# hzykent/LiDAL

Measured on AMD Instinct MI355X. Metric: voxels/sec SPVCNN fwd+bwd @120k pts, higher is better.
Workload: dtype bf16; 1 GPU; spvcnn train step (train.py:127-140: fwd + CE + bwd + Adam), 5 scans x ~120k pts per GPU, 0.05 m voxels, kernel maps rebuilt every step (each step builds the next step's coordinate tables on a second stream; variants.inline_geometry: built inside the forward pass); parallelism=dp1

## Files before the change

include/lidal_amd.h:

```cpp
#ifndef LIDAL_AMD_H
#define LIDAL_AMD_H

#include <stdint.h>

#ifdef __cplusplus
extern "C" {
#endif

#define LIDAL_F32 0
#define LIDAL_BF16 1
#define LIDAL_F32_SPLIT 2

const char* lidal_last_error(void);
int lidal_version(void);

int lidal_hash(const int32_t* coords, int64_t n, int64_t* out, void* stream);
int lidal_floor_coords(const float* coords, int64_t n, int stride, int32_t* out, void* stream);
int lidal_revoxelize_coords(const float* coords, int64_t n, float init_res, float after_res, float* out_float,
                            int32_t* out_floor, void* stream);
int lidal_kernel_hash(const int32_t* coords, int64_t n, const int32_t* offsets, int k,
                      int64_t* out, void* stream);

int64_t lidal_hash_table_bytes(int64_t n_keys);
int lidal_hash_table_build(const int64_t* keys, int64_t n, void* table, int64_t table_bytes,
                           void* stream);
int lidal_hash_table_build_coords(const int32_t* coords, int64_t n, int stride, void* table, int64_t table_bytes,
                                  void* stream);
int lidal_hash_table_query(const void* table, int64_t table_bytes, const int64_t* q, int64_t nq,
                           int64_t* out, void* stream);

int64_t lidal_unique_workspace_bytes(int64_t n);
int lidal_unique_sorted_i64(const int64_t* keys, int64_t n, int64_t* out, int64_t* n_out_dev,
                            void* ws, int64_t ws_bytes, void* stream);
int64_t lidal_downsample_workspace_bytes(int64_t n);
int lidal_downsample(const int32_t* coords, int64_t n, int sx, int sy, int sz, int32_t* out,
                     int64_t* n_out_dev, void* ws, int64_t ws_bytes, void* stream);

int64_t lidal_downsample_pyramid_workspace_bytes(int64_t n, int levels);
int lidal_downsample_pyramid(const int32_t* coords, int64_t n, int sx, int sy, int sz, int levels, int32_t* out,
                             int64_t* starts_dev, void* ws, int64_t ws_bytes, void* stream);

int64_t lidal_voxelize_points_workspace_bytes(int64_t p);
int lidal_voxelize_points(const float* points, const float* intensity, int64_t p,
                          const double* m_dev, const double* rnd_dev, double scale, int full_scale,
                          float* feats_p, int32_t* coords_v, int64_t* unique_idx, int64_t* inverse,
                          int64_t* n_out_dev, int32_t* n_invalid_dev, void* ws, int64_t ws_bytes,
                          void* stream);

int64_t lidal_train_labels_workspace_bytes(int64_t p);
int lidal_train_labels(const void* raw, int raw_bytes, int64_t p, const int64_t* label_map, int map_len,
                       const int64_t* sv_ptr, const int64_t* sv_idx, int64_t nnz, int s, const int64_t* sv_flag,
                       const int64_t* pseudo, const int64_t* unique_idx, int64_t n, int64_t* labels_p,
                       int64_t* labels_v, int32_t* n_invalid_dev, void* ws, int64_t ws_bytes, void* stream);

int64_t lidal_kmap_workspace_bytes(int64_t n_out, int k);
int lidal_kmap_build(const void* table, int64_t table_bytes, const int32_t* out_coords,
                     int64_t n_out, const int32_t* offsets, int k, int symmetric, int32_t* nbr_out,
                     int32_t* nbmaps, int32_t* nbsizes, int64_t* koff, int mode, void* ws,
                     int64_t ws_bytes, void* stream);
int lidal_kmap_from_rules(const int32_t* nbmaps, const int32_t* nbsizes, int k, int64_t n_rules,
                          int64_t n_in, int64_t n_out, int32_t* nbr_out, int32_t* n_bad_dev, void* stream);
int64_t lidal_kmap_build_batch_workspace_bytes(const int64_t* n_out, const int32_t* k, int n_jobs);
int lidal_kmap_build_batch(const void* const* tables, const int64_t* table_bytes,
                           const int32_t* const* out_coords, const int64_t* n_out,
                           const int32_t* const* offsets, const int32_t* k, const int32_t* symmetric,
                           int32_t* const* nbr_out, int32_t* const* nbmaps, int32_t* const* nbsizes,
                           int64_t* const* koff, int n_jobs, void* ws, int64_t ws_bytes, void* stream);
int lidal_kmap_invert(const int32_t* nbr_out, int64_t n_out, int k, int32_t* nbr_in, int64_t n_in,
                      void* stream);

int64_t lidal_sort_pairs_workspace_bytes(int64_t n);
int lidal_sort_pairs(const uint32_t* keys_in, const int32_t* vals_in, uint32_t* keys_out, int32_t* vals_out,
                     int64_t n, int bits, void* ws, int64_t ws_bytes, void* stream);
int lidal_sort_pairs_u64(const uint64_t* keys_in, const int32_t* vals_in, uint64_t* keys_out, int32_t* vals_out,
                         int64_t n, int bits, void* ws, int64_t ws_bytes, void* stream);
int64_t lidal_kmap_order_workspace_bytes(int64_t n_rows);
int lidal_kmap_order_batch(const int32_t* const* nbr, const int64_t* n_rows, int n_jobs, int k,
                           int32_t* const* perm, int32_t* const* nbr_perm, uint32_t* const* tile_masks,
                           void* ws, int64_t ws_bytes, void* stream);
int lidal_kmap_order(const int32_t* nbr, int64_t n_rows, int k, int32_t* perm, int32_t* nbr_perm,
                     uint32_t* tile_masks, void* ws, int64_t ws_bytes, void* stream);

int lidal_count(const int32_t* idx, int64_t n, int32_t* out, int64_t m, void* stream);
int lidal_voxelize_fwd(const float* feat, const int32_t* idx, const int32_t* counts, float* out,
                       int64_t n, int64_t m, int c, void* stream);
int lidal_voxelize_fwd_1to1(const void* feat, const int32_t* idx, void* out, int64_t n, int c, int dtype,
                            void* stream);
int lidal_voxelize_bwd(const void* gout, const int32_t* idx, const int32_t* counts,
                       const void* residual, void* gin, int64_t n, int64_t m, int c, int dtype,
                       void* stream);
int lidal_devoxelize_fwd(const void* feat, const int32_t* idx, const float* w, void* out,
                         int64_t n, int64_t m, int c, int dtype, void* stream);
int lidal_devoxelize_bwd(const float* gout, const int32_t* idx, const float* w, float* gin,
                         int64_t n, int64_t m, int c, void* stream);
int64_t lidal_invlist_workspace_bytes(int64_t n_entries);
int lidal_invlist_build(const int32_t* idx, const float* w, int64_t n_entries, int64_t m,
                        int32_t* order, int64_t* seg_ptr, void* ws, int64_t ws_bytes, void* stream);
int64_t lidal_segment_workspace_bytes(int64_t n_entries, int64_t m, int c);
int lidal_voxelize_fwd_sorted(const void* feat, const int32_t* order, const int64_t* seg_ptr,
                              const int32_t* counts, void* out, int64_t m, int c, int dtype,
                              int64_t n_entries, void* ws, int64_t ws_bytes, void* stream);
int lidal_devoxelize_bwd_sorted(const void* gout, const int32_t* order, const int64_t* seg_ptr,
                                const float* w, void* gin, int64_t m, int c, int dtype,
                                int64_t n_entries, void* ws, int64_t ws_bytes, void* stream);
int64_t lidal_devoxelize_bwd_cells_workspace_bytes(int64_t m, int c);
int lidal_devoxelize_bwd_cells(const void* gout, const int32_t* vorder, const int64_t* vseg, const float* w8,
                               const int32_t* corder, const int64_t* cseg, void* gin, int64_t m, int c, int dtype,
                               void* ws, int64_t ws_bytes, void* stream);
int lidal_ti_weights(const float* coords, int cstride, const int64_t* idx, int64_t n, float scale,
                     float* w, int32_t* idx32, void* stream);

int lidal_conv_stats_tile_rows(void);
int64_t lidal_conv_weight_image_bytes(int k, int ci, int co, int dtype, int64_t n_out);
int lidal_conv_weight_image_tiling(int ci, int co, int dtype, int64_t n_out);
int lidal_conv_weight_image(const void* w, int w_dtype, int role, void* img, int dtype, int k,
                            int n_red, int n_col, int64_t n_out, void* stream);
int lidal_conv_weight_image_pair(const void* w, int w_dtype, void* img_fwd, int64_t n_out_fwd,
                                 void* img_bwd, int64_t n_out_bwd, int dtype, int k, int ci, int co,
                                 void* stream);
int lidal_conv_weight_image_job_bytes(void);
int64_t lidal_conv_weight_image_job(void* job, const void* w, int role, void* img_fwd,
                                    int64_t n_out_fwd, void* img_bwd, int64_t n_out_bwd, int dtype,
                                    int k, int ci, int co, int64_t first);
int lidal_conv_weight_image_batch(const void* jobs, int n_jobs, int64_t total_segments, int w_dtype,
                                  int dtype, void* stream);
int lidal_conv_apply_image(const void* in, const void* wimg, const int32_t* nbr, const int32_t* perm,
                           const uint32_t* tile_masks, void* out, int64_t n_in, int64_t n_out,
                           int ci, int co, int k, int kflip, int dtype, const float* ep_scale,
                           const float* ep_shift, int ep_relu, const void* ep_residual,
                           float* tile_stats, void* stream);
int64_t lidal_conv_apply_workspace_bytes(int64_t n_out, int co);
int lidal_conv_apply_image_ws(const void* in, const void* wimg, const int32_t* nbr, const int32_t* perm,
                              const uint32_t* tile_masks, void* out, int64_t n_in, int64_t n_out,
                              int ci, int co, int k, int kflip, int dtype, const float* ep_scale,
                              const float* ep_shift, int ep_relu, const void* ep_residual,
                              float* tile_stats, void* ws, int64_t ws_bytes, void* stream);
int lidal_conv_dgrad_bn_sums(const void* gout, const void* wimg, const int32_t* nbr, const int32_t* perm,
                             const uint32_t* tile_masks, void* gin, int64_t n_gout, int64_t n_gin, int c_gout,
                             int c_gin, int k, int kflip, int dtype, const void* bn_x, const float* bn_mean,
                             const float* bn_invstd, const float* bn_gamma, const float* bn_beta, int bn_relu,
                             float* bn_sums, void* stream);
int lidal_conv_dgrad_bn_sums_ws(const void* gout, const void* wimg, const int32_t* nbr, const int32_t* perm,
                                const uint32_t* tile_masks, void* gin, int64_t n_gout, int64_t n_gin, int c_gout,
                                int c_gin, int k, int kflip, int dtype, const void* bn_x, const float* bn_mean,
                                const float* bn_invstd, const float* bn_gamma, const float* bn_beta, int bn_relu,
                                float* bn_sums, void* ws, int64_t ws_bytes, void* stream);
int64_t lidal_conv_wgrad_slabs(int64_t n_a, int64_t n_b, int k, int ca, int cb, int dtype);
int lidal_conv_wgrad(const void* a, const void* b, int64_t n_a, int64_t n_b, const int32_t* pairs,
                     const int64_t* koff, int a_col, float* gw, float* partial, int64_t n_slabs,
                     int k, int ca, int cb, int dtype, void* stream);

int lidal_wgrad_streams_workgroups(void);
int64_t lidal_wgrad_streams_rules(int64_t n_rows, int k, int n_wg);
int64_t lidal_wgrad_streams_desc_words(int k, int n_wg);
int64_t lidal_wgrad_streams_workspace_bytes(int64_t n_rows, int k);
int lidal_wgrad_streams_build(const int32_t* pairs, const int64_t* koff, int k, int64_t n_rows, const int32_t* key_tab,
                              int key_k, int64_t key_range, int n_wg, int32_t* spairs, int64_t spairs_rules,
                              int32_t* sdesc, void* ws, int64_t ws_bytes, void* stream);
int lidal_conv_wgrad_streams_serves(int64_t n_a, int64_t n_b, int k, int ca, int cb);
int lidal_conv_wgrad_streams(const void* a, const void* b, int64_t n_a, int64_t n_b, const int32_t* spairs,
                             const int32_t* sdesc, int n_wg, int a_col, float* gw, float* partial, int64_t n_slabs,
                             int k, int ca, int cb, int dtype, void* stream);

int64_t lidal_bn_workspace_bytes(int64_t n, int c);
int lidal_bn_train_fwd(const void* x, int dtype, int64_t n, int c, const float* gamma,
                       const float* beta, float eps, float momentum, float* running_mean,
                       float* running_var, int64_t* num_batches_tracked, int relu,
                       const void* residual, void* y, float* save_mean, float* save_invstd, void* ws,
                       int64_t ws_bytes, void* stream);
int lidal_bn_train_fwd_tiles(const void* x, int dtype, int64_t n, int c, const float* gamma,
                             const float* beta, float eps, float momentum, float* running_mean,
                             float* running_var, int64_t* num_batches_tracked, int relu,
                             const void* residual, void* y, float* save_mean, float* save_invstd,
                             const float* tile_stats, int64_t n_tiles, void* stream);
int lidal_bn_eval_fwd(const void* x, int dtype, int64_t n, int c, const float* gamma,
                      const float* beta, const float* running_mean, const float* running_var,
                      float eps, int relu, void* y, void* stream);
int lidal_bn_bwd(const void* x, const void* dy, int64_t dy_stride, int dtype, int64_t n, int c, const float* gamma,
                 const float* beta, int relu, const float* save_mean, const float* save_invstd,
                 void* dx, float* grad_gamma, float* grad_beta, void* ws, int64_t ws_bytes,
                 void* stream);
int lidal_bn_bwd_tiles(const void* x, const void* dy, int64_t dy_stride, int dtype, int64_t n, int c,
                       const float* gamma, const float* beta, int relu, const float* save_mean,
                       const float* save_invstd, void* dx, float* grad_gamma, float* grad_beta,
                       const float* tile_sums, int64_t n_tiles, void* stream);
int lidal_add_relu_bwd_bn_sums(const void* out, const void* g, void* gm, int dtype, int64_t n, int c,
                               const void* x_a, const float* mean_a, const float* invstd_a, void* part_a,
                               const void* x_b, const float* mean_b, const float* invstd_b, void* part_b,
                               int64_t part_bytes, void* stream);
int64_t lidal_bn_tail_parts(int64_t n, int c, int dtype);
int lidal_add_relu_bwd_bn_tile_sums(const void* out, const void* g, void* gm, int dtype, int64_t n, int c,
                                    const void* x_a, const float* mean_a, const float* invstd_a, float* sums_a,
                                    const void* x_b, const float* mean_b, const float* invstd_b, float* sums_b,
                                    int64_t n_parts, void* stream);
int lidal_bn_bwd_from_sums(const void* x, const void* dy, int64_t dy_stride, int dtype, int64_t n, int c,
                           const float* gamma, const float* beta, int relu, const float* save_mean,
                           const float* save_invstd, void* dx, float* grad_gamma, float* grad_beta,
                           const void* part, int64_t part_bytes, void* stream);
int lidal_bn_set_fused(int on);
int lidal_bn_set_slab_sums(int on);
int lidal_bn_check_device(void);
int lidal_bn_fold(const float* gamma, const float* beta, const float* running_mean,
                  const float* running_var, float eps, int c, float* scale, float* shift,
                  void* stream);
int lidal_colsum(const void* x, int dtype, int64_t n, int c, float* out, void* ws,
                 int64_t ws_bytes, void* stream);

int lidal_add_relu_fwd(const void* a, const void* b, void* y, int64_t numel, int dtype,
                       void* stream);
int lidal_add_relu_bwd(const void* y, const void* g, void* gin, int64_t numel, int dtype,
                       void* stream);
int64_t lidal_ce_workspace_bytes(int64_t n);
int lidal_ce_fwd(const void* logits, int dtype, const int64_t* labels, int64_t n, int c,
                 int64_t ignore_index, float* out2, void* ws, int64_t ws_bytes, void* stream);
int lidal_ce_bwd(const void* logits, int dtype, const int64_t* labels, int64_t n, int c,
                 int64_t ignore_index, const float* fwd_out2, const float* grad_scale,
                 void* dlogits, void* stream);

int lidal_view_mean_softmax(const float* logits, const int64_t* inverse, int reps, int64_t p,
                            int c, float* prob, int64_t* pred, void* stream);

int lidal_confusion_accumulate(const float* logits, const int64_t* inverse, const int64_t* labels,
                               int64_t p, int c, int32_t* conf, void* stream);

int lidal_register_points(const float* points, int64_t p, const double* pose_dev, double* world,
                          void* stream);
int64_t lidal_nn_grid_bytes(int64_t p);
int64_t lidal_nn_grid_workspace_bytes(int64_t p);
int lidal_nn_grid_build(const double* pts, int64_t p, double cell, void* grid, int64_t grid_bytes,
                        void* ws, int64_t ws_bytes, void* stream);
int64_t lidal_interframe_workspace_bytes(int64_t p, int n_nei);
int lidal_interframe_score(const double* q_pts, const float* q_prob, int64_t p, int c,
                           const void* const* nei_grids_host, const double* const* nei_pts_host,
                           const float* const* nei_prob_host, const int64_t* nei_p_host,
                           int n_nei, double dis_thresh, double* interd, float* intere,
                           int32_t* map_count, void* ws, int64_t ws_bytes, void* stream);
int lidal_interframe_score_ordered(const double* q_pts, const float* q_prob, int64_t p, int c,
                                   const void* const* nei_grids_host, const double* const* nei_pts_host,
                                   const float* const* nei_prob_host, const int64_t* nei_p_host,
                                   int n_nei, double dis_thresh, double* interd, float* intere,
                                   int32_t* map_count, void* ws, int64_t ws_bytes, const void* q_grid,
                                   void* stream);
int lidal_supervoxel_reduce(const double* interd, const float* intere, const double* pts,
                            const int64_t* sv_ptr, const int64_t* sv_idx, int s, float* sv_interd,
                            float* sv_intere, float* sv_center, void* stream);

int64_t lidal_knn_workspace_bytes(int64_t p);
int lidal_knn(const float* xyz, int64_t p, int k, double cell, int32_t* knn, void* ws, int64_t ws_bytes, void* stream);
int lidal_surface_variation(const float* xyz, int64_t p, int k, double cell, float threshold, float* sigma, void* ws,
                            int64_t ws_bytes, void* stream);
int64_t lidal_region_scores_workspace_bytes(int64_t p);
int lidal_region_scores(const float* prob, int64_t p, int c, const float* feat, int d, const float* curvature,
                        const int64_t* sv_ptr, const int64_t* sv_idx, int s, float alpha, float gamma, float* sv_scores,
                        float* sv_feats, int64_t* sv_pnums, void* ws, int64_t ws_bytes, void* stream);
int64_t lidal_kmeans_workspace_bytes(int64_t n, int d, int k, int trials);
int lidal_kmeans(const float* x, int64_t n, int d, int k, int64_t first, const double* u, int trials, int max_iter,
                 double tol, int32_t* seeds, int32_t* labels, double* centers, double* inertia_host,
                 int32_t* n_iter_host, void* ws, int64_t ws_bytes, void* stream);

int64_t lidal_frame_uncertainty_workspace_bytes(int64_t p);
int lidal_frame_uncertainty(const float* prob, int64_t p, int c, float* out, void* ws, int64_t ws_bytes, void* stream);
int64_t lidal_segment_entropy_workspace_bytes(int s);
int lidal_segment_entropy(const int64_t* pred, int64_t p, const int64_t* sv_ptr, const int64_t* sv_idx, int s,
                          int class_num, double* out, void* ws, int64_t ws_bytes, void* stream);
int64_t lidal_frame_feature_workspace_bytes(int64_t p);
int lidal_frame_feature(const float* feat, int64_t p, int d, float* out, void* ws, int64_t ws_bytes, void* stream);
int64_t lidal_coreset_workspace_bytes(int64_t n, int num_add);
int lidal_coreset(const float* feats, int64_t n, int d, const int64_t* labeled, int64_t n_labeled, int num_add,
                  int64_t* picks, float* min_dist, int32_t* status_dev, void* ws, int64_t ws_bytes, void* stream);

int lidal_copy2d(const void* src, int64_t src_pitch, void* dst, int64_t dst_pitch, int64_t rows, int64_t row_bytes,
                 int64_t zero_bytes, void* stream);
int lidal_add2d(const void* a, int64_t a_stride, const void* b, int64_t b_stride, void* out, int64_t out_stride,
                int64_t rows, int c, int dtype, void* stream);
int lidal_transpose_f32(const float* src, int64_t src_stride, float* dst, int rows, int cols, void* stream);
int lidal_cast_rows_bf16(const float* src, int c_src, void* dst, int c_dst, int64_t n, void* stream);

enum {
  LIDAL_OP_CONV_WEIGHT_IMAGE_BATCH = 1, LIDAL_OP_CONV_APPLY_IMAGE = 2, LIDAL_OP_CONV_DGRAD_BN_SUMS = 3,
  LIDAL_OP_CONV_WGRAD = 4, LIDAL_OP_BN_TRAIN_FWD = 5, LIDAL_OP_BN_TRAIN_FWD_TILES = 6, LIDAL_OP_BN_BWD = 7,
  LIDAL_OP_BN_BWD_TILES = 8, LIDAL_OP_BN_EVAL_FWD = 9, LIDAL_OP_BN_FOLD = 10, LIDAL_OP_COLSUM = 11,
  LIDAL_OP_ADD_RELU_FWD = 12, LIDAL_OP_ADD_RELU_BWD = 13, LIDAL_OP_VOXELIZE_FWD_1TO1 = 14,
  LIDAL_OP_VOXELIZE_FWD_SORTED = 15, LIDAL_OP_VOXELIZE_BWD = 16, LIDAL_OP_DEVOXELIZE_FWD = 17,
  LIDAL_OP_DEVOXELIZE_BWD_SORTED = 18, LIDAL_OP_CE_FWD = 19, LIDAL_OP_CE_BWD = 20, LIDAL_OP_COPY2D = 21,
  LIDAL_OP_ADD2D = 22, LIDAL_OP_TRANSPOSE_F32 = 23, LIDAL_OP_CAST_ROWS_BF16 = 24, LIDAL_OP_VIEW_MEAN_SOFTMAX = 25,
  LIDAL_OP_FORK_SIDE = 26, LIDAL_OP_JOIN_SIDE = 27, LIDAL_OP_CONV_APPLY_IMAGE_WS = 28,
  LIDAL_OP_CONV_DGRAD_BN_SUMS_WS = 29, LIDAL_OP_ADD_RELU_BWD_BN_SUMS = 30, LIDAL_OP_BN_BWD_FROM_SUMS = 31,
  LIDAL_OP_ADD_RELU_BWD_BN_TILE_SUMS = 32, LIDAL_OP_DEVOXELIZE_BWD_CELLS = 33,
  LIDAL_OP_CONV_WGRAD_STREAMS = 34
};
#define LIDAL_OP_FLAG_SIDE 1
int lidal_plan_op_args(int kind);
int lidal_debug_read(const void* dev, void* host, int64_t nbytes);
int lidal_plan_run(const int64_t* words, int64_t n_words, int64_t n_ops, void* stream, void* side_stream);
int lidal_plan_run_streams(const int64_t* words, int64_t n_words, int64_t n_ops, void* const* streams, int n_streams);

#ifdef __cplusplus
}
#endif
#endif
```

lidal_amd/backend.py:

```python
import ctypes
import os

import torch

_HERE = os.path.dirname(os.path.abspath(__file__))
LIB_PATH = os.environ.get('LIDAL_AMD_LIB') or os.path.join(_HERE, 'liblidal_amd.so')

F32, BF16 = 0, 1
_lib = None
HITS = {}


def hit(name):
    HITS[name] = HITS.get(name, 0) + 1

_vp, _i32, _i64, _f32, _f64 = (ctypes.c_void_p, ctypes.c_int, ctypes.c_int64, ctypes.c_float,
                               ctypes.c_double)

SIGNATURES = {
    'lidal_last_error': (ctypes.c_char_p, []),
    'lidal_version': (_i32, []),
    'lidal_floor_coords': (_i32, [_vp, _i64, _i32, _vp, _vp]),
    'lidal_revoxelize_coords': (_i32, [_vp, _i64, _f32, _f32, _vp, _vp, _vp]),
    'lidal_hash': (_i32, [_vp, _i64, _vp, _vp]),
    'lidal_kernel_hash': (_i32, [_vp, _i64, _vp, _i32, _vp, _vp]),
    'lidal_hash_table_bytes': (_i64, [_i64]),
    'lidal_hash_table_build_coords': (_i32, [_vp, _i64, _i32, _vp, _i64, _vp]),
    'lidal_hash_table_build': (_i32, [_vp, _i64, _vp, _i64, _vp]),
    'lidal_hash_table_query': (_i32, [_vp, _i64, _vp, _i64, _vp, _vp]),
    'lidal_unique_workspace_bytes': (_i64, [_i64]),
    'lidal_unique_sorted_i64': (_i32, [_vp, _i64, _vp, _vp, _vp, _i64, _vp]),
    'lidal_downsample_workspace_bytes': (_i64, [_i64]),
    'lidal_downsample': (_i32, [_vp, _i64, _i32, _i32, _i32, _vp, _vp, _vp, _i64, _vp]),
    'lidal_downsample_pyramid_workspace_bytes': (_i64, [_i64, _i32]),
    'lidal_downsample_pyramid': (_i32, [_vp, _i64, _i32, _i32, _i32, _i32, _vp, _vp, _vp, _i64, _vp]),
    'lidal_voxelize_points_workspace_bytes': (_i64, [_i64]),
    'lidal_voxelize_points': (_i32, [_vp, _vp, _i64, _vp, _vp, _f64, _i32, _vp, _vp, _vp, _vp, _vp, _vp,
                                     _vp, _i64, _vp]),
    'lidal_train_labels_workspace_bytes': (_i64, [_i64]),
    'lidal_train_labels': (_i32, [_vp, _i32, _i64, _vp, _i32, _vp, _vp, _i64, _i32, _vp, _vp, _vp, _i64, _vp, _vp, _vp,
                                  _vp, _i64, _vp]),
    'lidal_kmap_workspace_bytes': (_i64, [_i64, _i32]),
    'lidal_kmap_build': (_i32, [_vp, _i64, _vp, _i64, _vp, _i32, _i32, _vp, _vp, _vp, _vp, _i32, _vp,
                                _i64, _vp]),
    'lidal_kmap_build_batch_workspace_bytes': (_i64, [_vp, _vp, _i32]),
    'lidal_kmap_build_batch': (_i32, [_vp, _vp, _vp, _vp, _vp, _vp, _vp, _vp, _vp, _vp, _vp, _i32, _vp, _i64, _vp]),
    'lidal_kmap_invert': (_i32, [_vp, _i64, _i32, _vp, _i64, _vp]),
    'lidal_kmap_from_rules': (_i32, [_vp, _vp, _i32, _i64, _i64, _i64, _vp, _vp, _vp]),
    'lidal_count': (_i32, [_vp, _i64, _vp, _i64, _vp]),
    'lidal_voxelize_fwd': (_i32, [_vp, _vp, _vp, _vp, _i64, _i64, _i32, _vp]),
    'lidal_voxelize_fwd_1to1': (_i32, [_vp, _vp, _vp, _i64, _i32, _i32, _vp]),
    'lidal_voxelize_bwd': (_i32, [_vp, _vp, _vp, _vp, _vp, _i64, _i64, _i32, _i32, _vp]),
    'lidal_devoxelize_fwd': (_i32, [_vp, _vp, _vp, _vp, _i64, _i64, _i32, _i32, _vp]),
    'lidal_devoxelize_bwd': (_i32, [_vp, _vp, _vp, _vp, _i64, _i64, _i32, _vp]),
    'lidal_invlist_workspace_bytes': (_i64, [_i64]),
    'lidal_invlist_build': (_i32, [_vp, _vp, _i64, _i64, _vp, _vp, _vp, _i64, _vp]),
    'lidal_segment_workspace_bytes': (_i64, [_i64, _i64, _i32]),
    'lidal_voxelize_fwd_sorted': (_i32, [_vp, _vp, _vp, _vp, _vp, _i64, _i32, _i32, _i64, _vp, _i64, _vp]),
    'lidal_devoxelize_bwd_sorted': (_i32, [_vp, _vp, _vp, _vp, _vp, _i64, _i32, _i32, _i64, _vp, _i64, _vp]),
    'lidal_devoxelize_bwd_cells': (_i32, [_vp, _vp, _vp, _vp, _vp, _vp, _vp, _i64, _i32, _i32, _vp, _i64, _vp]),
    'lidal_devoxelize_bwd_cells_workspace_bytes': (_i64, [_i64, _i32]),
    'lidal_ti_weights': (_i32, [_vp, _i32, _vp, _i64, _f32, _vp, _vp, _vp]),
    'lidal_sort_pairs_workspace_bytes': (_i64, [_i64]),
    'lidal_sort_pairs': (_i32, [_vp, _vp, _vp, _vp, _i64, _i32, _vp, _i64, _vp]),
    'lidal_sort_pairs_u64': (_i32, [_vp, _vp, _vp, _vp, _i64, _i32, _vp, _i64, _vp]),
    'lidal_kmap_order_workspace_bytes': (_i64, [_i64]),
    'lidal_kmap_order': (_i32, [_vp, _i64, _i32, _vp, _vp, _vp, _vp, _i64, _vp]),
    'lidal_kmap_order_batch': (_i32, [_vp, _vp, _i32, _i32, _vp, _vp, _vp, _vp, _i64, _vp]),
    'lidal_conv_stats_tile_rows': (_i32, []),
    'lidal_conv_weight_image_bytes': (_i64, [_i32, _i32, _i32, _i32, _i64]),
    'lidal_conv_weight_image_tiling': (_i32, [_i32, _i32, _i32, _i64]),
    'lidal_conv_weight_image': (_i32, [_vp, _i32, _i32, _vp, _i32, _i32, _i32, _i32, _i64, _vp]),
    'lidal_conv_weight_image_pair': (_i32, [_vp, _i32, _vp, _i64, _vp, _i64, _i32, _i32, _i32, _i32, _vp]),
    'lidal_conv_weight_image_job_bytes': (_i32, []),
    'lidal_conv_weight_image_job': (_i64, [_vp, _vp, _i32, _vp, _i64, _vp, _i64, _i32, _i32, _i32, _i32, _i64]),
    'lidal_conv_weight_image_batch': (_i32, [_vp, _i32, _i64, _i32, _i32, _vp]),
    'lidal_conv_apply_image': (_i32, [_vp, _vp, _vp, _vp, _vp, _vp, _i64, _i64, _i32, _i32, _i32, _i32, _i32, _vp,
                                      _vp, _i32, _vp, _vp, _vp]),
    'lidal_conv_dgrad_bn_sums': (_i32, [_vp, _vp, _vp, _vp, _vp, _vp, _i64, _i64, _i32, _i32, _i32, _i32, _i32, _vp,
                                        _vp, _vp, _vp, _vp, _i32, _vp, _vp]),
    'lidal_conv_apply_workspace_bytes': (_i64, [_i64, _i32]),
    'lidal_conv_apply_image_ws': (_i32, [_vp, _vp, _vp, _vp, _vp, _vp, _i64, _i64, _i32, _i32, _i32, _i32, _i32, _vp,
                                         _vp, _i32, _vp, _vp, _vp, _i64, _vp]),
    'lidal_conv_dgrad_bn_sums_ws': (_i32, [_vp, _vp, _vp, _vp, _vp, _vp, _i64, _i64, _i32, _i32, _i32, _i32, _i32, _vp,
                                           _vp, _vp, _vp, _vp, _i32, _vp, _vp, _i64, _vp]),
    'lidal_conv_wgrad_slabs': (_i64, [_i64, _i64, _i32, _i32, _i32, _i32]),
    'lidal_conv_wgrad': (_i32, [_vp, _vp, _i64, _i64, _vp, _vp, _i32, _vp, _vp, _i64, _i32, _i32, _i32, _i32, _vp]),
    'lidal_conv_wgrad_streams': (_i32, [_vp, _vp, _i64, _i64, _vp, _vp, _i32, _i32, _vp, _vp, _i64, _i32, _i32, _i32, _i32, _vp]),
    'lidal_conv_wgrad_streams_serves': (_i32, [_i64, _i64, _i32, _i32, _i32]),
    'lidal_wgrad_streams_workgroups': (_i32, []),
    'lidal_wgrad_streams_rules': (_i64, [_i64, _i32, _i32]),
    'lidal_wgrad_streams_desc_words': (_i64, [_i32, _i32]),
    'lidal_wgrad_streams_workspace_bytes': (_i64, [_i64, _i32]),
    'lidal_wgrad_streams_build': (_i32, [_vp, _vp, _i32, _i64, _vp, _i32, _i64, _i32, _vp, _i64, _vp, _vp, _i64, _vp]),
    'lidal_bn_workspace_bytes': (_i64, [_i64, _i32]),
    'lidal_bn_train_fwd': (_i32, [_vp, _i32, _i64, _i32, _vp, _vp, _f32, _f32, _vp, _vp, _vp, _i32, _vp, _vp, _vp,
                                  _vp, _vp, _i64, _vp]),
    'lidal_bn_train_fwd_tiles': (_i32, [_vp, _i32, _i64, _i32, _vp, _vp, _f32, _f32, _vp, _vp, _vp, _i32, _vp, _vp,
                                        _vp, _vp, _vp, _i64, _vp]),
    'lidal_bn_eval_fwd': (_i32, [_vp, _i32, _i64, _i32, _vp, _vp, _vp, _vp, _f32, _i32, _vp, _vp]),
    'lidal_bn_bwd': (_i32, [_vp, _vp, _i64, _i32, _i64, _i32, _vp, _vp, _i32, _vp, _vp, _vp, _vp, _vp, _vp,
                            _i64, _vp]),
    'lidal_bn_bwd_tiles': (_i32, [_vp, _vp, _i64, _i32, _i64, _i32, _vp, _vp, _i32, _vp, _vp, _vp, _vp, _vp, _vp,
                                  _i64, _vp]),
    'lidal_add_relu_bwd_bn_sums': (_i32, [_vp, _vp, _vp, _i32, _i64, _i32, _vp, _vp, _vp, _vp, _vp, _vp, _vp, _vp, _i64, _vp]),
    'lidal_add_relu_bwd_bn_tile_sums': (_i32, [_vp, _vp, _vp, _i32, _i64, _i32, _vp, _vp, _vp, _vp, _vp, _vp, _vp, _vp, _i64, _vp]),
    'lidal_bn_tail_parts': (_i64, [_i64, _i32, _i32]),
    'lidal_bn_bwd_from_sums': (_i32, [_vp, _vp, _i64, _i32, _i64, _i32, _vp, _vp, _i32, _vp, _vp, _vp, _vp, _vp, _vp,
                                      _i64, _vp]),
    'lidal_bn_set_fused': (_i32, [_i32]),
    'lidal_bn_set_slab_sums': (_i32, [_i32]),
    'lidal_bn_check_device': (_i32, []),
    'lidal_bn_fold': (_i32, [_vp, _vp, _vp, _vp, _f32, _i32, _vp, _vp, _vp]),
    'lidal_colsum': (_i32, [_vp, _i32, _i64, _i32, _vp, _vp, _i64, _vp]),
    'lidal_add_relu_fwd': (_i32, [_vp, _vp, _vp, _i64, _i32, _vp]),
    'lidal_add_relu_bwd': (_i32, [_vp, _vp, _vp, _i64, _i32, _vp]),
    'lidal_ce_workspace_bytes': (_i64, [_i64]),
    'lidal_ce_fwd': (_i32, [_vp, _i32, _vp, _i64, _i32, _i64, _vp, _vp, _i64, _vp]),
    'lidal_ce_bwd': (_i32, [_vp, _i32, _vp, _i64, _i32, _i64, _vp, _vp, _vp, _vp]),
    'lidal_view_mean_softmax': (_i32, [_vp, _vp, _i32, _i64, _i32, _vp, _vp, _vp]),
    'lidal_confusion_accumulate': (_i32, [_vp, _vp, _vp, _i64, _i32, _vp, _vp]),
    'lidal_register_points': (_i32, [_vp, _i64, _vp, _vp, _vp]),
    'lidal_nn_grid_bytes': (_i64, [_i64]),
    'lidal_nn_grid_workspace_bytes': (_i64, [_i64]),
    'lidal_nn_grid_build': (_i32, [_vp, _i64, _f64, _vp, _i64, _vp, _i64, _vp]),
    'lidal_interframe_workspace_bytes': (_i64, [_i64, _i32]),
    'lidal_interframe_score': (_i32, [_vp, _vp, _i64, _i32, _vp, _vp, _vp, _vp, _i32, _f64, _vp,
                                      _vp, _vp, _vp, _i64, _vp]),
    'lidal_interframe_score_ordered': (_i32, [_vp, _vp, _i64, _i32, _vp, _vp, _vp, _vp, _i32, _f64, _vp,
                                              _vp, _vp, _vp, _i64, _vp, _vp]),
    'lidal_supervoxel_reduce': (_i32, [_vp, _vp, _vp, _vp, _vp, _i32, _vp, _vp, _vp, _vp]),
    'lidal_knn_workspace_bytes': (_i64, [_i64]),
    'lidal_knn': (_i32, [_vp, _i64, _i32, _f64, _vp, _vp, _i64, _vp]),
    'lidal_surface_variation': (_i32, [_vp, _i64, _i32, _f64, _f32, _vp, _vp, _i64, _vp]),
    'lidal_region_scores_workspace_bytes': (_i64, [_i64]),
    'lidal_region_scores': (_i32, [_vp, _i64, _i32, _vp, _i32, _vp, _vp, _vp, _i32, _f32, _f32, _vp, _vp, _vp, _vp,
                                   _i64, _vp]),
    'lidal_kmeans_workspace_bytes': (_i64, [_i64, _i32, _i32, _i32]),
    'lidal_kmeans': (_i32, [_vp, _i64, _i32, _i32, _i64, _vp, _i32, _i32, _f64, _vp, _vp, _vp, _vp, _vp, _vp, _i64,
                            _vp]),
    'lidal_frame_uncertainty_workspace_bytes': (_i64, [_i64]),
    'lidal_frame_uncertainty': (_i32, [_vp, _i64, _i32, _vp, _vp, _i64, _vp]),
    'lidal_segment_entropy_workspace_bytes': (_i64, [_i32]),
    'lidal_segment_entropy': (_i32, [_vp, _i64, _vp, _vp, _i32, _i32, _vp, _vp, _i64, _vp]),
    'lidal_frame_feature_workspace_bytes': (_i64, [_i64]),
    'lidal_frame_feature': (_i32, [_vp, _i64, _i32, _vp, _vp, _i64, _vp]),
    'lidal_coreset_workspace_bytes': (_i64, [_i64, _i32]),
    'lidal_coreset': (_i32, [_vp, _i64, _i32, _vp, _i64, _i32, _vp, _vp, _vp, _vp, _i64, _vp]),
    'lidal_copy2d': (_i32, [_vp, _i64, _vp, _i64, _i64, _i64, _i64, _vp]),
    'lidal_add2d': (_i32, [_vp, _i64, _vp, _i64, _vp, _i64, _i64, _i32, _i32, _vp]),
    'lidal_transpose_f32': (_i32, [_vp, _i64, _vp, _i32, _i32, _vp]),
    'lidal_cast_rows_bf16': (_i32, [_vp, _i32, _vp, _i32, _i64, _vp]),
    'lidal_plan_op_args': (_i32, [_i32]),
    'lidal_debug_read': (_i32, [_vp, _vp, _i64]),
    'lidal_plan_run': (_i32, [_vp, _i64, _i64, _vp, _vp]),
    'lidal_plan_run_streams': (_i32, [_vp, _i64, _i64, _vp, _i32]),
}


class _TimedLib:

    def __init__(self, handle, sink):
        self._handle, self._sink = handle, sink

    def __getattr__(self, name):
        fn = getattr(self._handle, name)
        if fn.restype is not _i32 or name.endswith(('_bytes', '_tiling', '_rows', '_workgroups', '_serves')) or name == 'lidal_version':
            return fn
        sink = self._sink

        def timed(*args):
            e0 = torch.cuda.Event(enable_timing=True)
            e1 = torch.cuda.Event(enable_timing=True)
            e0.record()
            rc = fn(*args)
            e1.record()
            sink(name, args, e0, e1)
            return rc
        return timed


_timer = None


def set_call_timer(sink):
    global _timer
    _timer = None if sink is None else _TimedLib(lib_handle(), sink)


def lib_handle():
    global _lib
    if _lib is None:
        if not os.path.exists(LIB_PATH):
            raise RuntimeError(
                'lidal_amd: %s is missing -- build it with `python -m lidal_amd.build` '
                '(hipcc --offload-arch=gfx950).  There is no CPU fallback.' % LIB_PATH)
        handle = ctypes.CDLL(LIB_PATH)
        for name, (res, args) in SIGNATURES.items():
            fn = getattr(handle, name)
            fn.restype = res
            fn.argtypes = args
        _lib = handle
    return _lib


def lib():
    return _timer if _timer is not None else lib_handle()


def check(rc, what):
    HITS[what] = HITS.get(what, 0) + 1
    if rc != 0:
        raise RuntimeError('lidal_amd.%s failed (%d): %s' %
                           (what, rc, lib().lidal_last_error().decode()))


def bind_cpus_near(device_index=0):
    try:
        props = torch.cuda.get_device_properties(device_index)
        bdf = '%04x:%02x:%02x.0' % (props.pci_domain_id, props.pci_bus_id, props.pci_device_id)
        text = open('/sys/bus/pci/devices/%s/local_cpulist' % bdf).read().strip()
        cpus = set()
        for part in text.split(','):
            if '-' in part:
                a, b = part.split('-')
                cpus.update(range(int(a), int(b) + 1))
            elif part:
                cpus.add(int(part))
        cpus &= os.sched_getaffinity(0)
        if not cpus:
            return None
        os.sched_setaffinity(0, cpus)
        for tid in os.listdir('/proc/self/task'):
            try:
                os.sched_setaffinity(int(tid), cpus)
            except (OSError, ValueError):
                pass
        return cpus
# ... 295 lines not shown
```

lidal_amd/csrc/conv_img.hip:

```cpp
#include <type_traits>

#include "common.h"

using namespace lidal;

namespace {

typedef __attribute__((ext_vector_type(4))) float f32x4;
typedef __attribute__((ext_vector_type(8))) __bf16 bf16x8;
typedef int raw4 __attribute__((ext_vector_type(4)));

template <typename T> struct DT;
template <> struct DT<float> {
  static constexpr int VEC = 4;
  static constexpr int CH = 16;
  typedef f32x4 frag;
  __device__ static float to_f32(float v) { return v; }
  __device__ static float from_f32(float v) { return v; }
};
template <> struct DT<__bf16> {
  static constexpr int VEC = 8;
  static constexpr int CH = 32;
  typedef bf16x8 frag;
  __device__ static float to_f32(__bf16 v) { return (float)v; }
  __device__ static __bf16 from_f32(float v) { return (__bf16)v; }
};

__device__ __forceinline__ void mma(f32x4& acc, const f32x4& a, const f32x4& b) {
#pragma unroll
  for (int e = 0; e < 4; ++e) acc = __builtin_amdgcn_mfma_f32_16x16x4f32(a[e], b[e], acc, 0, 0, 0);
}
__device__ __forceinline__ void mma(f32x4& acc, const bf16x8& a, const bf16x8& b) {
  acc = __builtin_amdgcn_mfma_f32_16x16x32_bf16(a, b, acc, 0, 0, 0);
}

constexpr int MAXK = 32;

constexpr int NB4_LIMIT = 384;
struct Tiling { int nb; int row_bytes; };

__host__ __device__ inline Tiling pick_tiling(int ci, int co, int64_t n_out, int esz) {
  Tiling t;
  const int row_bytes = ci * esz;
  t.row_bytes = (row_bytes % 192 == 0 && row_bytes % 128 != 0) ? 192
                : (row_bytes % 128 != 0 && row_bytes % 64 == 0) ? 64 : 128;
  if (co <= 32) t.nb = 2;
  else if (co <= 64 || (co % 64 == 0 && ((n_out + 127) / 128) * ((co + 127) / 128) <= NB4_LIMIT)) t.nb = 4;
  else if (co % 128 != 0 && (co % 96 == 0 || co < 128)) t.nb = 6;
  else t.nb = 8;
  return t;
}
__host__ __device__ inline int64_t image_bytes(int k, int ci, int co, Tiling t, int esz) {
  const int bn = 16 * t.nb, kc = t.row_bytes / esz;
  const int nblk = (co + bn - 1) / bn, npass = (ci + kc - 1) / kc;
  return (int64_t)k * nblk * npass * bn * t.row_bytes;
}

template <typename TI, typename TO>
__device__ __forceinline__ void image_segment(const TI* __restrict__ w, TO* __restrict__ img, int n_red,
                                              int n_col, int role, int nb, int kc, int64_t s) {
  constexpr int VEC = DT<TO>::VEC, CH = DT<TO>::CH;
  const int bn = 16 * nb, ncc = kc / CH;
  const int nblk = (n_col + bn - 1) / bn, npass = (n_red + kc - 1) / kc;
  unsigned r = (unsigned)s;
  const int row16 = (int)(r & 15u); r >>= 4;
  const int b = (int)(r % (unsigned)nb); r /= (unsigned)nb;
  const int gsel = (int)(r & 3u); r >>= 2;
  const int cc = (int)(r % (unsigned)ncc); r /= (unsigned)ncc;
  const int pass = (int)(r % (unsigned)npass); r /= (unsigned)npass;
  const int blk = (int)(r % (unsigned)nblk); r /= (unsigned)nblk;
  const int k = (int)r;
  const int col = blk * bn + b * 16 + row16;
  const int red0 = pass * kc + cc * CH + gsel * VEC;
  if (role != 0) {
    if (gsel != 0) return;
    const bool inside = col < n_col;
    const int64_t src = (int64_t)k * n_red * n_col + (int64_t)col * n_red + red0;
    float f[CH];
    if (inside && red0 + CH <= n_red && sizeof(TI) == 4 && (n_red & 3) == 0 && (reinterpret_cast<uintptr_t>(w) & 15) == 0) {
#pragma unroll
      for (int e = 0; e < CH; e += 4) {
        const float4 q = *reinterpret_cast<const float4*>(reinterpret_cast<const float*>(w) + src + e);
        f[e] = q.x; f[e + 1] = q.y; f[e + 2] = q.z; f[e + 3] = q.w;
      }
    } else {
#pragma unroll
      for (int e = 0; e < CH; ++e) f[e] = (inside && red0 + e < n_red) ? DT<TI>::to_f32(w[src + e]) : 0.f;
    }
    typedef typename DT<TO>::frag frag;
#pragma unroll
    for (int g = 0; g < 4; ++g) {
      TO v[VEC];
#pragma unroll
      for (int e = 0; e < VEC; ++e) v[e] = DT<TO>::from_f32(f[g * VEC + e]);
      *reinterpret_cast<frag*>(img + (s + (int64_t)g * nb * 16) * VEC) = *reinterpret_cast<frag*>(v);
    }
    return;
  }
  TO v[VEC];
#pragma unroll
  for (int e = 0; e < VEC; ++e) {
    const int red = red0 + e;
    float f = 0.f;
    if (col < n_col && red < n_red) {
      const int64_t base = (int64_t)k * n_red * n_col;
      f = DT<TI>::to_f32(role == 0 ? w[base + (int64_t)red * n_col + col] : w[base + (int64_t)col * n_red + red]);
    }
    v[e] = DT<TO>::from_f32(f);
  }
  typedef typename DT<TO>::frag frag;
  *reinterpret_cast<frag*>(img + s * VEC) = *reinterpret_cast<frag*>(v);
}

template <typename TI, typename TO>
__global__ void __launch_bounds__(256)
weight_image_kernel(const TI* __restrict__ w, TO* __restrict__ img_a, int n_red, int n_col, int role,
                    int nb_a, int kc_a, int64_t segs_a, TO* __restrict__ img_b, int nb_b, int kc_b,
                    int64_t segs_b) {
  const int64_t s = (int64_t)blockIdx.x * blockDim.x + threadIdx.x;
  if (s < segs_a) image_segment<TI, TO>(w, img_a, n_red, n_col, role, nb_a, kc_a, s);
  else if (s < segs_a + segs_b) image_segment<TI, TO>(w, img_b, n_col, n_red, role ^ 1, nb_b, kc_b, s - segs_a);
}

struct ImageJob {
  const void* w; void* img_a; void* img_b;
  long long first, segs_a, segs_b;
  int n_red, n_col, role, nb_a, kc_a, nb_b, kc_b, pad;
};
template <typename TI, typename TO>
__global__ void __launch_bounds__(256)
weight_image_batch_kernel(const ImageJob* __restrict__ jobs, int n_jobs, int64_t total) {
  const int64_t s = (int64_t)blockIdx.x * blockDim.x + threadIdx.x;
  if (s >= total) return;
  int lo = 0, hi = n_jobs - 1;
  while (lo < hi) {
    const int mid = (lo + hi + 1) >> 1;
    if (jobs[mid].first <= s) lo = mid; else hi = mid - 1;
  }
  const ImageJob j = jobs[lo];
  const int64_t l = s - j.first;
  if (l < j.segs_a) image_segment<TI, TO>((const TI*)j.w, (TO*)j.img_a, j.n_red, j.n_col, j.role, j.nb_a, j.kc_a, l);
  else if (l < j.segs_a + j.segs_b)
    image_segment<TI, TO>((const TI*)j.w, (TO*)j.img_b, j.n_col, j.n_red, j.role ^ 1, j.nb_b, j.kc_b, l - j.segs_a);
}

constexpr int TILE_ROWS = 128;
__device__ __forceinline__ int tile_of_block() { return (int)gridDim.x - 1 - (int)blockIdx.x; }
constexpr int LEAN_WAVES = 8;
constexpr int LEAN_MINWAVES = 4;
constexpr int64_t DEEP_MAX_ROWS = 150000;
struct BnBwd {
  const void* x; const float* mean; const float* invstd; const float* gamma; const float* beta;
  float* sums;
  int relu;
};

struct Split { float* partial; int nsplit; int co_pad; long long rows_pad; };

template <typename T, int NB, int G, int NWAVES>
__device__ __forceinline__ void store_tile(f32x4 (&acc)[G][NB], unsigned char* wl, int wave, int lane,
                                           int64_t r0, int n0, int64_t n_out, int co,
                                           const int* __restrict__ perm, T* __restrict__ out,
                                           const float* __restrict__ ep_scale,
                                           const float* __restrict__ ep_shift, int ep_relu,
                                           const T* __restrict__ ep_res, bool perm_in_reg = false,
                                           int perm_v = 0, float* __restrict__ tile_stats = nullptr,
                                           int stats_tile = -1, const BnBwd* bnb = nullptr) {
  constexpr int VEC = DT<T>::VEC;
  constexpr int BN = 16 * NB;
  constexpr int RW = G * 16;
  constexpr int ESTRIDE = BN + VEC;
  typedef typename DT<T>::frag frag;
  const int row16 = lane & 15, gsel = lane >> 4;
  T* et = reinterpret_cast<T*>(wl) + wave * RW * ESTRIDE;
  if (ep_scale != nullptr) {
#pragma unroll
    for (int nb = 0; nb < NB; ++nb) {
      const int col = n0 + nb * 16 + row16;
      const float es = col < co ? ep_scale[col] : 1.f, eh = col < co ? ep_shift[col] : 0.f;
#pragma unroll
      for (int g = 0; g < G; ++g)
#pragma unroll
        for (int r = 0; r < 4; ++r) {
          float v = acc[g][nb][r] * es + eh;
          acc[g][nb][r] = ((ep_relu & 1) && v < 0.f) ? 0.f : v;
        }
    }
  }
#pragma unroll
  for (int g = 0; g < G; ++g)
#pragma unroll
    for (int nb = 0; nb < NB; ++nb)
#pragma unroll
      for (int r = 0; r < 4; ++r)
        et[(g * 16 + gsel * 4 + r) * ESTRIDE + nb * 16 + row16] = DT<T>::from_f32(acc[g][nb][r]);
  __builtin_amdgcn_s_waitcnt(0xC07F);
  constexpr int RSEGS = BN / VEC;
  for (int i = lane; i < RW * RSEGS; i += 64) {
    const int r = i / RSEGS, cseg = (i - r * RSEGS) * VEC;
    const int prow = perm_in_reg ? __shfl(perm_v, r & (RW - 1), 64) : 0;
    if (r0 + r >= n_out) continue;
    const int64_t row = perm ? (perm_in_reg ? (int64_t)prow : (int64_t)perm[r0 + r]) : r0 + r;
    T* dst = out + row * co + n0 + cseg;
    const T* srcp = et + r * ESTRIDE + cseg;
    if (n0 + cseg + VEC <= co) {
      frag v = *reinterpret_cast<const frag*>(srcp);
      if (ep_res != nullptr) {
        const frag rr = *reinterpret_cast<const frag*>(ep_res + row * co + n0 + cseg);
#pragma unroll
        for (int e = 0; e < VEC; ++e) {
          float f = DT<T>::to_f32(v[e]) + DT<T>::to_f32(rr[e]);
          if ((ep_relu & 2) && f < 0.f) f = 0.f;
          v[e] = DT<T>::from_f32(f);
        }
      }
      *reinterpret_cast<frag*>(dst) = v;
    } else {
#pragma unroll
      for (int e = 0; e < VEC; ++e)
        if (n0 + cseg + e < co) {
          float v = DT<T>::to_f32(srcp[e]);
          if (ep_res != nullptr) {
            v += DT<T>::to_f32(ep_res[row * co + n0 + cseg + e]);
            if ((ep_relu & 2) && v < 0.f) v = 0.f;
          }
          dst[e] = DT<T>::from_f32(v);
        }
    }
  }
  if (tile_stats != nullptr) {
    constexpr int EPI_BYTES = NWAVES * RW * ESTRIDE * (int)sizeof(T);
    float* st = reinterpret_cast<float*>(wl + EPI_BYTES);
    const int64_t left = n_out - r0;
    const int nvalid = left <= 0 ? 0 : (left < RW ? (int)left : RW);
    const float inv_n = nvalid > 0 ? 1.f / (float)nvalid : 0.f;
#pragma unroll
    for (int nb = 0; nb < NB; ++nb) {
      float v[G][4];
      float sum = 0.f;
#pragma unroll
      for (int g = 0; g < G; ++g)
#pragma unroll
        for (int r = 0; r < 4; ++r) {
          v[g][r] = DT<T>::to_f32(DT<T>::from_f32(acc[g][nb][r]));
          if (g * 16 + gsel * 4 + r < nvalid) sum += v[g][r];
        }
      sum += __shfl_xor(sum, 16, 64);
      sum += __shfl_xor(sum, 32, 64);
      const float mean = sum * inv_n;
      float m2 = 0.f;
#pragma unroll
      for (int g = 0; g < G; ++g)
#pragma unroll
        for (int r = 0; r < 4; ++r)
          if (g * 16 + gsel * 4 + r < nvalid) { const float d = v[g][r] - mean; m2 += d * d; }
      m2 += __shfl_xor(m2, 16, 64);
      m2 += __shfl_xor(m2, 32, 64);
      if (gsel == 0) {
        st[(wave * BN + nb * 16 + row16) * 2] = mean;
        st[(wave * BN + nb * 16 + row16) * 2 + 1] = m2;
      }
    }
    __syncthreads();
    const int c = wave * 64 + lane;
    if (c < BN && n0 + c < co) {
      const int64_t rb = r0 - (int64_t)wave * RW;
      float na = 0.f, ma = 0.f, qa = 0.f;
      for (int w = 0; w < NWAVES; ++w) {
        const int64_t lw = n_out - (rb + (int64_t)w * RW);
        const float nw = lw <= 0 ? 0.f : (lw < RW ? (float)lw : (float)RW);
        if (nw > 0.f) {
          const float mw = st[(w * BN + c) * 2], qw = st[(w * BN + c) * 2 + 1];
          const float n = na + nw, d = mw - ma;
          ma += d * (nw / n);
          qa += qw + d * d * (na * nw / n);
          na = n;
        }
      }
      float* dst = tile_stats + ((int64_t)(n0 + c) * gridDim.x + (stats_tile >= 0 ? stats_tile : (int)blockIdx.x)) * 3;
      dst[0] = na; dst[1] = ma; dst[2] = qa;
    }
  }
  if (bnb != nullptr && bnb->sums != nullptr) {
    constexpr int EPI_BYTES = NWAVES * RW * ESTRIDE * (int)sizeof(T);
    float* st = reinterpret_cast<float*>(wl + EPI_BYTES);
    const T* bx = reinterpret_cast<const T*>(bnb->x);
    const int64_t left = n_out - r0;
    const int nvalid = left <= 0 ? 0 : (left < RW ? (int)left : RW);
    __builtin_amdgcn_s_waitcnt(0xC07F);
    for (int i = lane; i < RW * RSEGS; i += 64) {
      const int r = i / RSEGS, cseg = (i - r * RSEGS) * VEC;
      const int prow = perm_in_reg ? __shfl(perm_v, r & (RW - 1), 64) : 0;
      frag v;
#pragma unroll
      for (int e = 0; e < VEC; ++e) v[e] = DT<T>::from_f32(0.f);
      if (r < nvalid && n0 + cseg + VEC <= co) {
        const int64_t row = perm ? (perm_in_reg ? (int64_t)prow : (int64_t)perm[r0 + r]) : r0 + r;
        v = *reinterpret_cast<const frag*>(bx + row * co + n0 + cseg);
      }
      *reinterpret_cast<frag*>(et + r * ESTRIDE + cseg) = v;
    }
    __builtin_amdgcn_s_waitcnt(0xC07F);
#pragma unroll
    for (int nb = 0; nb < NB; ++nb) {
      const int col = n0 + nb * 16 + row16;
      const bool cok = col < co;
      const float mu = cok ? bnb->mean[col] : 0.f, is = cok ? bnb->invstd[col] : 0.f;
      const float ga = (cok && bnb->gamma) ? bnb->gamma[col] : 1.f, be = (cok && bnb->beta) ? bnb->beta[col] : 0.f;
      float a = 0.f, b = 0.f;
#pragma unroll
      for (int g = 0; g < G; ++g)
#pragma unroll
        for (int r = 0; r < 4; ++r) {
          const int rr = g * 16 + gsel * 4 + r;
          if (rr < nvalid) {
            const float xh = (DT<T>::to_f32(et[rr * ESTRIDE + nb * 16 + row16]) - mu) * is;
            float dy = DT<T>::to_f32(DT<T>::from_f32(acc[g][nb][r]));
            if (bnb->relu && !(xh * ga + be > 0.f)) dy = 0.f;
            a += dy; b += dy * xh;
          }
        }
      a += __shfl_xor(a, 16, 64); a += __shfl_xor(a, 32, 64);
      b += __shfl_xor(b, 16, 64); b += __shfl_xor(b, 32, 64);
      if (gsel == 0) {
        st[(wave * BN + nb * 16 + row16) * 2] = a;
        st[(wave * BN + nb * 16 + row16) * 2 + 1] = b;
      }
    }
    __syncthreads();
    const int c = wave * 64 + lane;
    if (c < BN && n0 + c < co) {
      float a = 0.f, b = 0.f;
      for (int w = 0; w < NWAVES; ++w) { a += st[(w * BN + c) * 2]; b += st[(w * BN + c) * 2 + 1]; }
      float* dst = bnb->sums + ((int64_t)(n0 + c) * gridDim.x + (stats_tile >= 0 ? stats_tile : (int)blockIdx.x)) * 2;
      dst[0] = a; dst[1] = b;
    }
  }
}

constexpr int IMG_MINWAVES = 2;

template <typename T, int NB, int ROW_BYTES, int G, int NWAVES, int MINW, bool DENSE, int D>
__global__ void __launch_bounds__(64 * NWAVES, MINW)
conv_apply_img_kernel(const T* __restrict__ in, const T* __restrict__ wimg,
                      const int* __restrict__ nbr, const int* __restrict__ perm,
                      const unsigned* __restrict__ tmasks, T* __restrict__ out, int64_t n_out,
                      int ci, int co, int K, int kflip, const float* __restrict__ ep_scale,
                      const float* __restrict__ ep_shift, int ep_relu, const T* __restrict__ ep_res,
                      unsigned in_bytes, unsigned img_bytes, unsigned nbr_bytes,
                      float* __restrict__ tile_stats, BnBwd bnb) {
  constexpr int NTHREADS = 64 * NWAVES;
  constexpr int BM = NWAVES * G * 16;
  constexpr int BN = 16 * NB;
  constexpr int VEC = DT<T>::VEC;
  constexpr int CH = DT<T>::CH;
  constexpr int KC = ROW_BYTES / (int)sizeof(T);
  constexpr int MAXCC = KC / CH;
  constexpr int SLAB = BN * ROW_BYTES;
  constexpr int PIECES = SLAB / 1024;
  constexpr int PPW = (PIECES + NWAVES - 1) / NWAVES;
  constexpr int RW = G * 16;
  constexpr int ESTRIDE = BN + VEC;
  constexpr int EPI = NWAVES * RW * ESTRIDE * (int)sizeof(T);
  constexpr int R = D + 1;
  constexpr int WREGION = (R * SLAB > EPI) ? R * SLAB : EPI;
  constexpr int GA = G * MAXCC;
  static_assert(D >= 1 && D <= 3, "pipeline depth 1..3");
  static_assert(SLAB % 1024 == 0, "slab must be whole LDS-DMA pieces");
  typedef typename DT<T>::frag frag;

  extern __shared__ __attribute__((aligned(16))) unsigned char smem[];
  unsigned char* wl = smem;
  unsigned char* dump = smem + WREGION;

  const int tid = threadIdx.x;
  const int lane = tid & 63;
  const int wave = __builtin_amdgcn_readfirstlane(tid >> 6);
  const int row16 = lane & 15;
  const int gsel = lane >> 4;
  const int bx = tile_of_block();
  const int64_t r0 = (int64_t)bx * BM + wave * RW;
  const int n0 = blockIdx.y * BN;
  const int npass = (ci + KC - 1) / KC;

  unsigned tmask;
  if constexpr (DENSE) {
    tmask = 1u;
  } else {
    unsigned m = 0u;
    const int64_t t0 = ((int64_t)bx * BM) >> 7;
#pragma unroll
    for (int h = 0; h < (BM >= 128 ? BM / 128 : 1); ++h)
      if ((t0 + h) * 128 < n_out) m |= tmasks[t0 + h];
    if (kflip) m = __brev(m) >> (32 - K);
    tmask = m;
  }
  tmask = __builtin_amdgcn_readfirstlane(tmask);
  const int n_act = __popc(tmask);
  const int nphase = n_act * npass;

  struct Walk { unsigned rem; int k; int pass; };
  auto walk_begin = [&]() {
    Walk w;
    w.k = tmask ? __builtin_ctz(tmask) : 0;
    w.rem = tmask & (tmask - 1u);
    w.pass = 0;
    return w;
  };
  auto walk_next = [&](Walk& w) {
    if (++w.pass == npass) {
      w.pass = 0;
      w.k = w.rem ? __builtin_ctz(w.rem) : 0;
      w.rem &= w.rem - 1u;
    }
  };

  constexpr unsigned OOB_OFF = 0x80000000u;
  const __amdgpu_buffer_rsrc_t rs_in =
      __builtin_amdgcn_make_buffer_rsrc(const_cast<T*>(in), 0, (int)in_bytes, 0x00020000);
  const __amdgpu_buffer_rsrc_t rs_w =
      __builtin_amdgcn_make_buffer_rsrc(const_cast<T*>(wimg), 0, (int)img_bytes, 0x00020000);
  const __amdgpu_buffer_rsrc_t rs_nbr =
      __builtin_amdgcn_make_buffer_rsrc(const_cast<int*>(nbr), 0, (int)nbr_bytes, 0x00020000);
  const int nblk = gridDim.y;

  auto stage_dma = [&](int k, int pass, int slot, bool live) {
    const unsigned slab_off = (unsigned)((((int64_t)k * nblk + blockIdx.y) * npass + pass) * SLAB);
#pragma unroll
    for (int t = 0; t < PPW; ++t) {
      const int piece = wave + t * NWAVES;
      const bool ok = live && piece < PIECES;
      unsigned char* dst = ok ? wl + slot * SLAB + piece * 1024 : dump;
      const unsigned soff = ok ? slab_off + (unsigned)piece * 1024u : OOB_OFF;
      __builtin_amdgcn_raw_ptr_buffer_load_lds(rs_w, (__attribute__((address_space(3))) void*)dst, 16,
                                               (unsigned)lane * 16u, soff, 0, 0);
    }
  };
  const unsigned row_off = (unsigned)((r0 + row16) * 4);
  bool row_ok[G];
#pragma unroll
  for (int g = 0; g < G; ++g) row_ok[g] = r0 + g * 16 + row16 < n_out;
  auto load_idx = [&](int (&dst)[G], int k) {
    if constexpr (DENSE) {
#pragma unroll
      for (int g = 0; g < G; ++g) dst[g] = (int)(r0 + g * 16 + row16);
    } else {
      const int kk = kflip ? (K - 1 - k) : k;
      const unsigned koff = (unsigned)kk * (unsigned)n_out * 4u;
#pragma unroll
      for (int g = 0; g < G; ++g)
        dst[g] = __builtin_amdgcn_raw_buffer_load_b32(rs_nbr, row_off + (unsigned)(g * 64), koff, 0);
    }
  };
  auto kill_bit = [&](bool live) {
    unsigned kb = live ? 0u : OOB_OFF;
    asm volatile("" : "+s"(kb));
    return kb;
  };
  auto load_a = [&](raw4 (&a)[G][MAXCC], unsigned long long (&present)[G], const int (&idx)[G],
                    int c0, bool live) {
    const int kc = min(KC, ci - c0);
    const unsigned row_bytes = (unsigned)(ci * (int)sizeof(T));
    const unsigned lane_off = (unsigned)((c0 + gsel * VEC) * (int)sizeof(T));
    const unsigned kill = kill_bit(live);
    const unsigned long long live_mask = kill ? 0ull : ~0ull;
#pragma unroll
    for (int g = 0; g < G; ++g) {
      int src = row_ok[g] ? idx[g] : -1;
      present[g] = __ballot(src != -1) & live_mask;
      const unsigned base = ((src >= 0) ? (unsigned)src * row_bytes + lane_off : OOB_OFF) | kill;
#pragma unroll
      for (int cc = 0; cc < MAXCC; ++cc) {
        const unsigned off = (cc * CH + gsel * VEC < kc) ? base + (unsigned)(cc * CH * (int)sizeof(T)) : OOB_OFF;
        a[g][cc] = __builtin_bit_cast(raw4, __builtin_amdgcn_raw_buffer_load_b128(rs_in, off, 0, 0));
      }
    }
  };

  f32x4 acc[G][NB];
#pragma unroll
  for (int g = 0; g < G; ++g)
#pragma unroll
    for (int nb = 0; nb < NB; ++nb) acc[g][nb] = f32x4{0.f, 0.f, 0.f, 0.f};

// ... 836 lines not shown
  constexpr int SLAB = BN * ROW_BYTES;
  constexpr int EPI = NWAVES * G * 16 * (BN + DT<T>::VEC) * (int)sizeof(T);
  constexpr int D = IMG_DEPTH;
  constexpr int WREGION = ((D + 1) * SLAB > EPI) ? (D + 1) * SLAB : EPI;
  static_assert(BM == TILE_ROWS, "tile masks and BatchNorm statistics triples are per 128-row tile");
  if constexpr (G == 1 && NWAVES == 8) {
    if (ci % (ROW_BYTES / (int)sizeof(T)) == 0 && ep.in_bytes / ((unsigned)ci * sizeof(T)) < (1u << 24)) {
      constexpr int LW = LEAN_WAVES;
      constexpr int LBM = LW * 16;
      static_assert(LBM == TILE_ROWS, "tile masks and BatchNorm statistics triples are per 128-row tile");
      constexpr int LEPI = LW * 16 * (BN + DT<T>::VEC) * (int)sizeof(T);
      constexpr int LSTATS = LW * BN * 2 * (int)sizeof(float);
      constexpr int LEAN_LDS = ((2 * SLAB > LEPI + LSTATS) ? 2 * SLAB : LEPI + LSTATS) + 4096;
      if constexpr (sizeof(T) == 2 && NB == 8 && ROW_BYTES == 128 && LW == 8) {
#ifdef LIDAL_PHASE_STAMPS
       if (false) {
#else
       if (nbr != nullptr && n_out <= DEEP_MAX_ROWS && n_out >= 30000 && ci >= 256) {
#endif
        constexpr int DEPI = LEPI + LSTATS;
        constexpr int DEEP_LDS = ((3 * SLAB > DEPI) ? 3 * SLAB : DEPI) + 4096;
        auto dk = conv_lean_deep_kernel<T, NB, ROW_BYTES, LW, false>;
        static size_t deep_attr[MAX_DEVICES] = {};
        const int ddev = current_device();
        if (deep_attr[ddev] < (size_t)DEEP_LDS) {
          LIDAL_HIP(hipFuncSetAttribute(reinterpret_cast<const void*>(dk),
                                        hipFuncAttributeMaxDynamicSharedMemorySize, DEEP_LDS));
          deep_attr[ddev] = DEEP_LDS;
        }
        dim3 dgrid((unsigned)cdiv(n_out, LBM), (unsigned)cdiv(co, BN));
        dk<<<dgrid, 64 * LW, DEEP_LDS, s>>>((const T*)in, (const T*)wimg, nbr, perm, tmasks, (T*)out, n_out,
                                            ci, co, K, kflip, ep.scale, ep.shift, ep.relu, (const T*)ep.res,
                                            ep.in_bytes, ep.img_bytes, ep.nbr_bytes, ep.tile_stats, ep.bnb);
        LIDAL_CHECK_LAUNCH("lidal_conv_apply_image(deep)");
        return 0;
       }
      }
      auto lk = nbr ? conv_lean_kernel<T, NB, ROW_BYTES, LW, false>
                    : conv_lean_kernel<T, NB, ROW_BYTES, LW, true>;
      static size_t lean_attr[2][MAX_DEVICES] = {};
      const int ldev = current_device();
      if (lean_attr[nbr ? 0 : 1][ldev] < (size_t)LEAN_LDS) {
        LIDAL_HIP(hipFuncSetAttribute(reinterpret_cast<const void*>(lk),
                                      hipFuncAttributeMaxDynamicSharedMemorySize, LEAN_LDS));
        lean_attr[nbr ? 0 : 1][ldev] = LEAN_LDS;
      }
      dim3 lgrid((unsigned)cdiv(n_out, LBM), (unsigned)cdiv(co, BN));
      Split sp{nullptr, 1, 0, 0};
      if (nbr != nullptr && ep.ws != nullptr && sizeof(T) == 2) {
        const int ns = pick_split((int64_t)lgrid.x * lgrid.y, K, ci / (ROW_BYTES / (int)sizeof(T)));
        const long long rows_pad = (long long)lgrid.x * LBM;
        const int co_pad = (int)lgrid.y * BN;
        if (ns > 1 && ep.ws_bytes >= (long long)ns * rows_pad * co_pad * 4)
          sp = Split{(float*)ep.ws, ns, co_pad, rows_pad};
      }
      lgrid.z = (unsigned)sp.nsplit;
      lk<<<lgrid, 64 * LW, LEAN_LDS, s>>>((const T*)in, (const T*)wimg, nbr, perm, tmasks, (T*)out, n_out,
                                          ci, co, K, kflip, ep.scale, ep.shift, ep.relu, (const T*)ep.res,
                                          ep.in_bytes, ep.img_bytes, ep.nbr_bytes, ep.tile_stats, ep.bnb, sp);
      LIDAL_CHECK_LAUNCH("lidal_conv_apply_image(lean)");
      if (sp.nsplit > 1) {
        constexpr int COMB_LDS = LEPI + LSTATS;
        auto ck = conv_combine_kernel<T, NB, LW>;
        static size_t comb_attr[MAX_DEVICES] = {};
        if (comb_attr[ldev] < (size_t)COMB_LDS) {
          LIDAL_HIP(hipFuncSetAttribute(reinterpret_cast<const void*>(ck),
                                        hipFuncAttributeMaxDynamicSharedMemorySize, COMB_LDS));
          comb_attr[ldev] = COMB_LDS;
        }
        lgrid.z = 1;
        ck<<<lgrid, 64 * LW, COMB_LDS, s>>>(sp, perm, (T*)out, n_out, co, ep.scale, ep.shift, ep.relu,
                                            (const T*)ep.res, ep.tile_stats, ep.bnb);
        LIDAL_CHECK_LAUNCH("lidal_conv_apply_image(combine)");
      }
      return 0;
    }
  }
  const size_t lds = WREGION + 1024 + NWAVES * BN * 2 * sizeof(float);
  auto kern = nbr ? conv_apply_img_kernel<T, NB, ROW_BYTES, G, NWAVES, IMG_MINWAVES, false, D>
                  : conv_apply_img_kernel<T, NB, ROW_BYTES, G, NWAVES, IMG_MINWAVES, true, D>;
  static size_t attr_set[2][MAX_DEVICES] = {};
  const int dev = current_device();
  if (attr_set[nbr ? 0 : 1][dev] < lds) {
    LIDAL_HIP(hipFuncSetAttribute(reinterpret_cast<const void*>(kern),
                                  hipFuncAttributeMaxDynamicSharedMemorySize, (int)lds));
    attr_set[nbr ? 0 : 1][dev] = lds;
  }
  dim3 grid((unsigned)cdiv(n_out, BM), (unsigned)cdiv(co, BN));
  kern<<<grid, NTHREADS, lds, s>>>((const T*)in, (const T*)wimg, nbr, perm, tmasks, (T*)out, n_out, ci,
                                   co, K, kflip, ep.scale, ep.shift, ep.relu, (const T*)ep.res,
                                   ep.in_bytes, ep.img_bytes, ep.nbr_bytes, ep.tile_stats, ep.bnb);
  LIDAL_CHECK_LAUNCH("lidal_conv_apply_image");
  return 0;
}

template <typename T>
int dispatch_img(Tiling t, const void* in, const void* wimg, const int* nbr, const int* perm,
                 const unsigned* tmasks, void* out, int64_t n_out, int ci, int co, int K, int kflip,
                 Epi ep, hipStream_t s) {
#define IMG_CASE(NBV, RB) \
  if (t.nb == NBV && t.row_bytes == RB) \
    return launch_img<T, NBV, RB>(in, wimg, nbr, perm, tmasks, out, n_out, ci, co, K, kflip, ep, s);
  IMG_CASE(2, 64) IMG_CASE(4, 64) IMG_CASE(6, 64) IMG_CASE(8, 64)
  IMG_CASE(2, 128) IMG_CASE(4, 128) IMG_CASE(6, 128) IMG_CASE(8, 128)
  IMG_CASE(2, 192) IMG_CASE(4, 192) IMG_CASE(6, 192) IMG_CASE(8, 192)
  IMG_CASE(2, 256) IMG_CASE(4, 256) IMG_CASE(6, 256) IMG_CASE(8, 256)
#undef IMG_CASE
  set_error("conv_apply_image: no kernel for tiling nb=%d row_bytes=%d", t.nb, t.row_bytes);
  return 2;
}


__host__ inline int split_nb(int co) { return co <= 32 ? 2 : (co <= 64 ? 4 : ((co % 128 != 0 && (co % 96 == 0 || co < 128)) ? 6 : 8)); }
__host__ inline int64_t split_image_bytes(int k, int n_red, int n_col) {
  const int bn = 16 * split_nb(n_col);
  return (int64_t)k * ((n_col + bn - 1) / bn) * (n_red / SPLIT_KCH) * bn * SPLIT_ROW;
}
template <int NB>
int launch_split(const void* in, const void* wimg, const int* nbr, const int* perm, const unsigned* tmasks, void* out,
                 int64_t n_out, int ci, int co, int K, int kflip, Epi ep, hipStream_t s) {
  constexpr int LW = 8, BN = 16 * NB, SLAB = BN * SPLIT_ROW;
  constexpr int LEPI_ALL = LW * 16 * (BN + 4) * 4 + LW * BN * 2 * (int)sizeof(float);
  constexpr int LDS = ((2 * SLAB > LEPI_ALL) ? 2 * SLAB : LEPI_ALL) + 4096;
  auto kern = nbr ? conv_split_kernel<NB, LW, false> : conv_split_kernel<NB, LW, true>;
  static size_t attr[2][MAX_DEVICES] = {};
  const int dev = current_device();
  if (attr[nbr ? 0 : 1][dev] < (size_t)LDS) {
    LIDAL_HIP(hipFuncSetAttribute(reinterpret_cast<const void*>(kern), hipFuncAttributeMaxDynamicSharedMemorySize, LDS));
    attr[nbr ? 0 : 1][dev] = LDS;
  }
  dim3 grid((unsigned)cdiv(n_out, LW * 16), (unsigned)cdiv(co, BN));
  Split sp{nullptr, 1, 0, 0};
  if (nbr != nullptr && ep.ws != nullptr) {
    const int64_t wgs = (int64_t)grid.x * grid.y;
    const int ns = (wgs > SPLIT_F32_MAX_WGS || K * (ci / SPLIT_KCH) < 54) ? 1 : (wgs <= 256 ? 4 : 3);
    const long long rows_pad = (long long)grid.x * LW * 16;
    const int co_pad = (int)grid.y * BN;
    if (ns > 1 && ep.ws_bytes >= (long long)ns * rows_pad * co_pad * 4) sp = Split{(float*)ep.ws, ns, co_pad, rows_pad};
  }
  grid.z = (unsigned)sp.nsplit;
  kern<<<grid, 64 * LW, LDS, s>>>((const float*)in, (const __bf16*)wimg, nbr, perm, tmasks, (float*)out, n_out, ci, co, K,
                                  kflip, ep.scale, ep.shift, ep.relu, (const float*)ep.res, ep.in_bytes, ep.img_bytes,
                                  ep.nbr_bytes, sp);
  LIDAL_CHECK_LAUNCH("lidal_conv_apply_image(split)");
  if (sp.nsplit > 1) {
    constexpr int COMB_LDS = LEPI_ALL;
    auto ck = conv_combine_kernel<float, NB, LW>;
    static size_t comb_attr[MAX_DEVICES] = {};
    if (comb_attr[dev] < (size_t)COMB_LDS) {
      LIDAL_HIP(hipFuncSetAttribute(reinterpret_cast<const void*>(ck), hipFuncAttributeMaxDynamicSharedMemorySize, COMB_LDS));
      comb_attr[dev] = COMB_LDS;
    }
    grid.z = 1;
    BnBwd none{nullptr, nullptr, nullptr, nullptr, nullptr, nullptr, 0};
    ck<<<grid, 64 * LW, COMB_LDS, s>>>(sp, perm, (float*)out, n_out, co, ep.scale, ep.shift, ep.relu, (const float*)ep.res,
                                       nullptr, none);
    LIDAL_CHECK_LAUNCH("lidal_conv_apply_image(split, combine)");
  }
  return 0;
}

}

extern "C" int lidal_conv_stats_tile_rows(void) { return TILE_ROWS; }

extern "C" int lidal_conv_weight_image_tiling(int ci, int co, int dtype, int64_t n_out) {
  if (dtype == LIDAL_F32_SPLIT) return split_nb(co) * 1000 + SPLIT_ROW + 1;
  const Tiling t = pick_tiling(ci, co, n_out, dtype == LIDAL_BF16 ? 2 : 4);
  return t.nb * 1000 + t.row_bytes;
}

extern "C" int64_t lidal_conv_weight_image_bytes(int k, int ci, int co, int dtype, int64_t n_out) {
  if (dtype == LIDAL_F32_SPLIT) return (ci > 0 && ci % SPLIT_KCH == 0) ? split_image_bytes(k, ci, co) : -1;
  const int esz = dtype == LIDAL_BF16 ? 2 : 4;
  return image_bytes(k, ci, co, pick_tiling(ci, co, n_out, esz), esz);
}

static int weight_images(const void* w, int w_dtype, int role, void* img_a, int64_t n_out_a, void* img_b,
                         int64_t n_out_b, int dtype, int k, int n_red, int n_col, hipStream_t s) {
  if (k == 0 || n_red == 0 || n_col == 0) return 0;
  LIDAL_REQUIRE(role == 0 || role == 1, "weight_image: role must be 0 (forward) or 1 (data gradient)");
  if (dtype == LIDAL_F32_SPLIT) {
    LIDAL_REQUIRE(img_b == nullptr && n_red % SPLIT_KCH == 0, "weight_image(split): one image per call, reduction a "
                  "multiple of %d channels (got %d)", SPLIT_KCH, n_red);
    const int64_t segs = split_image_bytes(k, n_red, n_col) / 16;
    LIDAL_REQUIRE(segs < (1ll << 31), "weight_image: an image of more than 2^31 segments");
    const unsigned grid = (unsigned)cdiv(segs, 256);
    if (w_dtype == LIDAL_F32)
      weight_image_split_kernel<float><<<grid, 256, 0, s>>>((const float*)w, (__bf16*)img_a, n_red, n_col, role,
                                                            split_nb(n_col), segs);
    else
      weight_image_split_kernel<__bf16><<<grid, 256, 0, s>>>((const __bf16*)w, (__bf16*)img_a, n_red, n_col, role,
                                                             split_nb(n_col), segs);
    LIDAL_CHECK_LAUNCH("lidal_conv_weight_image(split)");
    return 0;
  }
  const int esz = dtype == LIDAL_BF16 ? 2 : 4;
  const Tiling ta = pick_tiling(n_red, n_col, n_out_a, esz);
  const int64_t segs_a = image_bytes(k, n_red, n_col, ta, esz) / 16;
  Tiling tb = ta;
  int64_t segs_b = 0;
  if (img_b != nullptr) {
    tb = pick_tiling(n_col, n_red, n_out_b, esz);
    segs_b = image_bytes(k, n_col, n_red, tb, esz) / 16;
  }
  LIDAL_REQUIRE(segs_a < (1ll << 31) && segs_b < (1ll << 31), "weight_image: an image of more than 2^31 segments");
  const unsigned grid = (unsigned)cdiv(segs_a + segs_b, 256);
#define IMG_LAUNCH(TI, TO) \
  weight_image_kernel<TI, TO><<<grid, 256, 0, s>>>((const TI*)w, (TO*)img_a, n_red, n_col, role, ta.nb, \
                                                   ta.row_bytes / esz, segs_a, (TO*)img_b, tb.nb,       \
                                                   tb.row_bytes / esz, segs_b)
  if (w_dtype == LIDAL_F32 && dtype == LIDAL_F32) IMG_LAUNCH(float, float);
  else if (w_dtype == LIDAL_F32 && dtype == LIDAL_BF16) IMG_LAUNCH(float, __bf16);
  else if (w_dtype == LIDAL_BF16 && dtype == LIDAL_BF16) IMG_LAUNCH(__bf16, __bf16);
  else if (w_dtype == LIDAL_BF16 && dtype == LIDAL_F32) IMG_LAUNCH(__bf16, float);
  else {
    set_error("weight_image: bad dtypes %d %d", w_dtype, dtype);
    return 2;
  }
#undef IMG_LAUNCH
  LIDAL_CHECK_LAUNCH("lidal_conv_weight_image");
  return 0;
}

extern "C" int lidal_conv_weight_image(const void* w, int w_dtype, int role, void* img, int dtype,
                                       int k, int n_red, int n_col, int64_t n_out, void* stream) {
  return weight_images(w, w_dtype, role, img, n_out, nullptr, 0, dtype, k, n_red, n_col, (hipStream_t)stream);
}

extern "C" int lidal_conv_weight_image_pair(const void* w, int w_dtype, void* img_fwd, int64_t n_out_fwd,
                                            void* img_bwd, int64_t n_out_bwd, int dtype, int k, int ci,
                                            int co, void* stream) {
  return weight_images(w, w_dtype, 0, img_fwd, n_out_fwd, img_bwd, n_out_bwd, dtype, k, ci, co,
                       (hipStream_t)stream);
}

extern "C" int lidal_conv_weight_image_job_bytes(void) { return (int)sizeof(ImageJob); }

extern "C" int64_t lidal_conv_weight_image_job(void* job, const void* w, int role, void* img_fwd,
                                               int64_t n_out_fwd, void* img_bwd, int64_t n_out_bwd,
                                               int dtype, int k, int ci, int co, int64_t first) {
  if (job == nullptr || (dtype != LIDAL_F32 && dtype != LIDAL_BF16 && dtype != LIDAL_F32_SPLIT) || (role != 0 && role != 1)) {
    set_error("weight_image_job: bad arguments");
    return -1;
  }
  if (dtype == LIDAL_F32_SPLIT) {
    if (ci % SPLIT_KCH != 0 || (img_bwd != nullptr && co % SPLIT_KCH != 0)) {
      set_error("weight_image_job(split): the reduction must be a multiple of %d channels (got ci=%d%s co=%d)", SPLIT_KCH, ci,
                img_bwd != nullptr ? ", data-gradient image:" : ",", co);
      return -1;
    }
    ImageJob j;
    j.w = w; j.img_a = img_fwd; j.img_b = img_bwd; j.first = first;
    j.segs_a = split_image_bytes(k, ci, co) / 16;
    j.segs_b = img_bwd != nullptr ? split_image_bytes(k, co, ci) / 16 : 0;
    j.n_red = ci; j.n_col = co; j.role = role; j.nb_a = split_nb(co); j.kc_a = 0; j.nb_b = split_nb(ci); j.kc_b = 0; j.pad = 0;
    if (j.segs_a >= (1ll << 31) || j.segs_b >= (1ll << 31)) {
      set_error("weight_image_job: an image of %lld segments", (long long)(j.segs_a > j.segs_b ? j.segs_a : j.segs_b));
      return -1;
    }
    *reinterpret_cast<ImageJob*>(job) = j;
    return j.segs_a + j.segs_b;
  }
  const int esz = dtype == LIDAL_BF16 ? 2 : 4;
  const Tiling ta = pick_tiling(ci, co, n_out_fwd, esz);
  ImageJob j;
  j.w = w; j.img_a = img_fwd; j.img_b = img_bwd; j.first = first;
  j.segs_a = image_bytes(k, ci, co, ta, esz) / 16;
  j.n_red = ci; j.n_col = co; j.role = role; j.nb_a = ta.nb; j.kc_a = ta.row_bytes / esz;
  j.segs_b = 0; j.nb_b = ta.nb; j.kc_b = j.kc_a; j.pad = 0;
  if (img_bwd != nullptr) {
    const Tiling tb = pick_tiling(co, ci, n_out_bwd, esz);
    j.segs_b = image_bytes(k, co, ci, tb, esz) / 16;
    j.nb_b = tb.nb; j.kc_b = tb.row_bytes / esz;
  }
  if (j.segs_a >= (1ll << 31) || j.segs_b >= (1ll << 31)) {
    set_error("weight_image_job: an image of %lld segments", (long long)(j.segs_a > j.segs_b ? j.segs_a : j.segs_b));
    return -1;
  }
  *reinterpret_cast<ImageJob*>(job) = j;
  return j.segs_a + j.segs_b;
}

extern "C" int lidal_conv_weight_image_batch(const void* jobs, int n_jobs, int64_t total_segments,
                                             int w_dtype, int dtype, void* stream) {
  if (n_jobs == 0 || total_segments == 0) return 0;
  hipStream_t s = (hipStream_t)stream;
  const unsigned grid = (unsigned)cdiv(total_segments, 256);
#define IMG_BATCH(TI, TO) \
  weight_image_batch_kernel<TI, TO><<<grid, 256, 0, s>>>((const ImageJob*)jobs, n_jobs, total_segments)
  if (dtype == LIDAL_F32_SPLIT && w_dtype == LIDAL_F32)
    weight_image_batch_split_kernel<float><<<grid, 256, 0, s>>>((const ImageJob*)jobs, n_jobs, total_segments);
  else if (dtype == LIDAL_F32_SPLIT && w_dtype == LIDAL_BF16)
    weight_image_batch_split_kernel<__bf16><<<grid, 256, 0, s>>>((const ImageJob*)jobs, n_jobs, total_segments);
  else if (w_dtype == LIDAL_F32 && dtype == LIDAL_F32) IMG_BATCH(float, float);
  else if (w_dtype == LIDAL_F32 && dtype == LIDAL_BF16) IMG_BATCH(float, __bf16);
  else if (w_dtype == LIDAL_BF16 && dtype == LIDAL_BF16) IMG_BATCH(__bf16, __bf16);
  else if (w_dtype == LIDAL_BF16 && dtype == LIDAL_F32) IMG_BATCH(__bf16, float);
  else {
    set_error("weight_image_batch: bad dtypes %d %d", w_dtype, dtype);
    return 2;
  }
#undef IMG_BATCH
  LIDAL_CHECK_LAUNCH("lidal_conv_weight_image_batch");
  return 0;
}

static int conv_apply_image(const void* in, const void* wimg, const int32_t* nbr, const int32_t* perm,
                            const uint32_t* tile_masks, void* out, int64_t n_in, int64_t n_out, int ci, int co,
                            int k, int kflip, int dtype, const float* ep_scale, const float* ep_shift,
                            int ep_relu, const void* ep_residual, float* tile_stats, BnBwd bnb, void* ws,
                            int64_t ws_bytes, hipStream_t s) {
  if (n_out == 0 || co == 0) return 0;
  LIDAL_REQUIRE((ep_scale == nullptr) == (ep_shift == nullptr), "conv_apply_image: scale and shift go together");
  LIDAL_REQUIRE(dtype == LIDAL_F32 || dtype == LIDAL_BF16 || dtype == LIDAL_F32_SPLIT, "conv_apply_image: bad dtype %d", dtype);
  if (dtype == LIDAL_F32_SPLIT) {
    LIDAL_REQUIRE(ci > 0 && ci % SPLIT_KCH == 0 && co % 4 == 0 && k > 0 && k <= MAXK,
                  "conv_apply_image(split): ci must be a multiple of %d, co of 4, k <= %d (got ci=%d co=%d k=%d)",
                  SPLIT_KCH, MAXK, ci, co, k);
    LIDAL_REQUIRE(nbr == nullptr ? (k == 1 && n_in == n_out) : (tile_masks != nullptr),
                  "conv_apply_image: needs lidal_kmap_order's tile masks (or NULL table = identity, k = 1)");
    LIDAL_REQUIRE(tile_stats == nullptr && bnb.sums == nullptr, "conv_apply_image(split): no BatchNorm statistics (inference form)");
    const int64_t ib = split_image_bytes(k, ci, co);
    LIDAL_REQUIRE(n_in >= 0 && n_in * ci * 4 < 0x7FFFFFF0ll && ib < 0x7FFFFFF0ll && n_in < (1 << 24),
                  "conv_apply_image: the input matrix and the weight image must each stay below 2 GiB (2^24 rows)");
    LIDAL_REQUIRE((int64_t)k * n_out * 4 < 0x7FFFFFF0ll, "conv_apply_image: neighbour table above 2 GiB");
    Epi ep{ep_scale, ep_shift, ep_relu, ep_residual, (unsigned)(n_in * ci * 4), (unsigned)ib,
           (unsigned)((int64_t)k * n_out * 4), nullptr, bnb, ws, (long long)ws_bytes};
    switch (split_nb(co)) {
      case 2: return launch_split<2>(in, wimg, nbr, perm, tile_masks, out, n_out, ci, co, k, kflip, ep, s);
      case 4: return launch_split<4>(in, wimg, nbr, perm, tile_masks, out, n_out, ci, co, k, kflip, ep, s);
      case 6: return launch_split<6>(in, wimg, nbr, perm, tile_masks, out, n_out, ci, co, k, kflip, ep, s);
      default: return launch_split<8>(in, wimg, nbr, perm, tile_masks, out, n_out, ci, co, k, kflip, ep, s);
    }
  }
  const int esz = dtype == LIDAL_BF16 ? 2 : 4;
  const int vec = 16 / esz;
  LIDAL_REQUIRE(ci > 0 && ci % vec == 0 && co % 4 == 0 && k > 0 && k <= MAXK,
                "conv_apply_image: ci must be a multiple of %d, co of 4, k <= %d (got ci=%d co=%d k=%d)",
                vec, MAXK, ci, co, k);
  LIDAL_REQUIRE(nbr == nullptr ? (k == 1 && n_in == n_out) : (tile_masks != nullptr),
                "conv_apply_image: needs lidal_kmap_order's tile masks (or NULL table = identity, k = 1)");
  LIDAL_REQUIRE(bnb.sums == nullptr || (co % vec == 0 && ep_residual == nullptr && ep_scale == nullptr &&
                                        tile_stats == nullptr && bnb.x && bnb.mean && bnb.invstd),
                "conv_apply_image: BatchNorm backward sums need whole 16-byte column vectors, no other epilogue");
  const Tiling t = pick_tiling(ci, co, n_out, esz);
  const int64_t ib = image_bytes(k, ci, co, t, esz);
  LIDAL_REQUIRE(n_in >= 0 && n_in * ci * esz < 0x7FFFFFF0ll && ib < 0x7FFFFFF0ll,
                "conv_apply_image: the input matrix and the weight image must each stay below 2 GiB");
  LIDAL_REQUIRE((int64_t)k * n_out * 4 < 0x7FFFFFF0ll, "conv_apply_image: neighbour table above 2 GiB");
  Epi ep{ep_scale, ep_shift, ep_relu, ep_residual, (unsigned)(n_in * ci * esz), (unsigned)ib,
         (unsigned)((int64_t)k * n_out * 4), tile_stats, bnb, ws, (long long)ws_bytes};
  if (dtype == LIDAL_F32)
    return dispatch_img<float>(t, in, wimg, nbr, perm, tile_masks, out, n_out, ci, co, k, kflip, ep, s);
  return dispatch_img<__bf16>(t, in, wimg, nbr, perm, tile_masks, out, n_out, ci, co, k, kflip, ep, s);
}

#ifdef LIDAL_PHASE_STAMPS
extern "C" int lidal_debug_phase_stamps(void* buf) {
  LIDAL_HIP(hipMemcpyToSymbol(HIP_SYMBOL(g_stamp_buf), &buf, sizeof(buf)));
  return 0;
}
#endif

extern "C" int lidal_conv_apply_image(const void* in, const void* wimg, const int32_t* nbr,
                                      const int32_t* perm, const uint32_t* tile_masks, void* out,
                                      int64_t n_in, int64_t n_out, int ci, int co, int k, int kflip,
                                      int dtype, const float* ep_scale, const float* ep_shift,
                                      int ep_relu, const void* ep_residual, float* tile_stats,
                                      void* stream) {
  BnBwd none{nullptr, nullptr, nullptr, nullptr, nullptr, nullptr, 0};
  return conv_apply_image(in, wimg, nbr, perm, tile_masks, out, n_in, n_out, ci, co, k, kflip, dtype, ep_scale,
                          ep_shift, ep_relu, ep_residual, tile_stats, none, nullptr, 0, (hipStream_t)stream);
}

extern "C" int64_t lidal_conv_apply_workspace_bytes(int64_t n_out, int co) {
  const int64_t tiles = cdiv(n_out > 0 ? n_out : 1, TILE_ROWS);
  if (tiles * cdiv(co, 128) > SPLIT_F32_MAX_WGS) return 0;
  return 4 * tiles * TILE_ROWS * align_up(co, 128) * 4;
}

extern "C" int lidal_conv_apply_image_ws(const void* in, const void* wimg, const int32_t* nbr,
                                         const int32_t* perm, const uint32_t* tile_masks, void* out,
                                         int64_t n_in, int64_t n_out, int ci, int co, int k, int kflip,
                                         int dtype, const float* ep_scale, const float* ep_shift,
                                         int ep_relu, const void* ep_residual, float* tile_stats, void* ws,
                                         int64_t ws_bytes, void* stream) {
  BnBwd none{nullptr, nullptr, nullptr, nullptr, nullptr, nullptr, 0};
  return conv_apply_image(in, wimg, nbr, perm, tile_masks, out, n_in, n_out, ci, co, k, kflip, dtype, ep_scale,
                          ep_shift, ep_relu, ep_residual, tile_stats, none, ws, ws_bytes, (hipStream_t)stream);
}

extern "C" int lidal_conv_dgrad_bn_sums(const void* gout, const void* wimg, const int32_t* nbr,
                                        const int32_t* perm, const uint32_t* tile_masks, void* gin,
                                        int64_t n_gout, int64_t n_gin, int c_gout, int c_gin, int k, int kflip,
                                        int dtype, const void* bn_x, const float* bn_mean,
                                        const float* bn_invstd, const float* bn_gamma, const float* bn_beta,
                                        int bn_relu, float* bn_sums, void* stream) {
  BnBwd b{bn_x, bn_mean, bn_invstd, bn_gamma, bn_beta, bn_sums, bn_relu};
  return conv_apply_image(gout, wimg, nbr, perm, tile_masks, gin, n_gout, n_gin, c_gout, c_gin, k, kflip, dtype,
                          nullptr, nullptr, 0, nullptr, nullptr, b, nullptr, 0, (hipStream_t)stream);
}

extern "C" int lidal_conv_dgrad_bn_sums_ws(const void* gout, const void* wimg, const int32_t* nbr,
                                           const int32_t* perm, const uint32_t* tile_masks, void* gin,
                                           int64_t n_gout, int64_t n_gin, int c_gout, int c_gin, int k, int kflip,
                                           int dtype, const void* bn_x, const float* bn_mean,
                                           const float* bn_invstd, const float* bn_gamma, const float* bn_beta,
                                           int bn_relu, float* bn_sums, void* ws, int64_t ws_bytes, void* stream) {
  BnBwd b{bn_x, bn_mean, bn_invstd, bn_gamma, bn_beta, bn_sums, bn_relu};
  return conv_apply_image(gout, wimg, nbr, perm, tile_masks, gin, n_gout, n_gin, c_gout, c_gin, k, kflip, dtype,
                          nullptr, nullptr, 0, nullptr, nullptr, b, ws, ws_bytes, (hipStream_t)stream);
}
```

lidal_amd/csrc/plan.hip:

```cpp
#include <string.h>
#include <mutex>

#include "common.h"

using namespace lidal;

namespace {

typedef __attribute__((ext_vector_type(8))) __bf16 bf16x8_t;

template <typename U>
__global__ void __launch_bounds__(256) copy2d_kernel(const U* __restrict__ src, int64_t src_pitch,
                                                     U* __restrict__ dst, int64_t dst_pitch, int64_t rows,
                                                     int row_units, int zero_units) {
  const int per = row_units + zero_units;
  const int64_t total = rows * per;
  const int64_t stride = (int64_t)gridDim.x * 256;
  for (int64_t i = (int64_t)blockIdx.x * 256 + threadIdx.x; i < total; i += stride) {
    const int64_t r = i / per;
    const int u = (int)(i - r * per);
    U v;
    if (u < row_units) v = src[r * src_pitch + u];
    else memset(&v, 0, sizeof(U));
    dst[r * dst_pitch + u] = v;
// ... 132 lines not shown
  if (n == 0) return 0;
  cast_rows_kernel<<<grid_for(n * c_dst), 256, 0, (hipStream_t)stream>>>(src, c_src, (__bf16*)dst, c_dst, n);
  LIDAL_CHECK_LAUNCH("lidal_cast_rows_bf16");
  return 0;
}

extern "C" int lidal_debug_read(const void* dev, void* host, int64_t nbytes) {
  LIDAL_REQUIRE(dev != nullptr && host != nullptr && nbytes >= 0, "debug_read: bad arguments");
  LIDAL_HIP(hipDeviceSynchronize());
  LIDAL_HIP(hipMemcpy(host, dev, (size_t)nbytes, hipMemcpyDeviceToHost));
  return 0;
}

namespace {

struct OpInfo { int n_args; const char* name; };

const OpInfo kOps[] = {
     {-1, "(none)"},
     {5, "conv_weight_image_batch"},
     {18, "conv_apply_image"},
     {20, "conv_dgrad_bn_sums"},
     {14, "conv_wgrad"},
     {18, "bn_train_fwd"},
     {18, "bn_train_fwd_tiles"},
     {16, "bn_bwd"},
     {16, "bn_bwd_tiles"},
     {11, "bn_eval_fwd"},
     {8, "bn_fold"},
     {7, "colsum"},
     {5, "add_relu_fwd"},
     {5, "add_relu_bwd"},
     {6, "voxelize_fwd_1to1"},
     {11, "voxelize_fwd_sorted"},
     {9, "voxelize_bwd"},
     {8, "devoxelize_fwd"},
     {11, "devoxelize_bwd_sorted"},
     {9, "ce_fwd"},
     {9, "ce_bwd"},
     {7, "copy2d"},
     {9, "add2d"},
     {5, "transpose_f32"},
     {5, "cast_rows_bf16"},
     {7, "view_mean_softmax"},
     {0, "fork_side"},
     {0, "join_side"},
     {20, "conv_apply_image_ws"},
     {22, "conv_dgrad_bn_sums_ws"},
     {15, "add_relu_bwd_bn_sums"},
     {16, "bn_bwd_from_sums"},
     {15, "add_relu_bwd_bn_tile_sums"},
     {12, "devoxelize_bwd_cells"},
     {15, "conv_wgrad_streams"},
};
constexpr int kNumOps = (int)(sizeof(kOps) / sizeof(kOps[0]));

inline double as_double(int64_t w) {
  double d;
  memcpy(&d, &w, sizeof(d));
  return d;
}

constexpr int MAX_SIDE = 8;
hipEvent_t g_fork_ev[MAX_DEVICES][MAX_SIDE], g_join_ev[MAX_DEVICES][MAX_SIDE];
bool g_ev_ready[MAX_DEVICES][MAX_SIDE];
std::mutex g_ev_mutex[MAX_DEVICES];

int stream_edge(int idx, bool join, hipStream_t from, hipStream_t to) {
  const int d = current_device();
  std::lock_guard<std::mutex> lock(g_ev_mutex[d]);
  if (!g_ev_ready[d][idx]) {
    LIDAL_HIP(hipEventCreateWithFlags(&g_fork_ev[d][idx], hipEventDisableTiming));
    LIDAL_HIP(hipEventCreateWithFlags(&g_join_ev[d][idx], hipEventDisableTiming));
    g_ev_ready[d][idx] = true;
  }
  hipEvent_t ev = join ? g_join_ev[d][idx] : g_fork_ev[d][idx];
  LIDAL_HIP(hipEventRecord(ev, from));
  LIDAL_HIP(hipStreamWaitEvent(to, ev, 0));
  return 0;
}

}

extern "C" int lidal_plan_op_args(int kind) { return kind > 0 && kind < kNumOps ? kOps[kind].n_args : -1; }

extern "C" int lidal_plan_run(const int64_t* words, int64_t n_words, int64_t n_ops, void* stream, void* side_stream) {
  void* streams[2] = {stream, side_stream};
  return lidal_plan_run_streams(words, n_words, n_ops, streams, side_stream != nullptr ? 2 : 1);
}

namespace {
int run_ops(const int64_t* words, int64_t n_words, int64_t n_ops, void* const* streams, int n_streams, bool* side_open);
}

extern "C" int lidal_plan_run_streams(const int64_t* words, int64_t n_words, int64_t n_ops, void* const* streams,
                                      int n_streams) {
  LIDAL_REQUIRE(streams != nullptr && n_streams >= 1 && n_streams <= MAX_SIDE, "plan_run: 1..%d streams", MAX_SIDE);
  if (int rc = lidal_bn_check_device()) return rc;
  bool side_open[MAX_SIDE] = {};
  const int rc = run_ops(words, n_words, n_ops, streams, n_streams, side_open);
  if (rc != 0) {
    char msg[400];
    snprintf(msg, sizeof(msg), "%s", lidal_last_error());
    for (int i = 1; i < n_streams; ++i)
      if (side_open[i] && streams[i] != nullptr) stream_edge(i, true, (hipStream_t)streams[i], (hipStream_t)streams[0]);
    set_error("%s", msg);
  }
  return rc;
}

namespace {
int run_ops(const int64_t* words, int64_t n_words, int64_t n_ops, void* const* streams, int n_streams, bool* side_open) {
  void* const stream = streams[0];
#define P(i) ((void*)(uintptr_t)a[i])
#define CP(T, i) ((const T*)(uintptr_t)a[i])
#define MP(T, i) ((T*)(uintptr_t)a[i])
#define I(i) ((int)a[i])
#define L(i) ((int64_t)a[i])
#define F(i) ((float)as_double(a[i]))
  int64_t pos = 0;
  for (int64_t op = 0; op < n_ops; ++op) {
    LIDAL_REQUIRE(pos < n_words, "plan_run: op %lld starts past the end of the stream (%lld words)", (long long)op,
                  (long long)n_words);
    const int kind = (int)(words[pos] & 0xFFFF);
    const int flags = (int)((words[pos] >> 16) & 0xFFFF);
    LIDAL_REQUIRE(kind > 0 && kind < kNumOps, "plan_run: op %lld has unknown kind %d", (long long)op, kind);
    const int na = kOps[kind].n_args;
    LIDAL_REQUIRE(pos + 1 + na <= n_words, "plan_run: op %lld (%s) is truncated", (long long)op, kOps[kind].name);
    const int64_t* a = words + pos + 1;
    pos += 1 + na;
    void* st = stream;
    const int sidx = flags & 0xF;
    if (sidx != 0 && kind != LIDAL_OP_FORK_SIDE && kind != LIDAL_OP_JOIN_SIDE) {
      LIDAL_REQUIRE(sidx < n_streams && streams[sidx] != nullptr && side_open[sidx], "plan_run: op %lld (%s) wants side "
                    "stream %d outside a fork / join bracket", (long long)op, kOps[kind].name, sidx);
      st = streams[sidx];
    }
    int rc = 0;
    switch (kind) {
      case LIDAL_OP_CONV_WEIGHT_IMAGE_BATCH:
        rc = lidal_conv_weight_image_batch(P(0), I(1), L(2), I(3), I(4), st);
        break;
      case LIDAL_OP_CONV_APPLY_IMAGE:
        rc = lidal_conv_apply_image(P(0), P(1), CP(int32_t, 2), CP(int32_t, 3), CP(uint32_t, 4), P(5), L(6), L(7), I(8),
                                    I(9), I(10), I(11), I(12), CP(float, 13), CP(float, 14), I(15), P(16),
                                    MP(float, 17), st);
        break;
      case LIDAL_OP_CONV_DGRAD_BN_SUMS:
        rc = lidal_conv_dgrad_bn_sums(P(0), P(1), CP(int32_t, 2), CP(int32_t, 3), CP(uint32_t, 4), P(5), L(6), L(7),
                                      I(8), I(9), I(10), I(11), I(12), P(13), CP(float, 14), CP(float, 15),
                                      CP(float, 16), CP(float, 17), I(18), MP(float, 19), st);
        break;
      case LIDAL_OP_CONV_APPLY_IMAGE_WS:
        rc = lidal_conv_apply_image_ws(P(0), P(1), CP(int32_t, 2), CP(int32_t, 3), CP(uint32_t, 4), P(5), L(6), L(7),
                                       I(8), I(9), I(10), I(11), I(12), CP(float, 13), CP(float, 14), I(15), P(16),
                                       MP(float, 17), P(18), L(19), st);
        break;
      case LIDAL_OP_CONV_DGRAD_BN_SUMS_WS:
        rc = lidal_conv_dgrad_bn_sums_ws(P(0), P(1), CP(int32_t, 2), CP(int32_t, 3), CP(uint32_t, 4), P(5), L(6), L(7),
                                         I(8), I(9), I(10), I(11), I(12), P(13), CP(float, 14), CP(float, 15),
                                         CP(float, 16), CP(float, 17), I(18), MP(float, 19), P(20), L(21), st);
        break;
      case LIDAL_OP_CONV_WGRAD:
        rc = lidal_conv_wgrad(P(0), P(1), L(2), L(3), CP(int32_t, 4), CP(int64_t, 5), I(6), MP(float, 7), MP(float, 8),
                              L(9), I(10), I(11), I(12), I(13), st);
        break;
      case LIDAL_OP_CONV_WGRAD_STREAMS:
        rc = lidal_conv_wgrad_streams(P(0), P(1), L(2), L(3), CP(int32_t, 4), CP(int32_t, 5), I(6), I(7), MP(float, 8),
                                      MP(float, 9), L(10), I(11), I(12), I(13), I(14), st);
        break;
      case LIDAL_OP_BN_TRAIN_FWD:
        rc = lidal_bn_train_fwd(P(0), I(1), L(2), I(3), CP(float, 4), CP(float, 5), F(6), F(7), MP(float, 8),
                                MP(float, 9), MP(int64_t, 10), I(11), P(12), P(13), MP(float, 14), MP(float, 15), P(16),
                                L(17), st);
        break;
      case LIDAL_OP_BN_TRAIN_FWD_TILES:
        rc = lidal_bn_train_fwd_tiles(P(0), I(1), L(2), I(3), CP(float, 4), CP(float, 5), F(6), F(7), MP(float, 8),
                                      MP(float, 9), MP(int64_t, 10), I(11), P(12), P(13), MP(float, 14), MP(float, 15),
                                      CP(float, 16), L(17), st);
        break;
      case LIDAL_OP_BN_BWD:
        rc = lidal_bn_bwd(P(0), P(1), L(2), I(3), L(4), I(5), CP(float, 6), CP(float, 7), I(8), CP(float, 9),
                          CP(float, 10), P(11), MP(float, 12), MP(float, 13), P(14), L(15), st);
        break;
      case LIDAL_OP_BN_BWD_FROM_SUMS:
        rc = lidal_bn_bwd_from_sums(P(0), P(1), L(2), I(3), L(4), I(5), CP(float, 6), CP(float, 7), I(8), CP(float, 9),
                                    CP(float, 10), P(11), MP(float, 12), MP(float, 13), P(14), L(15), st);
        break;
      case LIDAL_OP_ADD_RELU_BWD_BN_SUMS:
        rc = lidal_add_relu_bwd_bn_sums(P(0), P(1), P(2), I(3), L(4), I(5), P(6), CP(float, 7), CP(float, 8), P(9), P(10),
                                        CP(float, 11), CP(float, 12), P(13), L(14), st);
        break;
      case LIDAL_OP_ADD_RELU_BWD_BN_TILE_SUMS:
        rc = lidal_add_relu_bwd_bn_tile_sums(P(0), P(1), P(2), I(3), L(4), I(5), P(6), CP(float, 7), CP(float, 8),
                                             MP(float, 9), P(10), CP(float, 11), CP(float, 12), MP(float, 13), L(14), st);
        break;
      case LIDAL_OP_BN_BWD_TILES:
        rc = lidal_bn_bwd_tiles(P(0), P(1), L(2), I(3), L(4), I(5), CP(float, 6), CP(float, 7), I(8), CP(float, 9),
                                CP(float, 10), P(11), MP(float, 12), MP(float, 13), CP(float, 14), L(15), st);
        break;
      case LIDAL_OP_BN_EVAL_FWD:
        rc = lidal_bn_eval_fwd(P(0), I(1), L(2), I(3), CP(float, 4), CP(float, 5), CP(float, 6), CP(float, 7), F(8),
                               I(9), P(10), st);
        break;
      case LIDAL_OP_BN_FOLD:
        rc = lidal_bn_fold(CP(float, 0), CP(float, 1), CP(float, 2), CP(float, 3), F(4), I(5), MP(float, 6),
                           MP(float, 7), st);
        break;
      case LIDAL_OP_COLSUM:
        rc = lidal_colsum(P(0), I(1), L(2), I(3), MP(float, 4), P(5), L(6), st);
        break;
      case LIDAL_OP_ADD_RELU_FWD:
        rc = lidal_add_relu_fwd(P(0), P(1), P(2), L(3), I(4), st);
        break;
      case LIDAL_OP_ADD_RELU_BWD:
        rc = lidal_add_relu_bwd(P(0), P(1), P(2), L(3), I(4), st);
        break;
      case LIDAL_OP_VOXELIZE_FWD_1TO1:
        rc = lidal_voxelize_fwd_1to1(P(0), CP(int32_t, 1), P(2), L(3), I(4), I(5), st);
        break;
      case LIDAL_OP_VOXELIZE_FWD_SORTED:
        rc = lidal_voxelize_fwd_sorted(P(0), CP(int32_t, 1), CP(int64_t, 2), CP(int32_t, 3), P(4), L(5), I(6), I(7),
                                       L(8), P(9), L(10), st);
        break;
      case LIDAL_OP_VOXELIZE_BWD:
        rc = lidal_voxelize_bwd(P(0), CP(int32_t, 1), CP(int32_t, 2), P(3), P(4), L(5), L(6), I(7), I(8), st);
        break;
      case LIDAL_OP_DEVOXELIZE_FWD:
        rc = lidal_devoxelize_fwd(P(0), CP(int32_t, 1), CP(float, 2), P(3), L(4), L(5), I(6), I(7), st);
        break;
      case LIDAL_OP_DEVOXELIZE_BWD_SORTED:
        rc = lidal_devoxelize_bwd_sorted(P(0), CP(int32_t, 1), CP(int64_t, 2), CP(float, 3), P(4), L(5), I(6), I(7),
                                         L(8), P(9), L(10), st);
        break;
      case LIDAL_OP_DEVOXELIZE_BWD_CELLS:
        rc = lidal_devoxelize_bwd_cells(P(0), CP(int32_t, 1), CP(int64_t, 2), CP(float, 3), CP(int32_t, 4), CP(int64_t, 5),
                                        P(6), L(7), I(8), I(9), P(10), L(11), st);
        break;
      case LIDAL_OP_CE_FWD:
        rc = lidal_ce_fwd(P(0), I(1), CP(int64_t, 2), L(3), I(4), L(5), MP(float, 6), P(7), L(8), st);
        break;
      case LIDAL_OP_CE_BWD:
        rc = lidal_ce_bwd(P(0), I(1), CP(int64_t, 2), L(3), I(4), L(5), CP(float, 6), CP(float, 7), P(8), st);
        break;
      case LIDAL_OP_COPY2D:
        rc = lidal_copy2d(P(0), L(1), P(2), L(3), L(4), L(5), L(6), st);
        break;
      case LIDAL_OP_ADD2D:
        rc = lidal_add2d(P(0), L(1), P(2), L(3), P(4), L(5), L(6), I(7), I(8), st);
        break;
      case LIDAL_OP_TRANSPOSE_F32:
        rc = lidal_transpose_f32(CP(float, 0), L(1), MP(float, 2), I(3), I(4), st);
        break;
      case LIDAL_OP_CAST_ROWS_BF16:
        rc = lidal_cast_rows_bf16(CP(float, 0), I(1), P(2), I(3), L(4), st);
        break;
      case LIDAL_OP_VIEW_MEAN_SOFTMAX:
        rc = lidal_view_mean_softmax(CP(float, 0), CP(int64_t, 1), I(2), L(3), I(4), MP(float, 5), MP(int64_t, 6), st);
        break;
      case LIDAL_OP_FORK_SIDE: {
        const int i = sidx ? sidx : 1;
        LIDAL_REQUIRE(i < n_streams && streams[i] != nullptr, "plan_run: op %lld forks to side stream %d, which was not "
                      "given", (long long)op, i);
        if (stream_edge(i, false, (hipStream_t)stream, (hipStream_t)streams[i])) return 1;
        side_open[i] = true;
        break;
      }
      case LIDAL_OP_JOIN_SIDE: {
        const int i = sidx ? sidx : 1;
        LIDAL_REQUIRE(i < n_streams && streams[i] != nullptr, "plan_run: op %lld joins side stream %d, which was not "
                      "given", (long long)op, i);
        if (stream_edge(i, true, (hipStream_t)streams[i], (hipStream_t)stream)) return 1;
        side_open[i] = false;
        break;
      }
      default:
        set_error("plan_run: op %lld: kind %d not handled", (long long)op, kind);
        return 2;
    }
    if (rc != 0) {
      char msg[400];
      snprintf(msg, sizeof(msg), "%s", lidal_last_error());
      set_error("plan_run: op %lld (%s): %s", (long long)op, kOps[kind].name, msg);
      return rc;
    }
  }
  LIDAL_REQUIRE(pos == n_words, "plan_run: %lld ops used %lld of %lld words", (long long)n_ops, (long long)pos,
                (long long)n_words);
  return 0;
#undef P
#undef CP
#undef MP
#undef I
#undef L
#undef F
}
}
```

lidal_amd/network/blocks.py:

```python
import torch
from torch import nn

from .. import SparseTensor
from .. import backend as B
from .. import nn as spnn
from ..nn.functional.conv import conv3d
from ..nn.functional.dense import rows_linear
from ..nn.functional.fused import add_relu
from ..utils import make_ntuple


import os as _os

from ..nn.functional import conv as _C
from ..nn.functional import dense as _D
from ..nn.functional import norm as _N

FUSE_BLOCKS = _os.environ.get('LIDAL_FUSE_BLOCKS', '1') != '0'
BN_SUMS = _os.environ.get('LIDAL_BN_SUMS', '1') != '0'


def _bn_args(bn):
    return (bn.weight, bn.bias, bn.running_mean, bn.running_var, bn.momentum, bn.eps)


def _bn_ok(bn, feats):
    return (bn.training and bn.track_running_stats and bn.momentum is not None and bn.weight is not None
            and bn.bias is not None and bn.weight.dtype == torch.float32 and feats.is_cuda)


class _ConvNormAct(torch.autograd.Function):

    @staticmethod
    def forward(ctx, feats, kernel, gamma, beta, kmap, transposed, bn, relu, stats):
        need_gx = ctx.needs_input_grad[0]
        xc, x1, ctx.img_bwd = _C._forward(feats, kernel, kmap, transposed, None, need_gx, stats)
        y, mean, invstd, x1, w, b = _N.train_forward(x1, gamma, beta, bn.running_mean, bn.running_var, bn.momentum,
                                                     bn.eps, relu, bn.num_batches_tracked,
                                                     getattr(x1, '_lidal_bn_stats', None))
        ctx.kmap, ctx.transposed, ctx.relu = kmap, transposed, relu
        ctx.save_for_backward(xc, kernel, x1, w, b, mean, invstd)
        return y

    @staticmethod
    def backward(ctx, g):
        B.note_backward()
        xc, kernel, x1, w, b, mean, invstd = ctx.saved_tensors
        dx, gg, gb, _ = _N.train_backward(x1, w, b, mean, invstd, ctx.relu, g, True)
        gx, gk = _C.conv_backward(xc, kernel, ctx.kmap, ctx.transposed, ctx.img_bwd, dx, None,
                                  ctx.needs_input_grad[0], ctx.needs_input_grad[1])
        return gx, gk, gg, gb, None, None, None, None, None


class _Residual(torch.autograd.Function):

    @staticmethod
    def forward(ctx, feats, k1, g1, b1, k2, g2, b2, ks, gs, bs, kmap, bn1, bn2, bns, stats):
        need_gx = ctx.needs_input_grad[0]
        xc, x1, ctx.img1 = _C._forward(feats, k1, kmap, False, None, need_gx, stats[0])
        y1, mean1, inv1, x1, w1, c1 = _N.train_forward(x1, g1, b1, bn1.running_mean, bn1.running_var, bn1.momentum,
                                                       bn1.eps, True, bn1.num_batches_tracked,
                                                       getattr(x1, '_lidal_bn_stats', None))
        _, x2, ctx.img2 = _C._forward(y1, k2, kmap, False, None, True, stats[1])
        ctx.shortcut = ks is not None
        if ctx.shortcut:
            xs_in, ctx.wcs, ctx.pads, xs, ctx.imgs = _D._forward(feats, ks, None, False, None, need_gx, stats[2])
            res, means, invs, xs, ws, cs = _N.train_forward(xs, gs, bs, bns.running_mean, bns.running_var,
                                                            bns.momentum, bns.eps, False, bns.num_batches_tracked,
                                                            getattr(xs, '_lidal_bn_stats', None))
        else:
            res = feats
        out, mean2, inv2, x2, w2, c2 = _N.train_forward(x2, g2, b2, bn2.running_mean, bn2.running_var, bn2.momentum,
                                                        bn2.eps, False, bn2.num_batches_tracked,
                                                        getattr(x2, '_lidal_bn_stats', None), res, True)
        ctx.kmap = kmap
        saved = [xc, k1, x1, w1, c1, mean1, inv1, y1, k2, x2, w2, c2, mean2, inv2, out]
        if ctx.shortcut:
            saved += [xs_in, ks, xs, ws, cs, means, invs]
        ctx.save_for_backward(*saved)
        return out

    @staticmethod
    def backward(ctx, g):
        B.note_backward()
        t = ctx.saved_tensors
        xc, k1, x1, w1, c1, mean1, inv1, y1, k2, x2, w2, c2, mean2, inv2, out = t[:15]
        need_gx = ctx.needs_input_grad[0]
        gks = ggs = gbs = None
        if ctx.shortcut:
            xs_in, ks, xs, ws, cs, means, invs = t[15:]
            gm, (dx2, gg2, gb2), (dxs, ggs, gbs) = _N.tail_backward(g, out, x2, w2, c2, mean2, inv2, (xs, ws, cs, means, invs))
            g_skip, gks, _ = _D.rows_backward(xs_in, ks, ctx.wcs, ctx.imgs, ctx.pads, False, dxs, need_gx,
                                              ctx.needs_input_grad[7], False)
        else:
            gm, (dx2, gg2, gb2), _ = _N.tail_backward(g, out, x2, w2, c2, mean2, inv2)
            g_skip = gm
        dy1, gk2 = _C.conv_backward(y1, k2, ctx.kmap, False, ctx.img2, dx2, None, True, ctx.needs_input_grad[4],
                                    (x1, mean1, inv1, w1, c1, True) if BN_SUMS else None)
        dx1, gg1, gb1, _ = _N.train_backward(x1, w1, c1, mean1, inv1, True, dy1, True, None,
                                             getattr(dy1, '_lidal_bnb_sums', None))
        gx, gk1 = _C.conv_backward(xc, k1, ctx.kmap, False, ctx.img1, dx1, g_skip if need_gx else None, need_gx,
                                   ctx.needs_input_grad[1])
        return gx, gk1, gg1, gb1, gk2, gg2, gb2, gks, ggs, gbs, None, None, None, None, None


def _kmap_of(x, conv):
    from ..nn.functional.conv import build_kernel_map
    if conv.transposed:
        ts = tuple(x.stride[k] // conv.stride[k] for k in range(3))
        return x.kmaps[(ts, conv.kernel_size, conv.stride, (1, 1, 1))], x.cmaps[ts], ts
    key = (x.stride, conv.kernel_size, conv.stride, (1, 1, 1))
    out_stride = tuple(x.stride[k] * conv.stride[k] for k in range(3))
    kmap = x.kmaps.get(key)
    if kmap is None:
        kmap, out_coords = build_kernel_map(x.coords, x.stride, conv.kernel_size, conv.stride, x.cmaps)
        x.kmaps[key] = kmap
        if any(s > 1 for s in conv.stride):
            x.cmaps.setdefault(out_stride, out_coords)
    out_coords = x.coords if all(s == 1 for s in conv.stride) else x.cmaps[out_stride]
    return kmap, out_coords, out_stride


def _wrap(feats, coords, stride, like):
    out = SparseTensor(feats, coords, stride)
    out.cmaps, out.kmaps = like.cmaps, like.kmaps
    out.cmaps.setdefault(out.stride, out.coords)
    return out


def _plain_conv(conv):
    d = conv.dilation
    return (conv.bias is None and conv.kernel_size != (1, 1, 1) and (d == 1 or tuple(make_ntuple(d, 3)) == (1, 1, 1)))


def fused_conv_norm_act(x, conv, bn):
    if not (FUSE_BLOCKS and _plain_conv(conv) and _bn_ok(bn, x.F) and B.wants_grad(x.F, conv.kernel, bn.weight)
            and isinstance(bn, spnn.BatchNorm)):
        return None
    kmap, coords, stride = _kmap_of(x, conv)
    y = _ConvNormAct.apply(x.F, conv.kernel, bn.weight, bn.bias, kmap, conv.transposed, bn, bool(bn.fused_relu),
                           bool(conv.bn_follows))
    return _wrap(y, coords, stride, x)


class ConvNormSequential(nn.Sequential):

    def forward(self, x, residual=None, relu_after=False, start=0):
        mods = list(self)
        while mods and isinstance(mods[-1], nn.Identity):
            mods.pop()
        i = start
        while i < len(mods):
            m = mods[i]
            nxt = mods[i + 1] if i + 1 < len(mods) else None
            if (FUSE_BLOCKS and isinstance(m, spnn.Conv3d) and isinstance(nxt, spnn.BatchNorm) and nxt.training
                    and nxt.fused_relu and not torch.is_tensor(x)
                    and not (i + 2 == len(mods) and residual is not None)):
                y = fused_conv_norm_act(x, m, nxt)
                if y is not None:
                    x = y
                    i += 2
                    continue
            if isinstance(m, spnn.Conv3d) and isinstance(nxt, spnn.BatchNorm) and _fusable(m, nxt, x):
                last = i + 2 == len(mods) and residual is not None
                x = _conv_norm(m, nxt, x, residual if last else None, relu_after)
                if last:
                    residual = None
                i += 2
            elif (isinstance(m, spnn.Linear) and isinstance(nxt, spnn.BatchNorm1d)
                  and torch.is_tensor(x) and _fusable_rows(nxt, x, m.weight, m.bias)):
                scale, shift = _fold(nxt, x.device)
                last = i + 2 == len(mods)
                relu = int(nxt.fused_relu) | (2 if (last and relu_after and residual is not None) else 0)
                x = rows_linear(x, m.weight, m.bias,
                                epilogue=(scale, shift, relu, residual if last else None))
                if last:
                    residual = None
                i += 2
            elif (isinstance(m, spnn.BatchNorm1d) and not isinstance(m, spnn.BatchNorm) and torch.is_tensor(x)
                  and i + 1 == len(mods) and residual is not None and not relu_after and m.training
                  and (B.FORK & 4)):
                x = m(x, residual=residual)
                residual = None
                i += 1
            elif (isinstance(m, spnn.BatchNorm) and not torch.is_tensor(x) and i + 1 == len(mods)
                  and residual is not None and relu_after and m.training and (B.FORK & 8)):
                x = m(x, residual=residual, relu_after=True)
                residual = None
                i += 1
            else:
                x = m(x)
                i += 1
        if residual is None:
            return x
        if torch.is_tensor(x):
            return add_relu(x, residual) if relu_after else residual + x
        out = SparseTensor(add_relu(x.F, residual) if relu_after else x.F + residual, x.C, x.s)
        out.cmaps, out.kmaps = x.cmaps, x.kmaps
        return out


def _fusable_rows(bn, feats, *params):
    return (not bn.training and bn.track_running_stats and feats.is_cuda
            and not B.wants_grad(feats, bn.weight, bn.bias, *params)
            and bn.weight is not None and bn.weight.dtype == torch.float32)


def _fusable(conv, bn, x):
    return conv.bias is None and _fusable_rows(bn, x.F, conv.kernel)


def _fold(bn, device):
    key = (B.weights_key(bn.weight), B.weights_key(bn.bias), B.weights_key(bn.running_mean),
           B.weights_key(bn.running_var), str(device))
    cached = getattr(bn, '_lidal_fold', None)
    if cached is not None and cached[0] == key:
        return cached[1], cached[2]
    c = bn.num_features
    fold = torch.empty((2, c), dtype=torch.float32, device=device)
    B.check(B.lib().lidal_bn_fold(B.ptr(bn.weight), B.ptr(bn.bias), B.ptr(bn.running_mean),
                                  B.ptr(bn.running_var), float(bn.eps), c, B.ptr(fold[0]),
                                  B.ptr(fold[1]), B.stream()), 'bn_fold')
    object.__setattr__(bn, '_lidal_fold', (key, fold[0], fold[1]))
    return fold[0], fold[1]


def _conv_norm(conv, bn, x, residual=None, relu_after=False):
    scale, shift = _fold(bn, x.F.device)
    relu = int(bn.fused_relu) | (2 if (relu_after and residual is not None) else 0)
    return conv3d(x, conv.kernel, kernel_size=conv.kernel_size, bias=None, stride=conv.stride,
                  dilation=conv.dilation, transposed=conv.transposed,
                  epilogue=(scale, shift, relu, residual))


def _conv_bn(inc, outc, ks, stride=1, transposed=False):
    conv = spnn.Conv3d(inc, outc, kernel_size=ks, stride=stride, dilation=1, transposed=transposed)
    conv.bn_follows = True
    return [conv, spnn.BatchNorm(outc)]


def conv_bn_relu(inc, outc, ks, stride=1, transposed=False):
    conv, bn = _conv_bn(inc, outc, ks, stride, transposed)
    bn.fused_relu = True
    return [conv, bn, nn.Identity()]


class BasicConvolutionBlock(nn.Module):

    def __init__(self, inc, outc, ks=3, stride=1, dilation=1):
        super().__init__()
        self.net = ConvNormSequential(*conv_bn_relu(inc, outc, ks, stride))

    def forward(self, x):
        return self.net(x)


class BasicDeconvolutionBlock(nn.Module):

    def __init__(self, inc, outc, ks=3, stride=1):
        super().__init__()
        self.net = ConvNormSequential(*conv_bn_relu(inc, outc, ks, stride, transposed=True))

    def forward(self, x):
        return self.net(x)


class ResidualBlock(nn.Module):

    def __init__(self, inc, outc, ks=3, stride=1, dilation=1):
        super().__init__()
        self.net = ConvNormSequential(*conv_bn_relu(inc, outc, ks, stride), *_conv_bn(outc, outc, ks, 1))
        if inc == outc and stride == 1:
            self.downsample = nn.Identity()
        else:
            self.downsample = ConvNormSequential(*_conv_bn(inc, outc, 1, stride))
        self.relu = spnn.ReLU(True)

    def _fused(self, x):
        net = self.net
        c1, n1, c2, n2 = net[0], net[1], net[3], net[4]
        if not (FUSE_BLOCKS and B.wants_grad(x.F, c1.kernel) and _plain_conv(c1) and _plain_conv(c2)
                and not c1.transposed and not c2.transposed and c1.stride == (1, 1, 1) and c2.stride == (1, 1, 1)
                and _bn_ok(n1, x.F) and _bn_ok(n2, x.F) and n1.fused_relu and not n2.fused_relu):
            return None
        ks = gs = bs = ns = None
        if not isinstance(self.downsample, nn.Identity):
            cs, ns = self.downsample[0], self.downsample[1]
            if not (cs.kernel_size == (1, 1, 1) and cs.stride == (1, 1, 1) and cs.bias is None and _bn_ok(ns, x.F)
                    and not ns.fused_relu):
                return None
            ks, gs, bs = cs.kernel, ns.weight, ns.bias
        elif x.F.shape[1] != c2.out_channels:
            return None
        kmap, coords, stride = _kmap_of(x, c1)
        stats = (bool(c1.bn_follows), bool(c2.bn_follows), bool(ks is not None and self.downsample[0].bn_follows))
        out = _Residual.apply(x.F, c1.kernel, n1.weight, n1.bias, c2.kernel, n2.weight, n2.bias, ks, gs, bs, kmap,
                              n1, n2, ns, stats)
        return _wrap(out, coords, stride, x)

    def forward(self, x):
        y = self._fused(x)
        if y is not None:
            return y
        first = self.net[0]
        if ((B.FORK & 1) and B.wants_grad(x.F) and x.F.requires_grad and first.bias is None
                and first.kernel_size != (1, 1, 1) and not first.transposed):
            y, x_skip = self.net[0](x, fork=True)
            b = self.downsample(x_skip)
            return self.net(y, residual=b.F, relu_after=True, start=1)
        b = self.downsample(x)
        return self.net(x, residual=b.F, relu_after=True)
```

lidal_amd/network/plan.py:

```python
import array
import ctypes
import os
import struct

import torch

from .. import backend as B
from ..nn.functional import conv as _C
from ..nn.functional import norm as _N
from ..nn.functional import devoxelize as _DV
from ..nn.functional.invlist import inverse_lists
from ..nn.functional.voxelize import _index32

__all__ = ['planned_forward', 'enabled', 'COUNTERS']

ENABLED = os.environ.get('LIDAL_PLAN', '1') != '0'
BN_SUMS = None

OP_CONV_WEIGHT_IMAGE_BATCH, OP_CONV_APPLY_IMAGE, OP_CONV_DGRAD_BN_SUMS, OP_CONV_WGRAD = 1, 2, 3, 4
OP_BN_TRAIN_FWD, OP_BN_TRAIN_FWD_TILES, OP_BN_BWD, OP_BN_BWD_TILES, OP_BN_EVAL_FWD, OP_BN_FOLD = 5, 6, 7, 8, 9, 10
OP_COLSUM, OP_ADD_RELU_FWD, OP_ADD_RELU_BWD, OP_VOXELIZE_FWD_1TO1, OP_VOXELIZE_FWD_SORTED = 11, 12, 13, 14, 15
OP_VOXELIZE_BWD, OP_DEVOXELIZE_FWD, OP_DEVOXELIZE_BWD_SORTED, OP_CE_FWD, OP_CE_BWD = 16, 17, 18, 19, 20
OP_COPY2D, OP_ADD2D, OP_TRANSPOSE_F32, OP_CAST_ROWS_BF16, OP_VIEW_MEAN_SOFTMAX = 21, 22, 23, 24, 25
OP_FORK_SIDE, OP_JOIN_SIDE, OP_CONV_APPLY_IMAGE_WS, OP_CONV_DGRAD_BN_SUMS_WS = 26, 27, 28, 29
OP_ADD_RELU_BWD_BN_SUMS, OP_BN_BWD_FROM_SUMS, OP_ADD_RELU_BWD_BN_TILE_SUMS, OP_DEVOXELIZE_BWD_CELLS = 30, 31, 32, 33
OP_CONV_WGRAD_STREAMS = 34

COUNTERS = {'ops': 0, 'plans': 0}
TALLY = os.environ.get('LIDAL_PLAN_TALLY', '0') != '0'
TRACE = None
SIDE_ROWS = int(os.environ.get('LIDAL_PLAN_SIDE_ROWS', str(1 << 40)))
SIDE_F32 = os.environ.get('LIDAL_PLAN_SIDE_F32', '0') == '1'
BRANCH_ROWS = int(os.environ.get('LIDAL_PLAN_BRANCH_ROWS', '100000'))
POINT_SIDE = int(os.environ.get('LIDAL_PLAN_POINT_SIDE', '1'))
F32_BN_ALONE = os.environ.get('LIDAL_PLAN_F32_BN_ALONE', '1') != '0'
_NARGS = {}
_HIT_NAMES = {1: 'conv_weight_image', 2: 'conv_apply', 3: 'conv_apply', 4: 'conv_wgrad', 5: 'bn_train_fwd',
              6: 'bn_train_fwd', 7: 'bn_bwd', 8: 'bn_bwd', 9: 'bn_eval_fwd', 10: 'bn_fold', 11: 'colsum',
              12: 'add_relu_fwd', 13: 'add_relu_bwd', 14: 'voxelize_fwd_1to1', 15: 'voxelize_fwd_sorted',
              16: 'voxelize_bwd', 17: 'devoxelize_fwd', 18: 'devoxelize_bwd_sorted', 19: 'ce_fwd', 20: 'ce_bwd',
              21: 'copy2d', 22: 'add2d', 23: 'transpose_f32', 24: 'cast_rows_bf16', 25: 'view_mean_softmax',
              26: 'fork_side', 27: 'join_side', 28: 'conv_apply', 29: 'conv_apply', 30: 'add_relu_bwd', 31: 'bn_bwd',
              32: 'add_relu_bwd', 33: 'devoxelize_bwd_cells', 34: 'conv_wgrad_streams'}


def _tally(words):
    if not _NARGS:
        L = B.lib_handle()
        for k in _HIT_NAMES:
            _NARGS[k] = int(L.lidal_plan_op_args(k))
    i, n = 0, len(words)
    while i < n:
        kind = words[i] & 0xFFFF
        name = _HIT_NAMES[kind]
        if kind in (OP_CONV_APPLY_IMAGE, OP_CONV_APPLY_IMAGE_WS) and words[i + 3] == 0:
            name = 'conv_apply(dense)'
        elif kind == OP_CONV_WGRAD and words[i + 5] == 0:
            name = 'conv_wgrad(dense)'
        elif kind == OP_BN_BWD_TILES:
            B.hit('bn_bwd(tile sums)')
        B.hit(name)
        i += 1 + _NARGS[kind]


def enabled():
    return ENABLED


def _dbits(x):
    return struct.unpack('<q', struct.pack('<d', float(x)))[0]


class _Arena:
    BLOCK = int(os.environ.get('LIDAL_PLAN_BLOCK_MB', '1024')) << 20

    def __init__(self, device):
        self.device = device
        self.blocks = []
        self.cur = self.end = 0

    def alloc(self, nbytes):
        nbytes = (nbytes + 255) & -256
        if nbytes > (self.BLOCK >> 2):
            size = (nbytes + (64 << 20) - 1) & -(64 << 20)
            t = torch.empty(size, dtype=torch.uint8, device=self.device)
            a = t.data_ptr()
            self.blocks.append((a, size, t))
            return a
        a = self.cur
        if a + nbytes > self.end:
            t = torch.empty(self.BLOCK, dtype=torch.uint8, device=self.device)
            a = t.data_ptr()
            self.blocks.append((a, self.BLOCK, t))
            self.end = a + self.BLOCK
        self.cur = a + nbytes
        return a

    def tensor(self, addr, shape, dtype):
        numel = 1
        for s in shape:
            numel *= s
        nbytes = numel * torch.empty((), dtype=dtype).element_size()
        for a, size, t in self.blocks:
            if a <= addr and addr + nbytes <= a + size:
                return t[addr - a:addr - a + nbytes].view(dtype).view(*shape)
        raise RuntimeError('lidal_amd.plan: address outside the arena')

    def release(self):
        self.blocks = []
        self.cur = self.end = 0


_SCRATCH = {}


def _scratch(device, stream, nbytes, keep):
    key = (device.index, stream)
    s = _SCRATCH.get(key)
    if s is None or s[2] < nbytes:
        if s is not None:
            keep.append(s[0])
        size = max(32 << 20, (int(nbytes * 1.25) + (1 << 20)) & -(1 << 20))
        t = torch.empty(size, dtype=torch.uint8, device=device)
        s = _SCRATCH[key] = [t, t.data_ptr(), size]
    return s[1]


class _Conv:
    __slots__ = ('w', 'k', 'ci', 'co', 'transposed', 'strided', 'shape', 'role', 'pad_in', 'img_f', 'img_b', 'tkey',
                 'param', 'ptrs')


class _BN:
    __slots__ = ('w', 'b', 'rm', 'rv', 'nbt', 'c', 'eps', 'mom', 'relu', 'mod', 'scale', 'shift')


class _Lin:
    __slots__ = ('conv', 'b', 'ci', 'co', 'co_pad', 'bias')


class _Res:
    __slots__ = ('c1', 'b1', 'c2', 'b2', 'cs', 'bs')


class _Program:

    def __init__(self, model):
        from . import blocks
        from .unet import SPVCNN
        from .. import nn as spnn
        self.kind = type(model).__name__
        self.spvcnn = isinstance(model, SPVCNN)
        self.params = list(model.parameters())
        self.where = [(m, k, p) for m in model.modules() for k, p in m._parameters.items() if p is not None]
        self.where_buf = []
        self.index = {id(p): i for i, p in enumerate(self.params)}
        assert len(self.index) == len(self.params), 'shared parameters are not planned'
        self.buffers = []
        self.used = set()
        self.convs = []
        self.bns = []

        def conv(m, pad_in=0):
            c = _Conv()
            c.param = m.kernel
            c.w = self._p(m.kernel)
            c.k, c.ci, c.co = m.kernel_volume, m.in_channels, m.out_channels
            c.transposed = bool(m.transposed)
            c.strided = any(s > 1 for s in m.stride)
            c.shape = (c.k, c.ci, c.co)
            c.role = 0
            c.pad_in = pad_in
            c.img_f = c.img_b = 0
            c.tkey = None
            c.ptrs = {}
            assert m.bias is None and m.bn_follows
            self.convs.append(c)
            return c

# ... 162 lines not shown
        return None
    f = x.F
    if not (torch.is_tensor(f) and f.is_cuda and f.dtype == torch.float32 and f.dim() == 2 and f.shape[1] == 4
            and f.is_contiguous() and not f.requires_grad and f.shape[0] > 1 and tuple(x.s) == (1, 1, 1)):
        return None
    if torch.is_autocast_enabled() and torch.get_autocast_dtype('cuda') != torch.bfloat16:
        return None
    return mode if _program(model, mode == 'train') is not None else None


_WS_BN = {}
_WS_SLABS = {}
_WS_SEG = {}


def _bn_ws(n, c):
    key = (n, c)
    v = _WS_BN.get(key)
    if v is None:
        if len(_WS_BN) > 4096:
            _WS_BN.clear()
        v = _WS_BN[key] = int(B.lib_handle().lidal_bn_workspace_bytes(n, c))
    return v


def _slabs(n_a, n_b, k, ca, cb, dtype):
    key = (n_a, n_b, k, ca, cb, dtype, B.SPLIT_F32_TRAIN, B.SPLIT_F32)
    v = _WS_SLABS.get(key)
    if v is None:
        if len(_WS_SLABS) > 4096:
            _WS_SLABS.clear()
        v = _WS_SLABS[key] = _C.wgrad_plan(n_a, n_b, k, ca, cb, dtype)
    return v


_WS_STREAM = {}


def _stream_serves(n, k, ca, cb):
    key = (n, k, ca, cb)
    v = _WS_STREAM.get(key)
    if v is None:
        if len(_WS_STREAM) > 4096:
            _WS_STREAM.clear()
        v = _WS_STREAM[key] = bool(B.lib_handle().lidal_conv_wgrad_streams_serves(n, n, k, ca, cb))
    return v


def _seg_ws(n_entries, m, c):
    key = (n_entries, m, c)
    v = _WS_SEG.get(key)
    if v is None:
        if len(_WS_SEG) > 4096:
            _WS_SEG.clear()
        v = _WS_SEG[key] = int(B.lib_handle().lidal_segment_workspace_bytes(n_entries, m, c))
    return v


class _Tables:

    def __init__(self, g, spvcnn, train, model_cs=None):
        x0 = g.x0
        km, cm = x0.kmaps, x0.cmaps
        self.n = []
        self.k3 = []
        self.k2 = []
        self.keep = []
        for l in range(5):
            s = 1 << l
            st = (s, s, s)
            self.n.append(int(cm[st].shape[0]))
            k3 = km[(st, (3, 3, 3), (1, 1, 1), (1, 1, 1))]
            oo = k3.order_out
            st3 = k3._streams if (train and k3._streams is not None) else None
            self.k3.append((oo.table.data_ptr(), oo.perm.data_ptr(), oo.tile_masks.data_ptr(),
                            k3._nbmaps_cap.data_ptr() if train else 0, k3.koff.data_ptr() if train else 0,
                            st3[0].data_ptr() if st3 else 0, st3[1].data_ptr() if st3 else 0, st3[2] if st3 else 0))
            self.keep.append(k3)
            if l < 4:
                k2 = km[(st, (2, 2, 2), (2, 2, 2), (1, 1, 1))]
                oo, oi = k2.order_out, k2.order_in
                self.k2.append((oo.table.data_ptr(), oo.perm.data_ptr(), oo.tile_masks.data_ptr(),
                                oi.table.data_ptr(), oi.perm.data_ptr(), oi.tile_masks.data_ptr(),
                                k2._nbmaps_cap.data_ptr() if train else 0, k2.koff.data_ptr() if train else 0))
                self.keep.append(k2)
        self.pt = {}
        self.p = 0
        if spvcnn:
            z = g.z
            af = z.additional_features
            self.p = int(z.C.shape[0])
            for l, key in ((0, 1), (4, (16, 16, 16)), (2, (4, 4, 4))):
                if l == 0 and af['idx_query'].get((1, 1, 1)) is not None:
                    key_v = (1, 1, 1)
                else:
                    key_v = key
                idx64, counts = af['idx_query'][key_v], af['counts'][key_v]
                m = self.n[l]
                idx32 = _index32(idx64)
                one = bool(getattr(idx64, '_lidal_one_to_one', False)) and idx64.numel() == m
                vorder = vseg = 0
                if not one:
                    o, sp = inverse_lists(idx32, m)
                    vorder, vseg = o.data_ptr(), sp.data_ptr()
                    self.keep += [o, sp]
                s = 1 << l
                idx8, w8 = z.idx_query[(s, s, s)], z.weights[(s, s, s)]
                assert idx8.dtype == torch.int32 and idx8.is_contiguous() and w8.dtype == torch.float32
                pc = {0: model_cs[8], 4: model_cs[4], 2: model_cs[6]}[l]
                cells = None
                do = dsp = idx8
                if train and _DV.cells_mode(idx8, self.p, m, pc):
                    if getattr(idx8, '_lidal_cell_index', None) is None:
                        idx8._lidal_cell_index = idx32
                    cells = _DV.devox_cells(idx8, m)
                elif train:
                    do, dsp = inverse_lists(idx8, m, w8)
                cnt = counts if counts.dtype == torch.int32 and counts.is_contiguous() else counts.contiguous().int()
                self.keep += [idx32, cnt, idx8, w8, do, dsp, cells]
                self.pt[l] = (idx32.data_ptr(), cnt.data_ptr(), int(one), vorder, vseg,
                              idx8.data_ptr(), w8.data_ptr(), do.data_ptr(), dsp.data_ptr(),
                              tuple(t.data_ptr() for t in cells) if cells is not None else None)


def _tables(g, spvcnn, train, model_cs=None):
    key = '_plan_tables_train' if train else '_plan_tables'
    t = g.__dict__.get(key) or (g.__dict__.get('_plan_tables_train') if not train else None)
    if t is None:
        t = g.__dict__[key] = _Tables(g, spvcnn, train, model_cs)
    return t


class _Run:
    TRAIN = True

    def __init__(self, model, prog, geometry, feats, code):
        self.prog = prog
        self.model = model
        self.dev = feats.device
        self.code = code
        self.esz = 2 if code == B.BF16 else 4
        self.vec = 8 if code == B.BF16 else 4
        self.bf16 = code == B.BF16
        self.dtype = torch.bfloat16 if self.bf16 else torch.float32
        self.geometry = geometry
        self.T = _tables(geometry, prog.spvcnn, self.TRAIN, getattr(model, 'cs', None))
        self.feats = feats
        self.stream = B.stream()
        self.arena = _Arena(self.dev)
        self.barena = None
        self.tile = B.stats_tile_rows()
        from . import blocks
        self.bn_sums = (blocks.BN_SUMS if BN_SUMS is None else BN_SUMS) and self.bf16
        self.saved = {}
        self.noise = []
        self.keep = []
        self.tapes = [] if TRACE is not None else None
        self.sides = {}
        self.open = set()
        self.w = []
        self.nops = 0
        self.done = False
        self.ptr = [t.data_ptr() for t in prog.tensors]
        self._constants()
        self._images()

    def _constants(self):
        prog, T = self.prog, self.T
        if prog.ones is None or prog.ones.device != self.dev:
            prog.ones = torch.ones(512, dtype=torch.float32, device=self.dev)
            prog.cls_shift = torch.zeros(64, dtype=torch.float32, device=self.dev)
        self.ones = prog.ones.data_ptr()
        self.cls_shift = prog.cls_shift.data_ptr()
        ns = [T.p] + T.n if prog.spvcnn else T.n
        host = []
        for n in ns:
            host += [0, n]
        k = torch.tensor(host, dtype=torch.int64).to(self.dev, non_blocking=True)
        self.koff_t = k
        base = k.data_ptr()
        self.koff = {n: base + 16 * i for i, n in reversed(list(enumerate(ns)))}

    def ccode(self, c):
        if c.k > 1 and not c.role:
            return B.conv_code(self.dtype, c.ci, False, c.co)
        return self.code

    def _images(self):
        prog, T = self.prog, self.T
        bank = _C._IMAGE_BANK
        code, dtype = self.code, self.dtype
        seen = []
        for c, (nf, nb) in self._conv_rows():
            code = self.ccode(c)
            key = (_C._tiling(c.ci, c.co, code, nf), _C._tiling(c.co, c.ci, code, nb), code)
            e = c.tkey.get(key) if c.tkey else None
            if e is None or e['ref']() is not c.param or bank.entries.get((id(c.param), e['key'])) is not e:
                bank.get(c.param, dtype, nf, nb, c.shape if (c.role or c.k == 1) else None, c.role, code)
                e = bank.entry(c.param, key)
                if c.tkey is None or len(c.tkey) > 8:
                    c.tkey = {}
                c.tkey[key] = e
                c.ptrs = {}
            p = c.ptrs.get(key)
            if p is None:
                p = c.ptrs[key] = (e['img_f'].data_ptr(), e['img_b'].data_ptr())
            c.img_f, c.img_b = p
            e['used'] = bank.tick
            seen.append((e, c.param))
        for e, w in seen:
            if e['version'] != B.weights_key(w):
                bank._rebuild(e['group'])

    def _conv_rows(self):
        prog, n = self.prog, self.T.n
        out = []
        for cb in prog.stem:
            out.append((cb[0], (n[0], n[0])))
        for l, (down, ra, rb) in enumerate(prog.stages):
            out.append((down[0], (n[l + 1], n[l])))
            for r in (ra, rb):
                for c in (r.c1, r.c2, r.cs):
                    if c is not None:
                        out.append((c, (n[l + 1], n[l + 1])))
        for i, (dec, ra, rb) in enumerate(prog.ups):
            l = 3 - i
            out.append((dec[0], (n[l], n[l + 1])))
            for r in (ra, rb):
                for c in (r.c1, r.c2, r.cs):
                    if c is not None:
                        out.append((c, (n[l], n[l])))
        rows = self.T.p if prog.spvcnn else n[0]
        out.append((prog.classifier.conv, (rows, rows)))
        for lin, _ in prog.points:
            out.append((lin.conv, (self.T.p, self.T.p)))
        return out

    def flush(self):
        if not self.nops:
            return
        for which in sorted(self.open):
            self.join(which)
        if TALLY:
            _tally(self.w)
        if self.tapes is not None:
            self.tapes.append(('bwd' if self.barena is not None else 'fwd', list(self.w)))
        arr = array.array('q', self.w)
        addr, n_words = arr.buffer_info()
        L = B.lib_handle()
        if self.sides:
            n = max(self.sides) + 1
            streams = (ctypes.c_void_p * n)(*([self.stream] + [self.sides.get(i) for i in range(1, n)]))
            rc = L.lidal_plan_run_streams(addr, n_words, self.nops, streams, n)
        else:
            rc = L.lidal_plan_run(addr, n_words, self.nops, self.stream, None)
        COUNTERS['plans'] += 1
        COUNTERS['ops'] += self.nops
        B.HITS['plan_run'] = B.HITS.get('plan_run', 0) + 1
        self.w = []
        self.nops = 0
        if rc != 0:
            raise RuntimeError('lidal_amd.plan_run failed (%d): %s' % (rc, L.lidal_last_error().decode()))

    def scratch(self, nbytes, flag=0):
        return _scratch(self.dev, (self.stream, flag) if flag else self.stream, nbytes, self.keep)

    def fork(self, which):
        if which not in self.sides:
            self.sides[which] = B.side_stream(self.dev, which).cuda_stream
        self.w.append(OP_FORK_SIDE | (which << 16))
        self.nops += 1
        self.open.add(which)
        return which << 16

    def join(self, which):
        self.w.append(OP_JOIN_SIDE | (which << 16))
        self.nops += 1
        self.open.discard(which)

    def _bn_alone(self):
        if self.open and F32_BN_ALONE and not self.bf16:
            for w_ in sorted(self.open):
                self.join(w_)

    def side(self, rows):
        if not SIDE_ROWS or rows > SIDE_ROWS:
            return 0
        if not self.bf16 and (not SIDE_F32 or _N.TAIL_SUMS_ROWS > 0):
            return 0
        return self.fork(1)

    def f_conv(self, c, x, n_in, ci, table, n_out, stats):
        A = self.arena
        out = A.alloc(n_out * c.co * self.esz)
        st = A.alloc(-(-n_out // self.tile) * c.co * 12) if (stats and self.bf16) else 0
        wb = _C.apply_workspace_bytes(n_out, c.co)
        self.w += (OP_CONV_APPLY_IMAGE_WS, x, c.img_f, table[0], table[1], table[2], out, n_in, n_out, ci, c.co, c.k, 0,
                   self.ccode(c), 0, 0, 0, 0, st, self.scratch(wb) if wb else 0, wb)
        self.nops += 1
        return out, st

    def f_dense(self, c, x, n, co, shift, stats, flag=0):
        A = self.arena
        out = A.alloc(n * co * self.esz)
        st = A.alloc(-(-n // self.tile) * co * 12) if (stats and self.bf16) else 0
        self.w += (OP_CONV_APPLY_IMAGE | flag, x, c.img_f, 0, 0, 0, out, n, n, c.ci, co, 1, 0, self.ccode(c),
# ... 83 lines not shown
    def f_point(self, pt, z_in, devox_out, pre=None):
        lin, r = pt
        P = self.T.p
        x1, st = pre if pre is not None else self.f_dense(lin.conv, z_in, P, lin.co, self.ptr[lin.b], True)
        self.point_join()
        y, mean, invstd = self.f_bn(r, x1, P, st, devox_out, False)
        self.saved[id(pt)] = (z_in, x1, mean, invstd)
        return y

    def f_classifier(self, x, n):
        lin = self.prog.classifier
        co_pad = lin.co + (-lin.co) % self.vec
        self.w += (OP_COPY2D, self.ptr[lin.b], lin.co * 4, self.cls_shift, co_pad * 4, 1, lin.co * 4, 0)
        self.nops += 1
        out, _ = self.f_dense(lin.conv, x, n, co_pad, self.cls_shift, False)
        self.saved['cls'] = (x, n, co_pad)
        return out, co_pad

    def f_dropout(self, addr, n, c):
        d = self.prog.dropout
        if d is None or not d.training or d.p == 0:
            self.noise.append(None)
            return
        self.flush()
        x = self.arena.tensor(addr, (n, c), self.dtype)
        if d.p == 1:
            x.zero_()
            self.noise.append(0)
            return
        noise = torch.empty_like(x).bernoulli_(1 - d.p).div_(1 - d.p)
        x.mul_(noise)
        self.noise.append(noise)

    def forward(self):
        prog, T, A = self.prog, self.T, self.arena
        n = T.n
        k3, k2 = T.k3, T.k2
        bf = self.bf16
        x = self.feats.data_ptr()
        if prog.spvcnn:
            x = self.f_vox(x, 0, 4, B.F32)
        c0 = prog.stem[0][0]
        if bf:
            xc = A.alloc(n[0] * 8 * 2)
            self.w += (OP_CAST_ROWS_BF16, x, 4, xc, 8, n[0])
            self.nops += 1
            x, ci0 = xc, 8
        else:
            ci0 = 4
        y = self.f_conv_bn(prog.stem[0], x, n[0], k3[0], n[0], ci0)
        x0 = self.f_conv_bn(prog.stem[1], y, n[0], k3[0], n[0])
        skips = [x0]
        cs = [c0.co]
        if prog.spvcnn:
            z0 = self.f_devox(x0, 0, cs[0])
            pre = self.f_point_lin(prog.points[0], z0) if self.TRAIN else None
            y = self.f_vox(z0, 0, cs[0])
        else:
            y = x0
        for l, (down, ra, rb) in enumerate(prog.stages):
            y = self.f_conv_bn(down, y, n[l], k2[l][0:3], n[l + 1])
            y = self.f_res(ra, y, n[l + 1], k3[l + 1])
            y = self.f_res(rb, y, n[l + 1], k3[l + 1])
            skips.append(y)
            cs.append(rb.c2.co)
        z = None
        if prog.spvcnn:
            z1 = self.f_point(prog.points[0], z0, self.f_devox(y, 4, cs[4]), pre)
            pre = self.f_point_lin(prog.points[1], z1) if self.TRAIN else None
            y = self.f_vox(z1, 4, cs[4])
            self.f_dropout(y, n[4], cs[4])
            z = z1
        for i, (dec, ra, rb) in enumerate(prog.ups):
            l = 3 - i
            y = self.f_conv_bn(dec, y, n[l + 1], k2[l][3:6], n[l])
            y = self.f_cat(y, dec[0].co, skips[l], cs[l], n[l])
            y = self.f_res(ra, y, n[l], k3[l])
            y = self.f_res(rb, y, n[l], k3[l])
            c_out = rb.c2.co
            if prog.spvcnn and i == 1:
                z2 = self.f_point(prog.points[1], z, self.f_devox(y, 2, c_out), pre)
                pre = self.f_point_lin(prog.points[2], z2) if self.TRAIN else None
                y = self.f_vox(z2, 2, c_out)
                self.f_dropout(y, n[2], c_out)
                z = z2
        if prog.spvcnn:
            feat = self.f_point(prog.points[2], z, self.f_devox(y, 0, c_out), pre)
            rows = T.p
        else:
            feat, rows = y, n[0]
        logits, co_pad = self.f_classifier(feat, rows)
        self.flush()
        if self.TRAIN:
            torch.autograd.graph.increment_version(prog.running)
        self.c_feat = c_out
        logits_t = A.tensor(logits, (rows, co_pad), self.dtype)[:, :prog.n_class]
        feat_t = A.tensor(feat, (rows, c_out), self.dtype)
        return logits_t, feat_t

    def galloc(self, nbytes):
        return self.barena.alloc(nbytes)

    def slot(self, i):
        return self.flat + 4 * self.prog.slot[i]

    def b_bn(self, r, x, n, mean, invstd, g, g_stride, sums=0, relu=None, flag=0, part=None, nparts=0):
        p = self.ptr
        c = r.c
        if not flag:
            self._bn_alone()
        dx = self.galloc(n * c * self.esz)
        relu = r.relu if relu is None else relu
        if part is not None and part[0]:
            self.w += (OP_BN_BWD_FROM_SUMS | flag, x, g, g_stride, self.code, n, c, p[r.w], p[r.b], relu, mean, invstd, dx,
                       self.slot(r.w), self.slot(r.b), part[0], part[1])
        elif sums:
            self.w += (OP_BN_BWD_TILES | flag, x, g, g_stride, self.code, n, c, p[r.w], p[r.b], relu, mean, invstd, dx,
                       self.slot(r.w), self.slot(r.b), sums, nparts or -(-n // self.tile))
        else:
            nb = _bn_ws(n, c)
            self.w += (OP_BN_BWD | flag, x, g, g_stride, self.code, n, c, p[r.w], p[r.b], relu, mean, invstd, dx,
                       self.slot(r.w), self.slot(r.b), self.scratch(nb, flag), nb)
        self.nops += 1
        return dx

    def b_wgrad(self, c, x, n_x, g, n_g, rules, ci=None):
        ci = c.ci if ci is None else ci
        wcode, slabs = _slabs(n_x, n_g, c.k, ci, c.co, self.dtype)
        flag = self.side(max(n_x, n_g))
        streams = (len(rules) >= 5 and rules[2] and wcode == B.BF16 and not c.transposed and n_x == n_g
                   and _stream_serves(n_x, c.k, ci, c.co))
        if streams:
            slabs = 2 * rules[4]
        nbytes = slabs * ci * c.co * 4 + (c.k * ci * c.co * 4 if ci != c.ci else 0)
        partial = self.scratch(nbytes, flag)
        gw = self.slot(c.w)
        if ci != c.ci:
            gw = partial + slabs * ci * c.co * 4
        if streams:
            self.w += (OP_CONV_WGRAD_STREAMS | flag, x, g, n_x, n_g, rules[2], rules[3], rules[4], 0, gw, partial, slabs,
                       c.k, ci, c.co, wcode)
        else:
            self.w += (OP_CONV_WGRAD | flag, x, g, n_x, n_g, rules[0], rules[1], 1 if c.transposed else 0, gw, partial, slabs,
                       c.k, ci, c.co, wcode)
        self.nops += 1
        if ci != c.ci:
            self.w += (OP_COPY2D | flag, gw, ci * c.co * 4, self.slot(c.w), c.ci * c.co * 4, c.k, c.ci * c.co * 4, 0)
            self.nops += 1

    def b_dgrad(self, c, g, n_g, table, n_out, kflip, skip=0, bnb=None):
        gin = self.galloc(n_out * c.ci * self.esz)
        wb = _C.apply_workspace_bytes(n_out, c.ci)
        ws = self.scratch(wb) if wb else 0
        if bnb is not None:
            sums = self.galloc(-(-n_out // self.tile) * c.ci * 8)
            self.w += (OP_CONV_DGRAD_BN_SUMS_WS, g, c.img_b, table[0], table[1], table[2], gin, n_g, n_out, c.co, c.ci,
                       c.k, kflip, self.code) + bnb + (sums, ws, wb)
            self.nops += 1
            return gin, sums
        self.w += (OP_CONV_APPLY_IMAGE_WS, g, c.img_b, table[0], table[1], table[2], gin, n_g, n_out, c.co, c.ci, c.k,
                   kflip, self.ccode(c), 0, 0, 0, skip, 0, ws, wb)
        self.nops += 1
        return gin, 0

    def b_dense(self, c, x, n, g, cg, need_gx=True, linear_slot=None, branch=0):
        ca, cb = c.ci, cg
        wcode, slabs = _slabs(n, n, 1, ca, cb, self.dtype)
        direct = linear_slot is None and cb == c.co
        flag = branch or self.side(n)
        nbytes = slabs * ca * cb * 4 + (0 if direct else ca * cb * 4)
        sc = self.scratch(nbytes, flag)
        gw = self.slot(c.w) if direct else sc + slabs * ca * cb * 4
        self.w += (OP_CONV_WGRAD | flag, x, g, n, n, 0, self.koff[n], 0, gw, sc, slabs, 1, ca, cb, wcode)
        self.nops += 1
        if not direct:
            self.w += (OP_TRANSPOSE_F32 | flag, gw, cb, self.slot(c.w), ca, c.co)
            self.nops += 1
        if not need_gx:
            return 0
        gx = self.galloc(n * ca * self.esz)
        self.w += (OP_CONV_APPLY_IMAGE | branch, g, c.img_b, 0, 0, 0, gx, n, n, cb, ca, 1, 0, self.code, 0, 0, 0, 0, 0)
        self.nops += 1
        return gx

    def b_colsum(self, g, n, c, out, flag=0):
        nb = _bn_ws(n, c) + 12 * c
        self.w += (OP_COLSUM | flag, g, self.code, n, c, out, self.scratch(nb, flag), nb)
        self.nops += 1

    def b_conv_bn(self, cb, g, g_stride, n_in, n_out, tables, need_gx=True, ci=None):
        c, r = cb
        x, x1, mean, invstd = self.saved[id(cb)]
        dx = self.b_bn(r, x1, n_out, mean, invstd, g, g_stride)
        if c.transposed:
            rules, table, n_gin, kflip = tables[6:8], tables[0:3], n_in, 0
        elif c.strided:
            rules, table, n_gin, kflip = tables[6:8], tables[3:6], n_in, 0
        else:
            rules, table, n_gin, kflip = tables[3:8], tables[0:3], n_in, 1
        self.b_wgrad(c, x, n_in, dx, n_out, rules, ci)
        if not need_gx:
            return 0
        return self.b_dgrad(c, dx, n_out, table, n_gin, kflip)[0]

    def b_res(self, r, g, n, k3):
        x, x1, mean1, inv1, y1, x2, mean2, inv2, out, xs, means, invs = self.saved[id(r)]
        co = r.c2.co
        gm = self.galloc(n * co * self.esz)
        part2 = parts = nb = 0
        sums2 = sumss = nparts = 0
        if _N.tail_tiles(n, self.dtype):
            nparts = int(B.lib().lidal_bn_tail_parts(n, co, self.code))
            sums2 = self.galloc(co * nparts * 8)
            sumss = self.galloc(co * nparts * 8) if r.cs is not None else 0
            self.w += (OP_ADD_RELU_BWD_BN_TILE_SUMS, out, g, gm, self.code, n, co, x2, mean2, inv2, sums2,
                       xs if sumss else 0, means if sumss else 0, invs if sumss else 0, sumss, nparts)
        elif _N.tail_sums(n):
            nb = _bn_ws(n, co)
            part2 = self.galloc(nb)
            parts = self.galloc(nb) if r.cs is not None else 0
            self.w += (OP_ADD_RELU_BWD_BN_SUMS, out, g, gm, self.code, n, co, x2, mean2, inv2, part2,
                       xs if parts else 0, means if parts else 0, invs if parts else 0, parts, nb)
        else:
            self.w += (OP_ADD_RELU_BWD, out, g, gm, n * co, self.code)
        self.nops += 1
        fl = 0
        if r.cs is not None:
            fl = self.fork(2) if (BRANCH_ROWS and n >= BRANCH_ROWS and (self.bf16 or not F32_BN_ALONE)) else 0
            dxs = self.b_bn(r.bs, xs, n, means, invs, gm, co, sumss, None, flag=fl, part=(parts, nb), nparts=nparts)
            g_skip = self.b_dense(r.cs, x, n, dxs, co, branch=fl)
        else:
            g_skip = gm
        dx2 = self.b_bn(r.b2, x2, n, mean2, inv2, gm, co, sums2, 0, part=(part2, nb), nparts=nparts)
        table, rules = k3[0:3], k3[3:8]
        self.b_wgrad(r.c2, y1, n, dx2, n, rules)
        p = self.ptr
        bnb = (x1, mean1, inv1, p[r.b1.w], p[r.b1.b], 1) if self.bn_sums else None
        dy1, sums = self.b_dgrad(r.c2, dx2, n, table, n, 1, 0, bnb)
        dx1 = self.b_bn(r.b1, x1, n, mean1, inv1, dy1, r.c1.co, sums)
        self.b_wgrad(r.c1, x, n, dx1, n, rules)
        if fl:
            self.join(2)
        return self.b_dgrad(r.c1, dx1, n, table, n, 1, g_skip)[0]

    def b_add(self, a, a_stride, b, b_stride, n, c):
        out = self.galloc(n * c * self.esz)
        self.w += (OP_ADD2D, a, a_stride, b, b_stride, out, c, n, c, self.code)
        self.nops += 1
        return out

    def b_devox(self, g, lvl, c):
        t = self.T.pt[lvl]
        P, m = self.T.p, self.T.n[lvl]
        gin = self.galloc(m * c * self.esz)
        if t[9] is not None:
            nb = m * 8 * c * 4
            self.w += (OP_DEVOXELIZE_BWD_CELLS, g, t[9][0], t[9][1], t[6], t[9][2], t[9][3], gin, m, c, self.code,
                       self.scratch(nb), nb)
            self.nops += 1
            return gin
        nb = _seg_ws(8 * P, m, c)
        self.w += (OP_DEVOXELIZE_BWD_SORTED, g, t[7], t[8], t[6], gin, m, c, self.code, 8 * P,
                   self.scratch(nb) if nb else 0, nb)
        self.nops += 1
        return gin

    def b_vox(self, g, lvl, c, skip):
        t = self.T.pt[lvl]
        P, m = self.T.p, self.T.n[lvl]
        gin = self.galloc(P * c * self.esz)
        self.w += (OP_VOXELIZE_BWD, g, t[0], t[1], skip, gin, P, m, c, self.code)
        self.nops += 1
        return gin

    def b_point(self, pt, g, need_gx=True, flag=0):
        lin, r = pt
        P = self.T.p
        z_in, x1, mean, invstd = self.saved[id(pt)]
        dx = self.b_bn(r, x1, P, mean, invstd, g, lin.co, flag=flag)
        gx = self.b_dense(lin.conv, z_in, P, dx, lin.co, need_gx, True, branch=flag)
        self.b_colsum(dx, P, lin.co, self.slot(lin.b), flag)
        return gx

    def point_fork(self):
        return self.fork(POINT_SIDE) if (POINT_SIDE and self.bf16) else 0

    def point_join(self):
        if POINT_SIDE and POINT_SIDE in self.open:
            self.join(POINT_SIDE)

    def b_dropout(self, which, g, n, c):
        noise = self.noise[which]
        if noise is None:
            return g
        self.flush()
        gt = self.barena.tensor(g, (n, c), self.dtype)
        if isinstance(noise, int):
            gt.zero_()
        else:
            torch.mul(gt, noise, out=gt)
        return g

    def backward(self, g_logits, g_feat):
        if self.done:
            raise RuntimeError('lidal_amd.plan: this step has already run its backward pass (its activations are '
                               'released; retain_graph is not supported by the planned step)')
        if not self.geometry.alive():
            raise RuntimeError('lidal_amd: this backward pass reads the coordinate tables of a geometry that is stale -- two '
                               'newer ones have been submitted to its prefetcher since (queue forward AND backward of a '
                               'batch before the second submit() after its own: network/geometry.py GeometryPrefetcher)')
        prog, T = self.prog, self.T
        n, k3, k2 = T.n, T.k3, T.k2
        e = self.esz
        self.stream = B.stream()
        self.barena = _Arena(self.dev)
        flat = torch.empty(prog.flat_numel + 16, dtype=torch.float32, device=self.dev)
        self.flat = flat.data_ptr()
        assert self.flat % 16 == 0
        lin = prog.classifier
        x, rows, co_pad = self.saved['cls']
        g = g_logits
        if g.dtype != self.dtype or not g.is_contiguous():
            g = g.contiguous().to(self.dtype)
        gp = self.galloc(rows * co_pad * e)
        self.w += (OP_COPY2D, g.data_ptr(), lin.co * e, gp, co_pad * e, rows, lin.co * e, (co_pad - lin.co) * e)
        self.nops += 1
        gy = self.b_dense(lin.conv, x, rows, gp, co_pad, True, True)
        self.b_colsum(gp, rows, co_pad, self.slot(lin.b))
        c_out = self.c_feat
        if g_feat is not None:
            gf = g_feat if (g_feat.dtype == self.dtype and g_feat.is_contiguous()) else g_feat.contiguous().to(self.dtype)
            self.keep_gf = gf
            gy = self.b_add(gy, c_out, gf.data_ptr(), c_out, rows, c_out)
        gz_lin = 0
        if prog.spvcnn:
            gz_lin = self.b_point(prog.points[2], gy, flag=self.point_fork())
            gy = self.b_devox(gy, 0, c_out)
        g_skip = [0] * 5
        for i in (3, 2, 1, 0):
            dec, ra, rb = prog.ups[i]
            l = 3 - i
            if prog.spvcnn and i == 1:
                c2 = rb.c2.co
                gy = self.b_dropout(1, gy, n[2], c2)
                self.point_join()
                gz = self.b_vox(gy, 2, c2, gz_lin)
                gz_lin = self.b_point(prog.points[1], gz, flag=self.point_fork())
                gy = self.b_devox(gz, 2, c2)
            gy = self.b_res(rb, gy, n[l], k3[l])
            gcat = self.b_res(ra, gy, n[l], k3[l])
            c_up, c_cat = dec[0].co, ra.c1.ci
            g_skip[l] = (gcat + c_up * e, c_cat)
            gy = self.b_conv_bn(dec, gcat, c_cat, n[l + 1], n[l], k2[l])
        cs4 = prog.stages[3][2].c2.co
        if prog.spvcnn:
            gy = self.b_dropout(0, gy, n[4], cs4)
            self.point_join()
            gz = self.b_vox(gy, 4, cs4, gz_lin)
            gz_lin = self.b_point(prog.points[0], gz, flag=self.point_fork())
            gy = self.b_devox(gz, 4, cs4)
        for l in (3, 2, 1, 0):
            down, ra, rb = prog.stages[l]
            c = rb.c2.co
            if l < 3:
                gy = self.b_add(gy, c, g_skip[l + 1][0], g_skip[l + 1][1], n[l + 1], c)
            gy = self.b_res(rb, gy, n[l + 1], k3[l + 1])
            gy = self.b_res(ra, gy, n[l + 1], k3[l + 1])
            gy = self.b_conv_bn(down, gy, down[0].co, n[l], n[l + 1], k2[l])
        c0 = prog.stem[1][0].co
        if prog.spvcnn:
            self.point_join()
            gz0 = self.b_vox(gy, 0, c0, gz_lin)
            gy = self.b_devox(gz0, 0, c0)
        gy = self.b_add(gy, c0, g_skip[0][0], g_skip[0][1], n[0], c0)
        gy = self.b_conv_bn(prog.stem[1], gy, c0, n[0], n[0], k3[0])
        self.b_conv_bn(prog.stem[0], gy, prog.stem[0][0].co, n[0], n[0], k3[0], False, 8 if self.bf16 else 4)
        self.flush()
        self.done = True
        self.flat_t = None
        if self.tapes is not None and TRACE is not None:
            self.flat_t = flat
            TRACE.append(self)
        else:
            self.release()
        return self._grads(flat)

    def release(self):
        self.arena.release()
        if self.barena is not None:
            self.barena.release()
        self.saved = {}
        self.noise = []
        self.flat_t = None

    def _grads(self, flat):
        prog = self.prog
        views = [None] * len(prog.params)
        if prog.flat_exact:
            order = prog.flat_order
            if prog.flat_params is None:
                prog.flat_params = [prog.params[i] for i in order]
            parts = torch._C._nn.unflatten_dense_tensors(flat[:prog.flat_numel], prog.flat_params)
            for i, t in zip(order, parts):
                views[i] = t
        else:
            for i, p in enumerate(prog.params):
                views[i] = flat[prog.slot[i]:prog.slot[i] + p.numel()].view(p.shape)
        return views


class _EvalRun(_Run):
    TRAIN = False

    def __init__(self, model, prog, geometry, feats, code):
        prog.eval_operands(feats.device)
        _Run.__init__(self, model, prog, geometry, feats, code)

    def ccode(self, c):
        return B.conv_code(self.dtype, c.ci, True)

    def _constants(self):
        prog = self.prog
        if prog.ones is None or prog.ones.device != self.dev:
            prog.ones = torch.ones(512, dtype=torch.float32, device=self.dev)
            prog.cls_shift = torch.zeros(64, dtype=torch.float32, device=self.dev)
        self.ones = prog.ones.data_ptr()
        self.cls_shift = prog.cls_shift.data_ptr()

    def f_conv_bn(self, cb, x, n_in, table, n_out, ci=None):
        c, r = cb
        out = self.arena.alloc(n_out * c.co * self.esz)
        wb = _C.apply_workspace_bytes(n_out, c.co)
        self.w += (OP_CONV_APPLY_IMAGE_WS, x, c.img_f, table[0], table[1], table[2], out, n_in, n_out,
                   c.ci if ci is None else ci, c.co, c.k, 0, self.ccode(c), r.scale, r.shift, r.relu, 0, 0,
                   self.scratch(wb) if wb else 0, wb)
        self.nops += 1
        return out

    def f_res(self, r, x, n, table):
        A, e = self.arena, self.esz
        skip = x
        fl = 0
        if r.cs is not None:
            fl = 0
            skip = A.alloc(n * r.cs.co * e)
            self.w += (OP_CONV_APPLY_IMAGE | fl, x, r.cs.img_f, 0, 0, 0, skip, n, n, r.cs.ci, r.cs.co, 1, 0, self.ccode(r.cs),
                       r.bs.scale, r.bs.shift, 0, 0, 0)
            self.nops += 1
        y1 = A.alloc(n * r.c1.co * e)
        out = A.alloc(n * r.c2.co * e)
        wb1, wb2 = _C.apply_workspace_bytes(n, r.c1.co), _C.apply_workspace_bytes(n, r.c2.co)
        self.w += (OP_CONV_APPLY_IMAGE_WS, x, r.c1.img_f, table[0], table[1], table[2], y1, n, n, r.c1.ci, r.c1.co, r.c1.k,
                   0, self.ccode(r.c1), r.b1.scale, r.b1.shift, 1, 0, 0, self.scratch(wb1) if wb1 else 0, wb1)
        self.nops += 1
        if fl:
            self.join(2)
        self.w += (OP_CONV_APPLY_IMAGE_WS, y1, r.c2.img_f, table[0], table[1], table[2], out, n, n, r.c2.ci, r.c2.co,
                   r.c2.k, 0, self.ccode(r.c2), r.b2.scale, r.b2.shift, 2, skip, 0, self.scratch(wb2) if wb2 else 0, wb2)
        self.nops += 1
        return out

    def f_point(self, pt, z_in, devox_out, pre=None):
        lin, r = pt
        P = self.T.p
        out = self.arena.alloc(P * lin.co * self.esz)
        shift = self.prog._point_shift[self.prog.points.index(pt)]
        self.w += (OP_CONV_APPLY_IMAGE, z_in, lin.conv.img_f, 0, 0, 0, out, P, P, lin.ci, lin.co, 1, 0, self.ccode(lin.conv),
                   r.scale, shift, 1, devox_out, 0)
        self.nops += 1
        return out

    def f_dropout(self, addr, n, c):
        return

    def forward(self):
        out = _Run.forward(self)
        self.saved = {}
        if self.tapes is not None and TRACE is not None:
            TRACE.append(self)
        return out


class _PlannedNet(torch.autograd.Function):

    @staticmethod
    def forward(ctx, run, *params):
        ctx.run = run
        ctx.set_materialize_grads(False)
        return run.forward()

    @staticmethod
    def backward(ctx, g_logits, g_feat):
        B.note_backward()
        run = ctx.run
        if g_logits is None:
            rows = run.T.p if run.prog.spvcnn else run.T.n[0]
            g_logits = torch.zeros((rows, run.prog.n_class), dtype=run.dtype, device=run.dev)
        return (None,) + tuple(run.backward(g_logits, g_feat))


def planned_forward(model, x):
    mode = plannable(model, x)
    if mode is None:
        return None
    from .geometry import Geometry
    g = getattr(x, 'geometry', None)
    if g is None:
        g = Geometry.build(model, x.C, mode == 'train')
        if g.z is None:
            x.cmaps.update(g.x0.cmaps)
            x.kmaps.update(g.x0.kmaps)
    else:
        g.admit(x, type(model).__name__)
        if mode == 'train' and not g.grad:
            return None
    prog = model.__dict__['_lidal_program']
    code = B.BF16 if B.compute_dtype(x.F) == torch.bfloat16 else B.F32
    if mode == 'eval':
        return _EvalRun(model, prog, g, x.F, code).forward()
    run = _Run(model, prog, g, x.F, code)
    return _PlannedNet.apply(run, *prog.params)
# ... 1 lines not shown
```

lidal_amd/nn/functional/conv.py:

```python
import os

import torch
from torch.autograd import Function

from ... import backend as B
from ...tensor import SparseTensor
from ...utils import make_ntuple
from ..utils import get_kernel_offsets
from .downsample import spdownsample
from .hash import sphash
from .query import coords_table

__all__ = ['conv3d', 'KernelMap', 'RowOrder', 'build_kernel_map', 'prefetch_kernel_maps', 'conv_backward']


class RowOrder:

    def __init__(self, nbr, build=True):
        k, n = nbr.shape
        dev = nbr.device
        self.n_rows = n
        self.perm = B.empty(max(n, 1), torch.int, dev)
        self.table = B.empty((k, n), torch.int, dev)
        self.tile_masks = B.empty(max(1, -(-n // 128)), torch.int32, dev)
# ... 318 lines not shown
            return cache[key]
    w = weight.detach().contiguous()
    nbytes = L.lidal_conv_weight_image_bytes(k, n_red, n_col, code, n_out)
    img = torch.empty(nbytes, dtype=torch.uint8, device=w.device)
    B.check(L.lidal_conv_weight_image(B.ptr(w), B.dtype_code(w.dtype), role, B.ptr(img), code,
                                      k, n_red, n_col, n_out, B.stream()), 'conv_weight_image')
    if key is not None:
        if cache is None or next(iter(cache))[0] != B.weights_key(weight):
            cache = {}
            weight._lidal_images = cache
        cache[key] = img
    return img


_TILING = {}


def _tiling(n_red, n_col, code, n_out):
    key = (n_red, n_col, code, n_out)
    t = _TILING.get(key)
    if t is None:
        if len(_TILING) > 4096:
            _TILING.clear()
        t = _TILING[key] = B.lib().lidal_conv_weight_image_tiling(n_red, n_col, code, n_out)
    return t


class _ImageBank:

    def __init__(self):
        self.entries = {}
        self.serial = 0
        self.tables = {}
    KEEP = 8

    @property
    def tick(self):
        return B.WEIGHT_EPOCH[0]

    def get(self, weight, dtype, n_out_fwd, n_out_bwd, shape=None, role=0, code=None):
        import weakref
        k, ci, co = shape if shape is not None else weight.shape
        code = B.dtype_code(dtype) if code is None else code
        L = B.lib()
        key = (weight.data_ptr(), code, weight.dtype, _tiling(ci, co, code, n_out_fwd), _tiling(co, ci, code, n_out_bwd), role)
        ekey = (id(weight), key)
        e = self.entries.get(ekey)
        if e is None or e['ref']() is not weight:
            nf = L.lidal_conv_weight_image_bytes(k, ci, co, code, n_out_fwd)
            nb = (0 if (code == B.F32_SPLIT and (co % 32 != 0 or role))
                  else L.lidal_conv_weight_image_bytes(k, co, ci, code, n_out_bwd))
            buf = torch.empty(nf + nb, dtype=torch.uint8, device=weight.device)
            self.serial += 1
            wid = id(weight)

            def gone(_r, wid=wid):
                for kk in [kk for kk in self.entries if kk[0] == wid]:
                    self.entries.pop(kk, None)
            e = {'ref': weakref.ref(weight, gone), 'key': key,
                 'serial': self.serial,
                 'buf': buf, 'img_f': buf[:nf], 'img_b': buf[nf:], 'version': -1, 'code': code,
                 'n_out': (n_out_fwd, n_out_bwd), 'shape': (k, ci, co), 'role': role, 'used': self.tick,
                 'group': (str(weight.device), code, B.dtype_code(weight.dtype))}
            self.entries[ekey] = e
        e['used'] = self.tick
        if e['version'] != B.weights_key(weight):
            self._rebuild(e['group'])
        return e['img_f'], e['img_b']

    def entry(self, weight, tkey):
        for kk, e in self.entries.items():
            if kk[0] == id(weight) and (kk[1][3], kk[1][4], kk[1][1]) == tkey and e['ref']() is weight:
                return e
        return None

    def _rebuild(self, group):
        L = B.lib()
        stale = []
        for kk in [kk for kk, e in self.entries.items() if e['used'] < self.tick - self.KEEP]:
            del self.entries[kk]
        for e in self.entries.values():
            w = e['ref']()
            if w is not None and e['group'] == group and e['version'] != B.weights_key(w):
                stale.append((e, w))
        if not stale:
            return
        sig = tuple(e['serial'] for e, _ in stale)
        cached = self.tables.get(group)
        if cached is None or cached[0] != sig:
            import ctypes
            jb = L.lidal_conv_weight_image_job_bytes()
            host = ctypes.create_string_buffer(jb * len(stale))
            first = 0
            for i, (e, w) in enumerate(stale):
                k, ci, co = e['shape']
                n = L.lidal_conv_weight_image_job(ctypes.c_void_p(ctypes.addressof(host) + i * jb), B.ptr(w),
                                                  e['role'], B.ptr(e['img_f']), e['n_out'][0],
                                                  B.ptr(e['img_b']) if e['img_b'].numel() else None,
                                                  e['n_out'][1], e['code'], k, ci, co, first)
                if n < 0:
                    B.check(1, 'conv_weight_image_job')
                first += n
            table = torch.frombuffer(bytearray(host.raw), dtype=torch.uint8).to(stale[0][1].device)
            cached = (sig, table, len(stale), first)
            self.tables[group] = cached
        _, table, n_jobs, total = cached
        B.check(L.lidal_conv_weight_image_batch(B.ptr(table), n_jobs, total, group[2], group[1], B.stream()),
                'conv_weight_image')
        for e, w in stale:
            e['version'] = B.weights_key(w)


_IMAGE_BANK = _ImageBank()
_IMAGE_BATCH = os.environ.get('LIDAL_IMAGE_BATCH', '1') != '0'


def _weight_image_pair(weight, dtype, n_out_fwd, n_out_bwd, code=None):
    if _IMAGE_BATCH and isinstance(weight, torch.nn.Parameter) and weight.is_contiguous():
        return _IMAGE_BANK.get(weight, dtype, n_out_fwd, n_out_bwd, code=code)
    k, ci, co = weight.shape
    w = weight.detach().contiguous()
    if code == B.F32_SPLIT:
        with torch.enable_grad():
            return (_weight_image(w, dtype, n_out_fwd, 0, code), _weight_image(w, dtype, n_out_bwd, 1, code))
    code = B.dtype_code(dtype)
    L = B.lib()
    nf = L.lidal_conv_weight_image_bytes(k, ci, co, code, n_out_fwd)
    nb = L.lidal_conv_weight_image_bytes(k, co, ci, code, n_out_bwd)
    buf = torch.empty(nf + nb, dtype=torch.uint8, device=w.device)
    img_f, img_b = buf[:nf], buf[nf:]
    B.check(L.lidal_conv_weight_image_pair(B.ptr(w), B.dtype_code(w.dtype), B.ptr(img_f), n_out_fwd,
                                           B.ptr(img_b), n_out_bwd, code, k, ci, co, B.stream()),
            'conv_weight_image')
    return img_f, img_b


def _apply(feats, img, k, co, order, kflip, epilogue=None, want_stats=False, bnb=None, code=None):
    ci = feats.shape[1]
    n_out = order.n_rows
    out = torch.empty((n_out, co), dtype=feats.dtype, device=feats.device)
    scale, shift, relu = epilogue[:3] if epilogue is not None else (None, None, 0)
    residual = epilogue[3] if epilogue is not None and len(epilogue) > 3 else None
    if residual is not None:
        residual = residual.contiguous().to(feats.dtype)
        assert residual.shape == (n_out, co)
    stats = None
    want_stats = want_stats and feats.dtype == torch.bfloat16
    if want_stats:
        stats = torch.empty((-(-n_out // B.stats_tile_rows()), co, 3), dtype=torch.float32, device=feats.device)
    ws_bytes = apply_workspace_bytes(n_out, co)
    ws = B.workspace(ws_bytes, feats.device) if ws_bytes else None
    if bnb is not None:
        bx, mean, invstd, gamma, beta, relu_bn = bnb
        assert epilogue is None and not want_stats and bx.shape == (n_out, co) and bx.dtype == feats.dtype
        sums = torch.empty((-(-n_out // B.stats_tile_rows()), co, 2), dtype=torch.float32, device=feats.device)
        B.check(B.lib().lidal_conv_dgrad_bn_sums_ws(B.ptr(feats), B.ptr(img), B.ptr(order.table), B.ptr(order.perm),
                                                    B.ptr(order.tile_masks), B.ptr(out), feats.shape[0], n_out, ci,
                                                    co, k, int(kflip), B.dtype_code(feats.dtype), B.ptr(bx),
                                                    B.ptr(mean), B.ptr(invstd), B.ptr(gamma), B.ptr(beta),
                                                    int(bool(relu_bn)), B.ptr(sums), B.ptr(ws), ws_bytes, B.stream()),
                'conv_apply')
        out._lidal_bnb_sums = sums
        return out
    B.check(B.lib().lidal_conv_apply_image_ws(B.ptr(feats), B.ptr(img), B.ptr(order.table), B.ptr(order.perm),
                                              B.ptr(order.tile_masks), B.ptr(out), feats.shape[0], n_out, ci,
                                              co, k, int(kflip), B.dtype_code(feats.dtype) if code is None else code,
                                              B.ptr(scale), B.ptr(shift), int(relu), B.ptr(residual), B.ptr(stats),
                                              B.ptr(ws), ws_bytes, B.stream()),
            'conv_apply')
    if want_stats:
        out._lidal_bn_stats = stats
    return out


_APPLY_WS = {}
_SPLIT = os.environ.get('LIDAL_CONV_SPLIT', '1') != '0'


def apply_workspace_bytes(n_out, co):
    if not _SPLIT:
        return 0
    key = (n_out, co)
    v = _APPLY_WS.get(key)
    if v is None:
        if len(_APPLY_WS) > 4096:
            _APPLY_WS.clear()
        v = _APPLY_WS[key] = int(B.lib_handle().lidal_conv_apply_workspace_bytes(n_out, co))
    return v


def wgrad_scratch(n_a, n_b, k, ca, cb, dtype, device, code=None):
    slabs = int(B.lib().lidal_conv_wgrad_slabs(n_a, n_b, k, ca, cb, B.dtype_code(dtype) if code is None else code))
    return torch.empty((slabs, ca, cb), dtype=torch.float32, device=device)


def wgrad_plan(n_a, n_b, k, ca, cb, dtype):
    code = B.wgrad_code(dtype, ca, cb)
    L = B.lib_handle()
    if code == B.F32_SPLIT:
        slabs = int(L.lidal_conv_wgrad_slabs(n_a, n_b, k, ca, cb, code))
        if slabs > 0:
            return code, slabs
        code = B.dtype_code(dtype)
    return code, int(L.lidal_conv_wgrad_slabs(n_a, n_b, k, ca, cb, code))


def _pad_channels(ci, dtype):
    vec = 8 if dtype == torch.bfloat16 else 4
    return (-ci) % vec


def _bwd_order(kmap, transposed):
    if transposed:
        return kmap.order_out, 0
    return (kmap.order_out, 1) if kmap.symmetric else (kmap.order_in, 0)


def _forward(feats, weight, kmap, transposed, epilogue=None, with_bwd_image=False, want_stats=False, inference=False):
    B.require_gpu(feats, weight)
    cdtype = B.compute_dtype(feats)
    x = feats.contiguous().to(cdtype)
    pad = _pad_channels(x.shape[1], cdtype)
    if pad:
        x = torch.nn.functional.pad(x, (0, pad))
        weight = torch.nn.functional.pad(weight.detach(), (0, 0, 0, pad))
    order = kmap.order_in if transposed else kmap.order_out
    k, _, co = weight.shape
    img_b = None
    code = B.conv_code(cdtype, x.shape[1], inference and not want_stats, None if inference else co)
    if with_bwd_image:
        img, img_b = _weight_image_pair(weight, cdtype, order.n_rows, _bwd_order(kmap, transposed)[0].n_rows, code)
        img_b._lidal_code = code
        return x, _apply(x, img, k, co, order, 0, epilogue, want_stats, None, code), img_b
    img = _weight_image(weight, cdtype, order.n_rows, 0, code)
    return x, _apply(x, img, k, co, order, 0, epilogue, want_stats, None, code), img_b


def _conv(feats, weight, kmap, transposed, epilogue=None, want_stats=False, fork=False):
    if B.wants_grad(feats, weight):
        assert epilogue is None, 'the fused BatchNorm epilogue is inference-only'
        fused = fork and feats.requires_grad and _pad_channels(feats.shape[1], B.compute_dtype(feats)) == 0
        res = ConvolutionFunction.apply(feats, weight, kmap, transposed, want_stats, fused)
        out, skip = res if fused else (res, feats)
        if ConvolutionFunction.last_stats is not None:
            out._lidal_bn_stats = ConvolutionFunction.last_stats
            ConvolutionFunction.last_stats = None
        return (out, skip) if fork else out
    out = _forward(feats, weight, kmap, transposed, epilogue, False, want_stats, True)[1]
    return (out, feats) if fork else out


def conv_backward(x, weight, kmap, transposed, img_bwd, grad_output, grad_skip=None, need_gx=True, need_gw=True,
                  bnb=None):
    kmap.check_alive()
    g = grad_output.contiguous().to(x.dtype)
    n_in, n_out = kmap.sizes
    grad_in = grad_w = None
    k, ci_w, co = weight.shape
    ci = x.shape[1]

    def wgrad():
        gw = torch.empty((k, ci, co), dtype=torch.float32, device=x.device)
        if kmap.streams_serve(x.dtype, ci, co, transposed):
            spairs, sdesc, n_wg = kmap.streams()
            partial = torch.empty((2 * n_wg, ci, co), dtype=torch.float32, device=x.device)
            B.check(B.lib().lidal_conv_wgrad_streams(B.ptr(x), B.ptr(g), x.shape[0], g.shape[0], B.ptr(spairs), B.ptr(sdesc),
                                                     n_wg, 0, B.ptr(gw), B.ptr(partial), partial.shape[0], k, ci, co,
                                                     B.BF16, B.stream()), 'conv_wgrad_streams')
            gw = gw[:, :ci_w].contiguous() if ci != ci_w else gw
            return gw if weight.dtype == torch.float32 else gw.to(weight.dtype)
        code, slabs = wgrad_plan(x.shape[0], g.shape[0], k, ci, co, x.dtype)
        partial = torch.empty((slabs, ci, co), dtype=torch.float32, device=x.device)
        B.check(B.lib().lidal_conv_wgrad(B.ptr(x), B.ptr(g), x.shape[0], g.shape[0],
                                         B.ptr(kmap._nbmaps_cap), B.ptr(kmap.koff),
                                         1 if transposed else 0, B.ptr(gw), B.ptr(partial),
                                         partial.shape[0], k, ci, co, code,
                                         B.stream()), 'conv_wgrad')
        gw = gw[:, :ci_w].contiguous() if ci != ci_w else gw
        return gw if weight.dtype == torch.float32 else gw.to(weight.dtype)

    side = None
    if need_gw:
        if B.overlap_wgrad(x.dtype, max(n_in, n_out)) and need_gx:
            _ = kmap.koff
            side = B.beside(x.device, (x, g, kmap._nbmaps_cap, kmap.koff)
                            + (tuple(kmap.streams()[:2]) if kmap.streams_serve(x.dtype, ci, co, transposed) else ()), weight)
            with side as done:
                grad_w = wgrad()
                done(grad_w)
        else:
            grad_w = wgrad()
    if need_gx:
        order, kflip = _bwd_order(kmap, transposed)
        ep = (None, None, 0, grad_skip) if grad_skip is not None else None
        if bnb is not None and (ep is not None or ci != ci_w or g.dtype != torch.bfloat16 or ci % 8 != 0
                                or tuple(bnb[0].shape) != (n_out if transposed else n_in, ci)
                                or bnb[0].dtype != g.dtype or not bnb[0].is_contiguous()):
            bnb = None
        grad_in = _apply(g, img_bwd, k, x.shape[1], order, kflip, ep, False, bnb, getattr(img_bwd, '_lidal_code', None))
        if ci != ci_w:
            grad_in = grad_in[:, :ci_w]
    elif grad_skip is not None:
        grad_in = grad_skip
    if side is not None:
        side.finish()
    return grad_in, grad_w


class ConvolutionFunction(Function):
    last_stats = None

    @staticmethod
    def forward(ctx, feats, weight, kmap, transposed, want_stats=False, fork=False):
        x, out, ctx.img_bwd = _forward(feats, weight, kmap, transposed, None, ctx.needs_input_grad[0],
                                       want_stats)
        ConvolutionFunction.last_stats = getattr(out, '_lidal_bn_stats', None) if want_stats else None
        ctx.kmap = kmap
        ctx.transposed = transposed
        ctx.save_for_backward(x, weight)
        return (out, feats) if fork else out

    @staticmethod
    def backward(ctx, grad_output, grad_skip=None):
        B.note_backward()
        x, weight = ctx.saved_tensors
        grad_in, grad_w = conv_backward(x, weight, ctx.kmap, ctx.transposed, ctx.img_bwd, grad_output, grad_skip,
                                        ctx.needs_input_grad[0], ctx.needs_input_grad[1])
        return grad_in, grad_w, None, None, None, None


def conv3d(input, weight, kernel_size, bias=None, stride=1, dilation=1, transposed=False,
           epilogue=None, want_stats=False, fork=False):
    feats, coords = input.feats, input.coords
    kernel_size = make_ntuple(kernel_size, ndim=3)
    stride = make_ntuple(stride, ndim=3)
    dilation = make_ntuple(dilation, ndim=3)

    if kernel_size == (1, 1, 1) and stride == (1, 1, 1) and dilation == (1, 1, 1):
        B.require_gpu(feats)
        from .dense import rows_matmul
        feats = rows_matmul(feats, weight, bias, epilogue, want_stats)
        output = SparseTensor(feats, coords, input.stride)
    elif not transposed:
        if dilation != (1, 1, 1):
            raise NotImplementedError('dilated sparse conv is not on the LiDAL path')
        key = (input.stride, kernel_size, stride, dilation)
        kmap = input.kmaps.get(key)
        trace = getattr(input.kmaps, 'trace', None)
        if trace is not None and key[:3] not in trace['maps']:
            trace['maps'].append(key[:3])
        out_stride = tuple(input.stride[k] * stride[k] for k in range(3))
        if kmap is None:
            kmap, out_coords = build_kernel_map(coords, input.stride, kernel_size, stride, input.cmaps)
            input.kmaps[key] = kmap
            if any(s > 1 for s in stride):
                input.cmaps.setdefault(out_stride, out_coords)
        out_coords = coords if all(s == 1 for s in stride) else input.cmaps[out_stride]
        if fork:
            feats, skip_feats = _conv(feats, weight, kmap, False, epilogue, want_stats and bias is None, True)
        else:
            feats = _conv(feats, weight, kmap, False, epilogue, want_stats and bias is None)
        if bias is not None:
            feats = feats + bias
        output = SparseTensor(feats, out_coords, out_stride)
    else:
        tensor_stride = tuple(input.stride[k] // stride[k] for k in range(3))
        kmap = input.kmaps[(tensor_stride, kernel_size, stride, dilation)]
        trace = getattr(input.kmaps, 'trace', None)
        if trace is not None:
            trace['transposed'] = True
        feats = _conv(feats, weight, kmap, True, epilogue, want_stats and bias is None)
        if bias is not None:
            feats = feats + bias
        output = SparseTensor(feats, input.cmaps[tensor_stride], tensor_stride)
    output.cmaps = input.cmaps
    output.cmaps.setdefault(output.stride, output.coords)
    output.kmaps = input.kmaps
    if fork:
        assert kernel_size != (1, 1, 1) and not transposed, 'fork: k > 1, not transposed'
        skip = SparseTensor(skip_feats, coords, input.stride)
        skip.cmaps, skip.kmaps = input.cmaps, input.kmaps
        return output, skip
    return output
```

lidal_amd/operators.py:

```python
import torch

from .tensor import SparseTensor

__all__ = ['cat']


def cat(inputs):
    out = SparseTensor(torch.cat([x.feats for x in inputs], dim=1), inputs[0].coords,
                       inputs[0].stride)
    out.cmaps = inputs[0].cmaps
    out.kmaps = inputs[0].kmaps
    return out
```

Measured before the change: 29.30 million voxels/s.

## Fuse upstream BatchNorm backward sums into residual dgrad with skip epilogue

Extends the image-conv dgrad epilogue so it can add the residual skip gradient and also compute the next BatchNorm layer's backward reduction sums over a column subset (bn_c ≤ co). The sums are carried across autograd nodes and planned ops (residual block to the following down/up conv-BN), so the separate BN backward column-sum pass over the gradient is skipped. This adds LDS writeback of the residual-added values, extra register arrays and bookkeeping through a global carry dict keyed by data pointer, which could be fragile.

```diff
diff --git a/include/lidal_amd.h b/include/lidal_amd.h
--- a/include/lidal_amd.h
+++ b/include/lidal_amd.h
@@ -145,6 +145,12 @@
                                 int c_gin, int k, int kflip, int dtype, const void* bn_x, const float* bn_mean,
                                 const float* bn_invstd, const float* bn_gamma, const float* bn_beta, int bn_relu,
                                 float* bn_sums, void* ws, int64_t ws_bytes, void* stream);
+int lidal_conv_dgrad_res_bn_sums_ws(const void* gout, const void* wimg, const int32_t* nbr, const int32_t* perm,
+                                    const uint32_t* tile_masks, void* gin, int64_t n_gout, int64_t n_gin, int c_gout,
+                                    int c_gin, int k, int kflip, int dtype, const void* residual, const void* bn_x,
+                                    int bn_c, const float* bn_mean, const float* bn_invstd, const float* bn_gamma,
+                                    const float* bn_beta, int bn_relu, float* bn_sums, void* ws, int64_t ws_bytes,
+                                    void* stream);
 int64_t lidal_conv_wgrad_slabs(int64_t n_a, int64_t n_b, int k, int ca, int cb, int dtype);
 int lidal_conv_wgrad(const void* a, const void* b, int64_t n_a, int64_t n_b, const int32_t* pairs,
                      const int64_t* koff, int a_col, float* gw, float* partial, int64_t n_slabs,
@@ -290,6 +296,7 @@
   LIDAL_OP_CONV_WGRAD_STREAMS = 34
 };
 #define LIDAL_OP_FLAG_SIDE 1
+#define LIDAL_OP_FLAG_RES_BN_SUMS 16
 int lidal_plan_op_args(int kind);
 int lidal_debug_read(const void* dev, void* host, int64_t nbytes);
 int lidal_plan_run(const int64_t* words, int64_t n_words, int64_t n_ops, void* stream, void* side_stream);
diff --git a/lidal_amd/backend.py b/lidal_amd/backend.py
--- a/lidal_amd/backend.py
+++ b/lidal_amd/backend.py
@@ -84,6 +84,8 @@
                                          _vp, _i32, _vp, _vp, _vp, _i64, _vp]),
     'lidal_conv_dgrad_bn_sums_ws': (_i32, [_vp, _vp, _vp, _vp, _vp, _vp, _i64, _i64, _i32, _i32, _i32, _i32, _i32, _vp,
                                            _vp, _vp, _vp, _vp, _i32, _vp, _vp, _i64, _vp]),
+    'lidal_conv_dgrad_res_bn_sums_ws': (_i32, [_vp, _vp, _vp, _vp, _vp, _vp, _i64, _i64, _i32, _i32, _i32, _i32, _i32,
+                                               _vp, _vp, _i32, _vp, _vp, _vp, _vp, _i32, _vp, _vp, _i64, _vp]),
     'lidal_conv_wgrad_slabs': (_i64, [_i64, _i64, _i32, _i32, _i32, _i32]),
     'lidal_conv_wgrad': (_i32, [_vp, _vp, _i64, _i64, _vp, _vp, _i32, _vp, _vp, _i64, _i32, _i32, _i32, _i32, _vp]),
     'lidal_conv_wgrad_streams': (_i32, [_vp, _vp, _i64, _i64, _vp, _vp, _i32, _i32, _vp, _vp, _i64, _i32, _i32, _i32, _i32, _vp]),
diff --git a/lidal_amd/csrc/conv_img.hip b/lidal_amd/csrc/conv_img.hip
--- a/lidal_amd/csrc/conv_img.hip
+++ b/lidal_amd/csrc/conv_img.hip
@@ -153,6 +153,7 @@
   const void* x; const float* mean; const float* invstd; const float* gamma; const float* beta;
   float* sums;
   int relu;
+  int c;
 };
 
 struct Split { float* partial; int nsplit; int co_pad; long long rows_pad; };
@@ -196,13 +197,16 @@
         et[(g * 16 + gsel * 4 + r) * ESTRIDE + nb * 16 + row16] = DT<T>::from_f32(acc[g][nb][r]);
   __builtin_amdgcn_s_waitcnt(0xC07F);
   constexpr int RSEGS = BN / VEC;
+  const int bn_c = (bnb != nullptr && bnb->sums != nullptr) ? (bnb->c > 0 ? bnb->c : co) : 0;
+  const bool bn_job = n0 < bn_c;
+  const bool bn_res = bn_job && ep_res != nullptr;
   for (int i = lane; i < RW * RSEGS; i += 64) {
     const int r = i / RSEGS, cseg = (i - r * RSEGS) * VEC;
     const int prow = perm_in_reg ? __shfl(perm_v, r & (RW - 1), 64) : 0;
     if (r0 + r >= n_out) continue;
     const int64_t row = perm ? (perm_in_reg ? (int64_t)prow : (int64_t)perm[r0 + r]) : r0 + r;
     T* dst = out + row * co + n0 + cseg;
-    const T* srcp = et + r * ESTRIDE + cseg;
+    T* srcp = et + r * ESTRIDE + cseg;
     if (n0 + cseg + VEC <= co) {
       frag v = *reinterpret_cast<const frag*>(srcp);
       if (ep_res != nullptr) {
@@ -213,6 +217,7 @@
           if ((ep_relu & 2) && f < 0.f) f = 0.f;
           v[e] = DT<T>::from_f32(f);
         }
+        if (bn_res) *reinterpret_cast<frag*>(srcp) = v;
       }
       *reinterpret_cast<frag*>(dst) = v;
     } else {
@@ -281,22 +286,23 @@
       dst[0] = na; dst[1] = ma; dst[2] = qa;
     }
   }
-  if (bnb != nullptr && bnb->sums != nullptr) {
+  if (bn_job) {
     constexpr int EPI_BYTES = NWAVES * RW * ESTRIDE * (int)sizeof(T);
     float* st = reinterpret_cast<float*>(wl + EPI_BYTES);
     const T* bx = reinterpret_cast<const T*>(bnb->x);
     const int64_t left = n_out - r0;
     const int nvalid = left <= 0 ? 0 : (left < RW ? (int)left : RW);
     __builtin_amdgcn_s_waitcnt(0xC07F);
+    auto take_sums = [&](f32x4 (&dyv)[G][NB]) {
     for (int i = lane; i < RW * RSEGS; i += 64) {
       const int r = i / RSEGS, cseg = (i - r * RSEGS) * VEC;
       const int prow = perm_in_reg ? __shfl(perm_v, r & (RW - 1), 64) : 0;
       frag v;
 #pragma unroll
       for (int e = 0; e < VEC; ++e) v[e] = DT<T>::from_f32(0.f);
-      if (r < nvalid && n0 + cseg + VEC <= co) {
+      if (r < nvalid && n0 + cseg + VEC <= bn_c) {
         const int64_t row = perm ? (perm_in_reg ? (int64_t)prow : (int64_t)perm[r0 + r]) : r0 + r;
-        v = *reinterpret_cast<const frag*>(bx + row * co + n0 + cseg);
+        v = *reinterpret_cast<const frag*>(bx + row * bn_c + n0 + cseg);
       }
       *reinterpret_cast<frag*>(et + r * ESTRIDE + cseg) = v;
     }
@@ -304,7 +310,7 @@
 #pragma unroll
     for (int nb = 0; nb < NB; ++nb) {
       const int col = n0 + nb * 16 + row16;
-      const bool cok = col < co;
+      const bool cok = col < bn_c;
       const float mu = cok ? bnb->mean[col] : 0.f, is = cok ? bnb->invstd[col] : 0.f;
       const float ga = (cok && bnb->gamma) ? bnb->gamma[col] : 1.f, be = (cok && bnb->beta) ? bnb->beta[col] : 0.f;
       float a = 0.f, b = 0.f;
@@ -315,7 +321,7 @@
           const int rr = g * 16 + gsel * 4 + r;
           if (rr < nvalid) {
             const float xh = (DT<T>::to_f32(et[rr * ESTRIDE + nb * 16 + row16]) - mu) * is;
-            float dy = DT<T>::to_f32(DT<T>::from_f32(acc[g][nb][r]));
+            float dy = DT<T>::to_f32(DT<T>::from_f32(dyv[g][nb][r]));
             if (bnb->relu && !(xh * ga + be > 0.f)) dy = 0.f;
             a += dy; b += dy * xh;
           }
@@ -327,9 +333,24 @@
         st[(wave * BN + nb * 16 + row16) * 2 + 1] = b;
       }
     }
+    };
+    if (bn_res) {
+      f32x4 dyv[G][NB];
+#pragma unroll
+      for (int g = 0; g < G; ++g)
+#pragma unroll
+        for (int nb = 0; nb < NB; ++nb)
+#pragma unroll
+          for (int r = 0; r < 4; ++r)
+            dyv[g][nb][r] = DT<T>::to_f32(et[(g * 16 + gsel * 4 + r) * ESTRIDE + nb * 16 + row16]);
+      __builtin_amdgcn_s_waitcnt(0xC07F);
+      take_sums(dyv);
+    } else {
+      take_sums(acc);
+    }
     __syncthreads();
     const int c = wave * 64 + lane;
-    if (c < BN && n0 + c < co) {
+    if (c < BN && n0 + c < bn_c) {
       float a = 0.f, b = 0.f;
       for (int w = 0; w < NWAVES; ++w) { a += st[(w * BN + c) * 2]; b += st[(w * BN + c) * 2 + 1]; }
       float* dst = bnb->sums + ((int64_t)(n0 + c) * gridDim.x + (stats_tile >= 0 ? stats_tile : (int)blockIdx.x)) * 2;
@@ -1472,7 +1493,7 @@
       comb_attr[dev] = COMB_LDS;
     }
     grid.z = 1;
-    BnBwd none{nullptr, nullptr, nullptr, nullptr, nullptr, nullptr, 0};
+    BnBwd none{nullptr, nullptr, nullptr, nullptr, nullptr, nullptr, 0, 0};
     ck<<<grid, 64 * LW, COMB_LDS, s>>>(sp, perm, (float*)out, n_out, co, ep.scale, ep.shift, ep.relu, (const float*)ep.res,
                                        nullptr, none);
     LIDAL_CHECK_LAUNCH("lidal_conv_apply_image(split, combine)");
@@ -1661,9 +1682,9 @@
                 vec, MAXK, ci, co, k);
   LIDAL_REQUIRE(nbr == nullptr ? (k == 1 && n_in == n_out) : (tile_masks != nullptr),
                 "conv_apply_image: needs lidal_kmap_order's tile masks (or NULL table = identity, k = 1)");
-  LIDAL_REQUIRE(bnb.sums == nullptr || (co % vec == 0 && ep_residual == nullptr && ep_scale == nullptr &&
-                                        tile_stats == nullptr && bnb.x && bnb.mean && bnb.invstd),
-                "conv_apply_image: BatchNorm backward sums need whole 16-byte column vectors, no other epilogue");
+  LIDAL_REQUIRE(bnb.sums == nullptr || (co % vec == 0 && ep_scale == nullptr && ep_relu == 0 && tile_stats == nullptr &&
+                                        bnb.x && bnb.mean && bnb.invstd && bnb.c >= 0 && bnb.c <= co && bnb.c % vec == 0),
+                "conv_apply_image: BatchNorm backward sums need whole 16-byte column vectors, no epilogue but a residual");
   const Tiling t = pick_tiling(ci, co, n_out, esz);
   const int64_t ib = image_bytes(k, ci, co, t, esz);
   LIDAL_REQUIRE(n_in >= 0 && n_in * ci * esz < 0x7FFFFFF0ll && ib < 0x7FFFFFF0ll,
@@ -1689,7 +1710,7 @@
                                       int dtype, const float* ep_scale, const float* ep_shift,
                                       int ep_relu, const void* ep_residual, float* tile_stats,
                                       void* stream) {
-  BnBwd none{nullptr, nullptr, nullptr, nullptr, nullptr, nullptr, 0};
+  BnBwd none{nullptr, nullptr, nullptr, nullptr, nullptr, nullptr, 0, 0};
   return conv_apply_image(in, wimg, nbr, perm, tile_masks, out, n_in, n_out, ci, co, k, kflip, dtype, ep_scale,
                           ep_shift, ep_relu, ep_residual, tile_stats, none, nullptr, 0, (hipStream_t)stream);
 }
@@ -1706,7 +1727,7 @@
                                          int dtype, const float* ep_scale, const float* ep_shift,
                                          int ep_relu, const void* ep_residual, float* tile_stats, void* ws,
                                          int64_t ws_bytes, void* stream) {
-  BnBwd none{nullptr, nullptr, nullptr, nullptr, nullptr, nullptr, 0};
+  BnBwd none{nullptr, nullptr, nullptr, nullptr, nullptr, nullptr, 0, 0};
   return conv_apply_image(in, wimg, nbr, perm, tile_masks, out, n_in, n_out, ci, co, k, kflip, dtype, ep_scale,
                           ep_shift, ep_relu, ep_residual, tile_stats, none, ws, ws_bytes, (hipStream_t)stream);
 }
@@ -1717,7 +1738,7 @@
                                         int dtype, const void* bn_x, const float* bn_mean,
                                         const float* bn_invstd, const float* bn_gamma, const float* bn_beta,
                                         int bn_relu, float* bn_sums, void* stream) {
-  BnBwd b{bn_x, bn_mean, bn_invstd, bn_gamma, bn_beta, bn_sums, bn_relu};
+  BnBwd b{bn_x, bn_mean, bn_invstd, bn_gamma, bn_beta, bn_sums, bn_relu, 0};
   return conv_apply_image(gout, wimg, nbr, perm, tile_masks, gin, n_gout, n_gin, c_gout, c_gin, k, kflip, dtype,
                           nullptr, nullptr, 0, nullptr, nullptr, b, nullptr, 0, (hipStream_t)stream);
 }
@@ -1728,7 +1749,19 @@
                                            int dtype, const void* bn_x, const float* bn_mean,
                                            const float* bn_invstd, const float* bn_gamma, const float* bn_beta,
                                            int bn_relu, float* bn_sums, void* ws, int64_t ws_bytes, void* stream) {
-  BnBwd b{bn_x, bn_mean, bn_invstd, bn_gamma, bn_beta, bn_sums, bn_relu};
+  BnBwd b{bn_x, bn_mean, bn_invstd, bn_gamma, bn_beta, bn_sums, bn_relu, 0};
   return conv_apply_image(gout, wimg, nbr, perm, tile_masks, gin, n_gout, n_gin, c_gout, c_gin, k, kflip, dtype,
                           nullptr, nullptr, 0, nullptr, nullptr, b, ws, ws_bytes, (hipStream_t)stream);
 }
+
+extern "C" int lidal_conv_dgrad_res_bn_sums_ws(const void* gout, const void* wimg, const int32_t* nbr,
+                                               const int32_t* perm, const uint32_t* tile_masks, void* gin,
+                                               int64_t n_gout, int64_t n_gin, int c_gout, int c_gin, int k, int kflip,
+                                               int dtype, const void* residual, const void* bn_x, int bn_c,
+                                               const float* bn_mean, const float* bn_invstd, const float* bn_gamma,
+                                               const float* bn_beta, int bn_relu, float* bn_sums, void* ws,
+                                               int64_t ws_bytes, void* stream) {
+  BnBwd b{bn_x, bn_mean, bn_invstd, bn_gamma, bn_beta, bn_sums, bn_relu, bn_c};
+  return conv_apply_image(gout, wimg, nbr, perm, tile_masks, gin, n_gout, n_gin, c_gout, c_gin, k, kflip, dtype,
+                          nullptr, nullptr, 0, residual, nullptr, b, ws, ws_bytes, (hipStream_t)stream);
+}
diff --git a/lidal_amd/csrc/plan.hip b/lidal_amd/csrc/plan.hip
--- a/lidal_amd/csrc/plan.hip
+++ b/lidal_amd/csrc/plan.hip
@@ -308,6 +308,17 @@
                                       CP(float, 16), CP(float, 17), I(18), MP(float, 19), st);
         break;
       case LIDAL_OP_CONV_APPLY_IMAGE_WS:
+        if (flags & LIDAL_OP_FLAG_RES_BN_SUMS) {
+          const int64_t* d = CP(int64_t, 18);
+          LIDAL_REQUIRE(d != nullptr && L(19) == 10 && a[13] == 0 && a[14] == 0 && a[15] == 0 && a[17] == 0,
+                        "plan_run: op %lld (conv_apply_image_ws with BatchNorm sums) is malformed", (long long)op);
+          rc = lidal_conv_dgrad_res_bn_sums_ws(P(0), P(1), CP(int32_t, 2), CP(int32_t, 3), CP(uint32_t, 4), P(5), L(6), L(7),
+                                               I(8), I(9), I(10), I(11), I(12), P(16), (const void*)(uintptr_t)d[2], (int)d[3],
+                                               (const float*)(uintptr_t)d[4], (const float*)(uintptr_t)d[5],
+                                               (const float*)(uintptr_t)d[6], (const float*)(uintptr_t)d[7], (int)d[8],
+                                               (float*)(uintptr_t)d[9], (void*)(uintptr_t)d[0], d[1], st);
+          break;
+        }
         rc = lidal_conv_apply_image_ws(P(0), P(1), CP(int32_t, 2), CP(int32_t, 3), CP(uint32_t, 4), P(5), L(6), L(7),
                                        I(8), I(9), I(10), I(11), I(12), CP(float, 13), CP(float, 14), I(15), P(16),
                                        MP(float, 17), P(18), L(19), st);
diff --git a/lidal_amd/network/blocks.py b/lidal_amd/network/blocks.py
--- a/lidal_amd/network/blocks.py
+++ b/lidal_amd/network/blocks.py
@@ -30,6 +30,7 @@
 
 
 class _ConvNormAct(torch.autograd.Function):
+    last_bn = None
 
     @staticmethod
     def forward(ctx, feats, kernel, gamma, beta, kmap, transposed, bn, relu, stats):
@@ -40,13 +41,16 @@
                                                      getattr(x1, '_lidal_bn_stats', None))
         ctx.kmap, ctx.transposed, ctx.relu = kmap, transposed, relu
         ctx.save_for_backward(xc, kernel, x1, w, b, mean, invstd)
+        _C.drop_carried_sums()
+        _ConvNormAct.last_bn = (x1, mean, invstd, w, b, relu)
         return y
 
     @staticmethod
     def backward(ctx, g):
         B.note_backward()
         xc, kernel, x1, w, b, mean, invstd = ctx.saved_tensors
-        dx, gg, gb, _ = _N.train_backward(x1, w, b, mean, invstd, ctx.relu, g, True)
+        dx, gg, gb, _ = _N.train_backward(x1, w, b, mean, invstd, ctx.relu, g, True, None,
+                                          _C.carried_sums(g, x1) if BN_SUMS else None)
         gx, gk = _C.conv_backward(xc, kernel, ctx.kmap, ctx.transposed, ctx.img_bwd, dx, None,
                                   ctx.needs_input_grad[0], ctx.needs_input_grad[1])
         return gx, gk, gg, gb, None, None, None, None, None
@@ -55,7 +59,9 @@
 class _Residual(torch.autograd.Function):
 
     @staticmethod
-    def forward(ctx, feats, k1, g1, b1, k2, g2, b2, ks, gs, bs, kmap, bn1, bn2, bns, stats):
+    def forward(ctx, feats, k1, g1, b1, k2, g2, b2, ks, gs, bs, kmap, bn1, bn2, bns, stats, bn_src=None):
+        _C.drop_carried_sums()
+        ctx.bn_src = bn_src
         need_gx = ctx.needs_input_grad[0]
         xc, x1, ctx.img1 = _C._forward(feats, k1, kmap, False, None, need_gx, stats[0])
         y1, mean1, inv1, x1, w1, c1 = _N.train_forward(x1, g1, b1, bn1.running_mean, bn1.running_var, bn1.momentum,
@@ -99,9 +105,12 @@
                                     (x1, mean1, inv1, w1, c1, True) if BN_SUMS else None)
         dx1, gg1, gb1, _ = _N.train_backward(x1, w1, c1, mean1, inv1, True, dy1, True, None,
                                              getattr(dy1, '_lidal_bnb_sums', None))
+        src = ctx.bn_src if (BN_SUMS and need_gx) else None
         gx, gk1 = _C.conv_backward(xc, k1, ctx.kmap, False, ctx.img1, dx1, g_skip if need_gx else None, need_gx,
-                                   ctx.needs_input_grad[1])
-        return gx, gk1, gg1, gb1, gk2, gg2, gb2, gks, ggs, gbs, None, None, None, None, None
+                                   ctx.needs_input_grad[1], src)
+        if src is not None:
+            _C.carry_sums(gx, src[0])
+        return gx, gk1, gg1, gb1, gk2, gg2, gb2, gks, ggs, gbs, None, None, None, None, None, None
 
 
 def _kmap_of(x, conv):
@@ -140,7 +149,10 @@
     kmap, coords, stride = _kmap_of(x, conv)
     y = _ConvNormAct.apply(x.F, conv.kernel, bn.weight, bn.bias, kmap, conv.transposed, bn, bool(bn.fused_relu),
                            bool(conv.bn_follows))
-    return _wrap(y, coords, stride, x)
+    out = _wrap(y, coords, stride, x)
+    out.bn_src = (y,) + _ConvNormAct.last_bn
+    _ConvNormAct.last_bn = None
+    return out
 
 
 class ConvNormSequential(nn.Sequential):
@@ -294,8 +306,10 @@
             return None
         kmap, coords, stride = _kmap_of(x, c1)
         stats = (bool(c1.bn_follows), bool(c2.bn_follows), bool(ks is not None and self.downsample[0].bn_follows))
+        src = getattr(x, 'bn_src', None)
+        src = src[1:] if (BN_SUMS and src is not None and src[0] is x.F) else None
         out = _Residual.apply(x.F, c1.kernel, n1.weight, n1.bias, c2.kernel, n2.weight, n2.bias, ks, gs, bs, kmap,
-                              n1, n2, ns, stats)
+                              n1, n2, ns, stats, src)
         return _wrap(out, coords, stride, x)
 
     def forward(self, x):
diff --git a/lidal_amd/network/plan.py b/lidal_amd/network/plan.py
--- a/lidal_amd/network/plan.py
+++ b/lidal_amd/network/plan.py
@@ -25,6 +25,7 @@
 OP_FORK_SIDE, OP_JOIN_SIDE, OP_CONV_APPLY_IMAGE_WS, OP_CONV_DGRAD_BN_SUMS_WS = 26, 27, 28, 29
 OP_ADD_RELU_BWD_BN_SUMS, OP_BN_BWD_FROM_SUMS, OP_ADD_RELU_BWD_BN_TILE_SUMS, OP_DEVOXELIZE_BWD_CELLS = 30, 31, 32, 33
 OP_CONV_WGRAD_STREAMS = 34
+FLAG_RES_BN_SUMS = 16 << 16
 
 COUNTERS = {'ops': 0, 'plans': 0}
 TALLY = os.environ.get('LIDAL_PLAN_TALLY', '0') != '0'
@@ -493,6 +494,7 @@
         self.tile = B.stats_tile_rows()
         from . import blocks
         self.bn_sums = (blocks.BN_SUMS if BN_SUMS is None else BN_SUMS) and self.bf16
+        self.desc = []
         self.saved = {}
         self.noise = []
         self.keep = []
@@ -882,7 +884,16 @@
         gin = self.galloc(n_out * c.ci * self.esz)
         wb = _C.apply_workspace_bytes(n_out, c.ci)
         ws = self.scratch(wb) if wb else 0
+        if bnb is not None and (skip or bnb[6] != c.ci):
+            sums = self.galloc(-(-n_out // self.tile) * bnb[6] * 8)
+            desc = array.array('q', (ws, wb, bnb[0], bnb[6]) + tuple(bnb[1:6]) + (sums,))
+            self.desc.append(desc)
+            self.w += (OP_CONV_APPLY_IMAGE_WS | FLAG_RES_BN_SUMS, g, c.img_b, table[0], table[1], table[2], gin, n_g, n_out,
+                       c.co, c.ci, c.k, kflip, self.code, 0, 0, 0, skip, 0, desc.buffer_info()[0], 10)
+            self.nops += 1
+            return gin, sums
         if bnb is not None:
+            bnb = bnb[:6]
             sums = self.galloc(-(-n_out // self.tile) * c.ci * 8)
             self.w += (OP_CONV_DGRAD_BN_SUMS_WS, g, c.img_b, table[0], table[1], table[2], gin, n_g, n_out, c.co, c.ci,
                        c.k, kflip, self.code) + bnb + (sums, ws, wb)
@@ -918,10 +929,10 @@
         self.w += (OP_COLSUM | flag, g, self.code, n, c, out, self.scratch(nb, flag), nb)
         self.nops += 1
 
-    def b_conv_bn(self, cb, g, g_stride, n_in, n_out, tables, need_gx=True, ci=None):
+    def b_conv_bn(self, cb, g, g_stride, n_in, n_out, tables, need_gx=True, ci=None, sums=0):
         c, r = cb
         x, x1, mean, invstd = self.saved[id(cb)]
-        dx = self.b_bn(r, x1, n_out, mean, invstd, g, g_stride)
+        dx = self.b_bn(r, x1, n_out, mean, invstd, g, g_stride, sums)
         if c.transposed:
             rules, table, n_gin, kflip = tables[6:8], tables[0:3], n_in, 0
         elif c.strided:
@@ -933,7 +944,7 @@
             return 0
         return self.b_dgrad(c, dx, n_out, table, n_gin, kflip)[0]
 
-    def b_res(self, r, g, n, k3):
+    def b_res(self, r, g, n, k3, unit=None):
         x, x1, mean1, inv1, y1, x2, mean2, inv2, out, xs, means, invs = self.saved[id(r)]
         co = r.c2.co
         gm = self.galloc(n * co * self.esz)
@@ -965,13 +976,20 @@
         table, rules = k3[0:3], k3[3:8]
         self.b_wgrad(r.c2, y1, n, dx2, n, rules)
         p = self.ptr
-        bnb = (x1, mean1, inv1, p[r.b1.w], p[r.b1.b], 1) if self.bn_sums else None
+        bnb = (x1, mean1, inv1, p[r.b1.w], p[r.b1.b], 1, r.c1.co) if self.bn_sums else None
         dy1, sums = self.b_dgrad(r.c2, dx2, n, table, n, 1, 0, bnb)
         dx1 = self.b_bn(r.b1, x1, n, mean1, inv1, dy1, r.c1.co, sums)
         self.b_wgrad(r.c1, x, n, dx1, n, rules)
         if fl:
             self.join(2)
-        return self.b_dgrad(r.c1, dx1, n, table, n, 1, g_skip)[0]
+        if unit is None:
+            return self.b_dgrad(r.c1, dx1, n, table, n, 1, g_skip)[0]
+        bnb = None
+        ub = unit[1]
+        if self.bn_sums and ub.c % 8 == 0 and ub.c <= r.c1.ci and r.c1.ci % 8 == 0:
+            _, ux1, umean, uinv = self.saved[id(unit)]
+            bnb = (ux1, umean, uinv, p[ub.w], p[ub.b], int(bool(ub.relu)), ub.c)
+        return self.b_dgrad(r.c1, dx1, n, table, n, 1, g_skip, bnb)
 
     def b_add(self, a, a_stride, b, b_stride, n, c):
         out = self.galloc(n * c * self.esz)
@@ -1078,10 +1096,10 @@
                 gz_lin = self.b_point(prog.points[1], gz, flag=self.point_fork())
                 gy = self.b_devox(gz, 2, c2)
             gy = self.b_res(rb, gy, n[l], k3[l])
-            gcat = self.b_res(ra, gy, n[l], k3[l])
+            gcat, sums = self.b_res(ra, gy, n[l], k3[l], dec)
             c_up, c_cat = dec[0].co, ra.c1.ci
             g_skip[l] = (gcat + c_up * e, c_cat)
-            gy = self.b_conv_bn(dec, gcat, c_cat, n[l + 1], n[l], k2[l])
+            gy = self.b_conv_bn(dec, gcat, c_cat, n[l + 1], n[l], k2[l], sums=sums)
         cs4 = prog.stages[3][2].c2.co
         if prog.spvcnn:
             gy = self.b_dropout(0, gy, n[4], cs4)
@@ -1095,8 +1113,8 @@
             if l < 3:
                 gy = self.b_add(gy, c, g_skip[l + 1][0], g_skip[l + 1][1], n[l + 1], c)
             gy = self.b_res(rb, gy, n[l + 1], k3[l + 1])
-            gy = self.b_res(ra, gy, n[l + 1], k3[l + 1])
-            gy = self.b_conv_bn(down, gy, down[0].co, n[l], n[l + 1], k2[l])
+            gy, sums = self.b_res(ra, gy, n[l + 1], k3[l + 1], down)
+            gy = self.b_conv_bn(down, gy, down[0].co, n[l], n[l + 1], k2[l], sums=sums)
         c0 = prog.stem[1][0].co
         if prog.spvcnn:
             self.point_join()
diff --git a/lidal_amd/nn/functional/conv.py b/lidal_amd/nn/functional/conv.py
--- a/lidal_amd/nn/functional/conv.py
+++ b/lidal_amd/nn/functional/conv.py
@@ -494,8 +494,19 @@
     ws = B.workspace(ws_bytes, feats.device) if ws_bytes else None
     if bnb is not None:
         bx, mean, invstd, gamma, beta, relu_bn = bnb
-        assert epilogue is None and not want_stats and bx.shape == (n_out, co) and bx.dtype == feats.dtype
-        sums = torch.empty((-(-n_out // B.stats_tile_rows()), co, 2), dtype=torch.float32, device=feats.device)
+        assert not want_stats and bx.shape[0] == n_out and bx.shape[1] <= co and bx.dtype == feats.dtype
+        assert scale is None and not relu
+        bn_c = bx.shape[1]
+        sums = torch.empty((-(-n_out // B.stats_tile_rows()), bn_c, 2), dtype=torch.float32, device=feats.device)
+        if residual is not None or bn_c != co:
+            B.check(B.lib().lidal_conv_dgrad_res_bn_sums_ws(B.ptr(feats), B.ptr(img), B.ptr(order.table), B.ptr(order.perm),
+                                                            B.ptr(order.tile_masks), B.ptr(out), feats.shape[0], n_out,
+                                                            ci, co, k, int(kflip), B.dtype_code(feats.dtype),
+                                                            B.ptr(residual), B.ptr(bx), bn_c, B.ptr(mean), B.ptr(invstd),
+                                                            B.ptr(gamma), B.ptr(beta), int(bool(relu_bn)), B.ptr(sums),
+                                                            B.ptr(ws), ws_bytes, B.stream()), 'conv_apply')
+            out._lidal_bnb_sums = sums
+            return out
         B.check(B.lib().lidal_conv_dgrad_bn_sums_ws(B.ptr(feats), B.ptr(img), B.ptr(order.table), B.ptr(order.perm),
                                                     B.ptr(order.tile_masks), B.ptr(out), feats.shape[0], n_out, ci,
                                                     co, k, int(kflip), B.dtype_code(feats.dtype), B.ptr(bx),
@@ -635,8 +646,10 @@
     if need_gx:
         order, kflip = _bwd_order(kmap, transposed)
         ep = (None, None, 0, grad_skip) if grad_skip is not None else None
-        if bnb is not None and (ep is not None or ci != ci_w or g.dtype != torch.bfloat16 or ci % 8 != 0
-                                or tuple(bnb[0].shape) != (n_out if transposed else n_in, ci)
+        if bnb is not None and (ci != ci_w or g.dtype != torch.bfloat16 or ci % 8 != 0
+                                or bnb[0].shape[0] != (n_out if transposed else n_in)
+                                or bnb[0].shape[1] % 8 != 0 or bnb[0].shape[1] > ci
+                                or (bnb[0].shape[1] != ci and ep is None)
                                 or bnb[0].dtype != g.dtype or not bnb[0].is_contiguous()):
             bnb = None
         grad_in = _apply(g, img_bwd, k, x.shape[1], order, kflip, ep, False, bnb, getattr(img_bwd, '_lidal_code', None))
@@ -647,6 +660,28 @@
     if side is not None:
         side.finish()
     return grad_in, grad_w
+
+
+_CARRIED = {}
+
+
+def carry_sums(grad_in, bn_x):
+    sums = getattr(grad_in, '_lidal_bnb_sums', None)
+    if sums is not None:
+        _CARRIED[grad_in.data_ptr()] = (bn_x.data_ptr(), grad_in.shape[0], grad_in.shape[1], grad_in._version, sums)
+
+
+def carried_sums(g, bn_x):
+    e = _CARRIED.pop(g.data_ptr(), None) if _CARRIED else None
+    if (e is None or e[0] != bn_x.data_ptr() or g.dim() != 2 or g.shape[0] != e[1] or g.stride(0) != e[2]
+            or g.stride(1) != 1 or g._version != e[3] or g.dtype != bn_x.dtype):
+        return None
+    return e[4]
+
+
+def drop_carried_sums():
+    if _CARRIED:
+        _CARRIED.clear()
 
 
 class ConvolutionFunction(Function):
diff --git a/lidal_amd/operators.py b/lidal_amd/operators.py
--- a/lidal_amd/operators.py
+++ b/lidal_amd/operators.py
@@ -10,4 +10,7 @@
                        inputs[0].stride)
     out.cmaps = inputs[0].cmaps
     out.kmaps = inputs[0].kmaps
+    src = getattr(inputs[0], 'bn_src', None)
+    if src is not None and src[0] is inputs[0].feats:
+        out.bn_src = (out.feats,) + src[1:]
     return out
```

Result: slower. 27.09 million voxels/s (-7.6%).
